# AcherStyx/SSD-Object-Detection

Measured on AMD Instinct MI355X. Metric: images/sec SSD300 train step, batch 64, higher is better.
Workload: dtype bf16; 1 GPU; BASELINE configs[2]: SSD300 full train step (anchor match+encode, image normalisation, conv fwd, loss, conv bwd, per-variable clip (64 variables) + Adam), per-GPU batch 64, 80 classes, synthetic COCO-shaped boxes; per_gpu_batch=64, global_batch=64, parallelism=single

## Files before the change

### include/ssd_hip.h

```cpp
#ifndef SSD_HIP_H
#define SSD_HIP_H

#include <stddef.h>
#include <stdint.h>

#ifdef __cplusplus
extern "C" {
#endif

typedef enum {
    SSD_OK = 0,
    SSD_ERR_ASSERT = -1,
    SSD_ERR_VALUE = -2,
    SSD_ERR_WORKSPACE = -3,
    SSD_ERR_LAUNCH = -4,
    SSD_ERR_UNSUPPORTED = -5
} ssd_status;

typedef enum { SSD_F32 = 0, SSD_BF16 = 1 } ssd_dtype;

int ssd_hip_abi_version(void);
const char* ssd_status_string(int status);

int ssd_priors_count(const int* grid_hw, int levels, const int* ratio_off);
int ssd_priors(const int* grid_hw, int levels, const double* s_ref, const int* ratios,
               const int* ratio_off, double in_size, double* out, void* stream);

#define SSD_MAX_LEVELS 8
#define SSD_GRID_VERIFIED 0x5D5D0001
typedef struct {
    int levels;
    int grid_h[SSD_MAX_LEVELS];
    int grid_w[SSD_MAX_LEVELS];
    int per_cell[SSD_MAX_LEVELS];
    int verified;
} ssd_prior_grid;

int ssd_prior_grid_verify(const double* priors, int A, ssd_prior_grid* grid, int32_t* scratch, void* stream);

int ssd_encode_zero(const double* priors, int A, float* enc_zero, void* stream);

size_t ssd_match_encode_workspace_bytes(int B, int A, int total_gt);
int ssd_match_encode(const float* gt_box, const float* gt_cls, const int32_t* gt_off, int B,
                     int total_gt, int max_nt, const double* priors, const float* enc_zero, int A,
                     const ssd_prior_grid* grid, double thresh, int32_t* out_cls, float* out_loc,
                     uint8_t* out_mask, int32_t* out_owner, void* ws, size_t ws_bytes, void* stream);

int ssd_apply_anchor_box(const float* box, const double* priors, int n, double* out, void* stream);

int ssd_iou_n(const float* b1, const double* b2, int n, double* out, void* stream);

size_t ssd_loss_workspace_bytes(int B, int A, int C);
int ssd_loss_fwd_bwd(const void* conf, const void* loc, int dtype, const int32_t* gt_cls,
                     const float* gt_loc, const uint8_t* gt_mask, int B, int A, int C, float grad_scale,
                     float* out8, void* dconf, void* dloc, void* ws, size_t ws_bytes, void* stream);

typedef struct {
    int levels;
    int hw[SSD_MAX_LEVELS];
    int per_cell[SSD_MAX_LEVELS];
    int npad[SSD_MAX_LEVELS];
    void* rows[SSD_MAX_LEVELS];
    int32_t* row_of_pixel[SSD_MAX_LEVELS];
    int32_t* pixel_of_row[SSD_MAX_LEVELS];
    int32_t* count;
} ssd_head_grads;
size_t ssd_loss_heads_workspace_bytes(int B, int A, int C);
int ssd_loss_fwd_bwd_heads(const void* conf, const void* loc, int dtype, const int32_t* gt_cls, const float* gt_loc,
                           const uint8_t* gt_mask, int B, int A, int C, float grad_scale, float* out8,
                           const ssd_head_grads* hg, void* ws, size_t ws_bytes, int ws_clean, void* stream);

int ssd_score_decode(const void* conf, const void* loc, int dtype, const double* priors, int B, int A, int C,
                     float score_thresh, double in_size, float* score, int32_t* cls, float* box,
                     uint8_t* cand, void* stream);

int ssd_nms_max_candidates(void);
int ssd_nms(const float* score, const int32_t* cls, const float* box, const uint8_t* cand, int B, int A,
            float iou_thresh, int max_cand, uint8_t* keep, int32_t* keep_count, void* stream);

int ssd_conv2d_fwd(const void* x, const void* w, const float* bias, void* y, int B, int H, int W, int Cin,
                   int Cout, int ksize, int stride, int pad_t, int pad_l, int Ho, int Wo, int relu, void* ws,
                   size_t ws_bytes, void* stream);
int ssd_conv2d_fwd_pool(const void* x, const void* w, const float* bias, void* y, void* y_pool, void* pool_code, int B, int H,
                        int W, int Cin, int Cout, int ksize, int stride, int pad_t, int pad_l, int Ho, int Wo, int relu, int Hp,
                        int Wp, void* ws, size_t ws_bytes, void* stream);
int ssd_conv2d_head_fwd(const void* x, const void* w, const float* bias, void* loc, void* conf, int B, int H, int W,
                        int Cin, int per_cell, int classes, int anchors_total, int level_off, void* ws, size_t ws_bytes,
                        void* stream);
int ssd_conv2d_bwd_data(const void* dy, const void* w_t, const void* relu_src, void* dx, int B, int H, int W, int Cin,
                        int Cout_pad, int ksize, int stride, int pad_t, int pad_l, int Ho, int Wo, int accumulate,
                        void* ws, size_t ws_bytes, void* stream);

int ssd_conv2d_fwd_relubits(const void* x, const void* w, const float* bias, void* y, void* relu_bits, int B, int H, int W, int Cin,
                            int Cout, int ksize, int stride, int pad_t, int pad_l, int Ho, int Wo, void* ws, size_t ws_bytes,
                            void* stream);
int ssd_conv2d_bwd_data_bits(const void* dy, const void* w_t, const void* relu_bits, void* dx, int B, int H, int W, int Cin,
                             int Cout_pad, int ksize, int stride, int pad_t, int pad_l, int Ho, int Wo, int accumulate, void* ws,
                             size_t ws_bytes, void* stream);
size_t ssd_conv2d_bwd_data_wgrad_first_workspace_bytes(int B, int H, int W);
int ssd_conv2d_bwd_data_wgrad_first(const void* dy, const void* w_t, const void* relu_bits, const void* image, float* dw0,
                                    float* dbias0, int B, int H, int W, void* ws, size_t ws_bytes, void* stream);
int ssd_conv2d_bwd_data_unpool(const void* dy, const void* w_t, const void* relu_src, const void* pool_code, void* dx_pooled,
                               void* dx_full, int B, int H, int W, int Cin, int Cout_pad, int Hf, int Wf, void* ws, size_t ws_bytes,
                               void* stream);
size_t ssd_conv2d_bwd_weight_unpooled_workspace_bytes(int B, int H, int W, int Cin, int Cout, int Hp, int Wp);
int ssd_conv2d_bwd_weight_unpooled(const void* x, const void* dpool, const void* pool_code, float* dw, float* dbias, int B, int H,
                                   int W, int Cin, int Cout, int Hp, int Wp, void* ws, size_t ws_bytes, void* stream);
size_t ssd_conv2d_bwd_weight_workspace_bytes(int B, int Ho, int Wo, int Cin, int Cout, int ldy, int ksize);
int ssd_conv2d_bwd_weight(const void* x, const void* dy, float* dw, float* dbias, int B, int H, int W, int Cin,
                          int Cout, int ldy, int ksize, int stride, int pad_t, int pad_l, int Ho, int Wo, void* ws,
                          size_t ws_bytes, void* stream);
typedef struct {
    const void* x;
    const void* dy;
    float* dw;
    float* dbias;
    int B, H, W, Cin, Cout, ldy, ksize, stride, pad_t, pad_l, Ho, Wo;
} ssd_wgrad_item;
size_t ssd_conv2d_bwd_weight_batched_workspace_bytes(const ssd_wgrad_item* items, int count);
int ssd_conv2d_bwd_weight_batched(const ssd_wgrad_item* items, int count, void* ws, size_t ws_bytes, void* stream);
int ssd_set_wgrad_reduce_stream(void* stream);
int ssd_weight_transpose(const void* w, void* w_t, int Cout, int ksize, int Cin, int Cout_pad, void* stream);
int ssd_weight_transpose_batched(const long long* desc, int ntensors, int max_tiles, void* stream);
int ssd_cast_bf16(const float* src, void* dst, long long n, void* stream);
int ssd_image_prep(const float* img, void* out, int B, int H, int W, int normalize, void* stream);
int ssd_image_resize_prep(const void* src, const int64_t* src_off, const int32_t* src_hw, void* out, int B, int S,
                          int normalize, void* stream);
int ssd_box_prep(const float* box_tlwh, const int32_t* gt_off, const int32_t* src_hw, float* box_out, int B, int total_gt,
                 void* stream);
int ssd_maxpool2x2_fwd(const void* x, void* y, int B, int H, int W, int C, int Ho, int Wo, void* stream);
int ssd_maxpool2x2_bwd(const void* x, const void* y, const void* dy, void* dx, int B, int H, int W, int C, int Ho,
                       int Wo, void* stream);
int ssd_maxpool2x2_fwd_argmax(const void* x, void* y, void* code, int B, int H, int W, int C, int Ho, int Wo, void* stream);
int ssd_maxpool2x2_bwd_argmax(const void* code, const void* dy, void* dx, int B, int H, int W, int C, int Ho, int Wo,
                              void* stream);
int ssd_quantize_mx_fp8(const void* x_bf16, void* q, void* scale, long long n, void* stream);
int ssd_conv3x3_fwd_mxfp8(const void* x8, const void* xscale, const void* w8, const void* wscale, const float* bias, void* y, int B,
                          int H, int W, int Cin, int Cout, int relu, void* stream);
int ssd_conv2d_fwd_mxfp8(const void* x8, const void* xscale, const void* w8, const void* wscale, const float* bias, void* y_bf16,
                         void* y8, void* yscale, int B, int H, int W, int Cin, int Cout, int k, int stride, int pad_t, int pad_l,
                         int Ho, int Wo, int relu, void* stream);
int ssd_add_relu_fwd_mxfp8(const void* a, const void* b, void* out_bf16, void* q, void* scale, long long n, void* stream);
int ssd_conv2d_fwd_pool_mxfp8(const void* x8, const void* xscale, const void* w8, const void* wscale, const float* bias,
                              void* y_pool_bf16, void* y_pool8, void* y_pool_scale, int B, int H, int W, int Cin, int Cout, int k,
                              int stride, int pad_t, int pad_l, int Ho, int Wo, int relu, int Hp, int Wp, void* stream);
int ssd_conv2d_bwd_data_mxfp8(const void* dy8, const void* dyscale, const void* wt8, const void* wtscale, const void* relu_src,
                              void* dx_bf16, void* dx8, void* dxscale, int B, int H, int W, int Cin, int Cout, int k, int pad_t,
                              int pad_l, int Ho, int Wo, int accumulate, void* stream);
#define SSD_CHAIN_MAX_LAYERS 8
#define SSD_CHAIN_PACK_MAX 16
typedef struct {
    const void* src;
    void* dst;
    int N, K;
} ssd_chain_pack;
int ssd_chain_pack_weights(const ssd_chain_pack* items, int count, void* stream);
int ssd_chain_prefetch(const ssd_chain_pack* items, int count, void* stream);
typedef struct {
    const void* w;
    const float* bias;
    void* out;
    const void* mask_bits;
    const void* mask_src;
    void* relu_bits;
    int Hi, Wi, Kc, Ho, Wo, N, ksize, mul, div, pad_t, pad_l, relu, accumulate;
} ssd_chain_layer;
int ssd_conv_chain(const void* in0, const ssd_chain_layer* layers, int nlayers, int B, void* stream);
int ssd_add_relu_fwd(const void* a, const void* b, void* out, long long n, void* stream);
int ssd_relu_mask_bwd(const void* g, const void* act, void* out, int accumulate, long long n, void* stream);
int ssd_maxpool3x3s2_fwd(const void* x, void* y, void* code, int B, int H, int W, int C, int Ho, int Wo, int pad_t, int pad_l,
                         void* stream);
int ssd_maxpool3x3s2_bwd(const void* code, const void* dy, void* dx, int B, int H, int W, int C, int Ho, int Wo, int pad_t, int pad_l,
                         void* stream);
typedef struct {
    int levels;
    int H[SSD_MAX_LEVELS], W[SSD_MAX_LEVELS], Cin[SSD_MAX_LEVELS], cout[SSD_MAX_LEVELS];
    const void* x[SSD_MAX_LEVELS];
    const void* w_tap[SSD_MAX_LEVELS];
    const void* relu_bits[SSD_MAX_LEVELS];
    const void* relu_src[SSD_MAX_LEVELS];
    void* dx[SSD_MAX_LEVELS];
    float* dw[SSD_MAX_LEVELS];
    float* dbias[SSD_MAX_LEVELS];
} ssd_head_layers;
size_t ssd_heads_bwd_data_sparse_workspace_bytes(int B, const ssd_head_layers* hl);
int ssd_heads_bwd_data_sparse(const ssd_head_grads* hg, const ssd_head_layers* hl, int B, void* ws, size_t ws_bytes,
                              void* stream);
int ssd_heads_bwd_data_sparse_levels(const ssd_head_grads* hg, const ssd_head_layers* hl, int B, unsigned level_mask, int prezeroed,
                                     void* ws, size_t ws_bytes, void* stream);
size_t ssd_heads_bwd_weight_sparse_workspace_bytes(int B, const ssd_head_grads* hg, const ssd_head_layers* hl);
int ssd_heads_bwd_weight_sparse(const ssd_head_grads* hg, const ssd_head_layers* hl, int B, void* ws, size_t ws_bytes,
                                void* stream);

int ssd_head_grad_pack(const void* dloc, const void* dconf, void* out, int B, int hw, int per_cell, int classes,
                       int npad, int anchors_total, int level_off, void* stream);

int ssd_opt_block_elems(void);
int ssd_grad_clip_scales(const float* grad, long long n, const int32_t* tensor_block_off, int ntensors, float clip,
                         double* partial, float* scale, float* norms, void* stream);
int ssd_grad_apply_scale(float* grad, long long n, const int32_t* block_tensor, const float* scale, void* stream);
int ssd_grad_accumulate(float* acc, const float* grad, long long n, const int32_t* block_tensor, const float* scale,
                        int first, void* stream);
int ssd_adam_step(float* param, const float* grad, float* m, float* v, void* param_bf16, long long n,
                  const int32_t* block_tensor, const float* scale, float grad_scale, float lr_t, float beta1,
                  float beta2, float eps, void* stream);
int ssd_sgd_step(float* param, const float* grad, void* param_bf16, long long n, const int32_t* block_tensor,
                 const float* scale, float grad_scale, float lr, void* stream);

enum ssd_conv_plan {
    SSD_PLAN_KERNEL_MASK = 0xff,
    SSD_PLAN_C64B = 1, SSD_PLAN_P32_64, SSD_PLAN_P32_128, SSD_PLAN_8PH,
    SSD_PLAN_DMA_256_256, SSD_PLAN_DMA_256_128, SSD_PLAN_DMA_256_64, SSD_PLAN_DMA_128_64, SSD_PLAN_DMA_128_128,
    SSD_PLAN_CONV0_FWD, SSD_PLAN_P512, SSD_PLAN_PW,
    SSD_PLAN_WG_FIRST = 32, SSD_PLAN_WG_PATCH_16x16, SSD_PLAN_WG_PATCH_6x40, SSD_PLAN_WG_PATCH_10x24, SSD_PLAN_WG_TILE,
    SSD_PLAN_WG_GENERIC,
    SSD_PLAN_F_FLAT = 0x100,
    SSD_PLAN_F_ROWFLAT = 0x200,
    SSD_PLAN_F_SPLITK = 0x400,
    SSD_PLAN_F_POOL_FUSED = 0x800,
    SSD_PLAN_F_S2 = 0x1000,
    SSD_PLAN_F_REDUCE_WIDE = 0x2000
};
int ssd_conv2d_fwd_plan(int B, int H, int W, int Cin, int Cout, int ksize, int stride, int pad_t, int pad_l, int Ho, int Wo,
                        int pool, size_t ws_bytes);
int ssd_conv2d_head_fwd_plan(int B, int H, int W, int Cin, int per_cell, int classes, size_t ws_bytes);
int ssd_conv2d_bwd_data_plan(int B, int H, int W, int Cin, int Cout_pad, int ksize, int stride, int pad_t, int pad_l, int Ho,
                             int Wo, int accumulate, size_t ws_bytes);
int ssd_conv2d_bwd_weight_plan(int B, int H, int W, int Cin, int Cout, int ldy, int ksize, int stride, int pad_t, int pad_l,
                               int Ho, int Wo);
const char* ssd_conv_plan_name(int plan);

int ssd_dev_knob(const char* name, int value);

int ssd_dev_mfma_calibration_workgroups(void);
double ssd_dev_mfma_calibration_flops(int iters);
int ssd_dev_mfma_calibration(int iters, void* stamps, void* sink, void* stream);

#ifdef __cplusplus
}
#endif
#endif
```

### ssd-object-detection_amd/_lib.py

```python
import ctypes
import os

HERE = os.path.dirname(os.path.abspath(__file__))
LIB_PATH = os.path.join(HERE, os.environ.get("SSD_HIP_LIB", "libssd_hip.so"))

SSD_OK, SSD_ERR_ASSERT, SSD_ERR_VALUE, SSD_ERR_WORKSPACE, SSD_ERR_LAUNCH, SSD_ERR_UNSUPPORTED = 0, -1, -2, -3, -4, -5
SSD_MAX_LEVELS = 8

_c_int_p = ctypes.POINTER(ctypes.c_int)
_c_double_p = ctypes.POINTER(ctypes.c_double)
VP = ctypes.c_void_p


class PriorGrid(ctypes.Structure):
    _fields_ = [("levels", ctypes.c_int),
                ("grid_h", ctypes.c_int * SSD_MAX_LEVELS),
                ("grid_w", ctypes.c_int * SSD_MAX_LEVELS),
                ("per_cell", ctypes.c_int * SSD_MAX_LEVELS),
                ("verified", ctypes.c_int)]


class HeadGrads(ctypes.Structure):
    _fields_ = [("levels", ctypes.c_int),
                ("hw", ctypes.c_int * SSD_MAX_LEVELS),
                ("per_cell", ctypes.c_int * SSD_MAX_LEVELS),
                ("npad", ctypes.c_int * SSD_MAX_LEVELS),
                ("rows", VP * SSD_MAX_LEVELS),
                ("row_of_pixel", VP * SSD_MAX_LEVELS),
                ("pixel_of_row", VP * SSD_MAX_LEVELS),
                ("count", VP)]


class HeadLayers(ctypes.Structure):
    _fields_ = [("levels", ctypes.c_int),
                ("H", ctypes.c_int * SSD_MAX_LEVELS),
                ("W", ctypes.c_int * SSD_MAX_LEVELS),
                ("Cin", ctypes.c_int * SSD_MAX_LEVELS),
                ("cout", ctypes.c_int * SSD_MAX_LEVELS),
                ("x", VP * SSD_MAX_LEVELS),
                ("w_tap", VP * SSD_MAX_LEVELS),
                ("relu_bits", VP * SSD_MAX_LEVELS),
                ("relu_src", VP * SSD_MAX_LEVELS),
                ("dx", VP * SSD_MAX_LEVELS),
                ("dw", VP * SSD_MAX_LEVELS),
                ("dbias", VP * SSD_MAX_LEVELS)]


class ChainLayer(ctypes.Structure):
    _fields_ = [("w", VP), ("bias", VP), ("out", VP), ("mask_bits", VP), ("mask_src", VP), ("relu_bits", VP)] + \
               [(n, ctypes.c_int) for n in ("Hi", "Wi", "Kc", "Ho", "Wo", "N", "ksize", "mul", "div", "pad_t", "pad_l", "relu",
                                            "accumulate")]


class WgradItem(ctypes.Structure):
    _fields_ = [("x", VP), ("dy", VP), ("dw", VP), ("dbias", VP)] + \
               [(n, ctypes.c_int) for n in ("B", "H", "W", "Cin", "Cout", "ldy", "ksize", "stride", "pad_t", "pad_l", "Ho", "Wo")]


class ChainPack(ctypes.Structure):
    _fields_ = [("src", VP), ("dst", VP), ("N", ctypes.c_int), ("K", ctypes.c_int)]


SSD_CHAIN_MAX_LAYERS = 8
SSD_CHAIN_PACK_MAX = 16
_HG = ctypes.POINTER(HeadGrads)
_HL = ctypes.POINTER(HeadLayers)

_SIGNATURES = {
    "ssd_hip_abi_version": (ctypes.c_int, []),
    "ssd_status_string": (ctypes.c_char_p, [ctypes.c_int]),
    "ssd_priors_count": (ctypes.c_int, [_c_int_p, ctypes.c_int, _c_int_p]),
    "ssd_priors": (ctypes.c_int, [_c_int_p, ctypes.c_int, _c_double_p, _c_int_p, _c_int_p, ctypes.c_double, VP, VP]),
    "ssd_encode_zero": (ctypes.c_int, [VP, ctypes.c_int, VP, VP]),
    "ssd_prior_grid_verify": (ctypes.c_int, [VP, ctypes.c_int, ctypes.POINTER(PriorGrid), VP, VP]),
    "ssd_match_encode_workspace_bytes": (ctypes.c_size_t, [ctypes.c_int, ctypes.c_int, ctypes.c_int]),
    "ssd_match_encode": (ctypes.c_int, [VP, VP, VP, ctypes.c_int, ctypes.c_int, ctypes.c_int, VP, VP, ctypes.c_int,
                                        ctypes.POINTER(PriorGrid), ctypes.c_double, VP, VP, VP, VP, VP, ctypes.c_size_t, VP]),
    "ssd_apply_anchor_box": (ctypes.c_int, [VP, VP, ctypes.c_int, VP, VP]),
    "ssd_iou_n": (ctypes.c_int, [VP, VP, ctypes.c_int, VP, VP]),
    "ssd_score_decode": (ctypes.c_int, [VP, VP, ctypes.c_int, VP, ctypes.c_int, ctypes.c_int, ctypes.c_int,
                                        ctypes.c_float, ctypes.c_double, VP, VP, VP, VP, VP]),
    "ssd_nms_max_candidates": (ctypes.c_int, []),
    "ssd_nms": (ctypes.c_int, [VP, VP, VP, VP, ctypes.c_int, ctypes.c_int, ctypes.c_float, ctypes.c_int, VP, VP, VP]),
    "ssd_conv2d_fwd": (ctypes.c_int, [VP, VP, VP, VP] + [ctypes.c_int] * 12 + [VP, ctypes.c_size_t, VP]),
    "ssd_conv2d_fwd_pool": (ctypes.c_int, [VP, VP, VP, VP, VP, VP] + [ctypes.c_int] * 14 + [VP, ctypes.c_size_t, VP]),
    "ssd_conv2d_head_fwd": (ctypes.c_int, [VP, VP, VP, VP, VP] + [ctypes.c_int] * 8 + [VP, ctypes.c_size_t, VP]),
    "ssd_conv2d_bwd_data": (ctypes.c_int, [VP, VP, VP, VP] + [ctypes.c_int] * 12 + [VP, ctypes.c_size_t, VP]),
    "ssd_conv2d_fwd_relubits": (ctypes.c_int, [VP] * 5 + [ctypes.c_int] * 11 + [VP, ctypes.c_size_t, VP]),
    "ssd_conv2d_bwd_data_bits": (ctypes.c_int, [VP] * 4 + [ctypes.c_int] * 12 + [VP, ctypes.c_size_t, VP]),
    "ssd_conv2d_bwd_data_unpool": (ctypes.c_int, [VP] * 6 + [ctypes.c_int] * 7 + [VP, ctypes.c_size_t, VP]),
    "ssd_quantize_mx_fp8": (ctypes.c_int, [VP, VP, VP, ctypes.c_longlong, VP]),
    "ssd_conv3x3_fwd_mxfp8": (ctypes.c_int, [VP] * 6 + [ctypes.c_int] * 6 + [VP]),
    "ssd_conv2d_fwd_mxfp8": (ctypes.c_int, [VP] * 8 + [ctypes.c_int] * 12 + [VP]),
    "ssd_add_relu_fwd_mxfp8": (ctypes.c_int, [VP] * 5 + [ctypes.c_longlong, VP]),
    "ssd_conv2d_bwd_data_mxfp8": (ctypes.c_int, [VP] * 8 + [ctypes.c_int] * 11 + [VP]),
    "ssd_conv2d_fwd_pool_mxfp8": (ctypes.c_int, [VP] * 8 + [ctypes.c_int] * 14 + [VP]),
    "ssd_chain_pack_weights": (ctypes.c_int, [ctypes.POINTER(ChainPack), ctypes.c_int, VP]),
    "ssd_chain_prefetch": (ctypes.c_int, [ctypes.POINTER(ChainPack), ctypes.c_int, VP]),
    "ssd_set_wgrad_reduce_stream": (ctypes.c_int, [VP]),
    "ssd_conv2d_bwd_weight_batched_workspace_bytes": (ctypes.c_size_t, [ctypes.POINTER(WgradItem), ctypes.c_int]),
    "ssd_conv2d_bwd_weight_batched": (ctypes.c_int, [ctypes.POINTER(WgradItem), ctypes.c_int, VP, ctypes.c_size_t, VP]),
    "ssd_conv_chain": (ctypes.c_int, [VP, ctypes.POINTER(ChainLayer), ctypes.c_int, ctypes.c_int, VP]),
    "ssd_add_relu_fwd": (ctypes.c_int, [VP, VP, VP, ctypes.c_longlong, VP]),
    "ssd_relu_mask_bwd": (ctypes.c_int, [VP, VP, VP, ctypes.c_int, ctypes.c_longlong, VP]),
    "ssd_maxpool3x3s2_fwd": (ctypes.c_int, [VP, VP, VP] + [ctypes.c_int] * 8 + [VP]),
    "ssd_maxpool3x3s2_bwd": (ctypes.c_int, [VP, VP, VP] + [ctypes.c_int] * 8 + [VP]),
    "ssd_conv2d_bwd_weight_unpooled_workspace_bytes": (ctypes.c_size_t, [ctypes.c_int] * 7),
    "ssd_conv2d_bwd_weight_unpooled": (ctypes.c_int, [VP] * 5 + [ctypes.c_int] * 7 + [VP, ctypes.c_size_t, VP]),
    "ssd_conv2d_bwd_data_wgrad_first_workspace_bytes": (ctypes.c_size_t, [ctypes.c_int] * 3),
    "ssd_conv2d_bwd_data_wgrad_first": (ctypes.c_int, [VP] * 6 + [ctypes.c_int] * 3 + [VP, ctypes.c_size_t, VP]),
    "ssd_conv2d_bwd_weight_workspace_bytes": (ctypes.c_size_t, [ctypes.c_int] * 7),
    "ssd_conv2d_bwd_weight": (ctypes.c_int, [VP, VP, VP, VP] + [ctypes.c_int] * 12 + [VP, ctypes.c_size_t, VP]),
    "ssd_weight_transpose": (ctypes.c_int, [VP, VP, ctypes.c_int, ctypes.c_int, ctypes.c_int, ctypes.c_int, VP]),
    "ssd_cast_bf16": (ctypes.c_int, [VP, VP, ctypes.c_longlong, VP]),
    "ssd_image_prep": (ctypes.c_int, [VP, VP, ctypes.c_int, ctypes.c_int, ctypes.c_int, ctypes.c_int, VP]),
    "ssd_image_resize_prep": (ctypes.c_int, [VP, VP, VP, VP, ctypes.c_int, ctypes.c_int, ctypes.c_int, VP]),
    "ssd_box_prep": (ctypes.c_int, [VP, VP, VP, VP, ctypes.c_int, ctypes.c_int, VP]),
    "ssd_maxpool2x2_fwd": (ctypes.c_int, [VP, VP] + [ctypes.c_int] * 6 + [VP]),
    "ssd_maxpool2x2_bwd": (ctypes.c_int, [VP, VP, VP, VP] + [ctypes.c_int] * 6 + [VP]),
    "ssd_weight_transpose_batched": (ctypes.c_int, [VP, ctypes.c_int, ctypes.c_int, VP]),
    "ssd_maxpool2x2_fwd_argmax": (ctypes.c_int, [VP, VP, VP] + [ctypes.c_int] * 6 + [VP]),
    "ssd_maxpool2x2_bwd_argmax": (ctypes.c_int, [VP, VP, VP] + [ctypes.c_int] * 6 + [VP]),
    "ssd_head_grad_pack": (ctypes.c_int, [VP, VP, VP] + [ctypes.c_int] * 7 + [VP]),
    "ssd_opt_block_elems": (ctypes.c_int, []),
    "ssd_grad_clip_scales": (ctypes.c_int, [VP, ctypes.c_longlong, VP, ctypes.c_int, ctypes.c_float, VP, VP, VP, VP]),
    "ssd_grad_apply_scale": (ctypes.c_int, [VP, ctypes.c_longlong, VP, VP, VP]),
    "ssd_grad_accumulate": (ctypes.c_int, [VP, VP, ctypes.c_longlong, VP, VP, ctypes.c_int, VP]),
    "ssd_adam_step": (ctypes.c_int, [VP, VP, VP, VP, VP, ctypes.c_longlong, VP, VP] + [ctypes.c_float] * 5 + [VP]),
    "ssd_sgd_step": (ctypes.c_int, [VP, VP, VP, ctypes.c_longlong, VP, VP, ctypes.c_float, ctypes.c_float, VP]),
    "ssd_dev_knob": (ctypes.c_int, [ctypes.c_char_p, ctypes.c_int]),
    "ssd_dev_mfma_calibration_workgroups": (ctypes.c_int, []),
    "ssd_dev_mfma_calibration_flops": (ctypes.c_double, [ctypes.c_int]),
    "ssd_dev_mfma_calibration": (ctypes.c_int, [ctypes.c_int, VP, VP, VP]),
    "ssd_conv2d_fwd_plan": (ctypes.c_int, [ctypes.c_int] * 12 + [ctypes.c_size_t]),
    "ssd_conv2d_head_fwd_plan": (ctypes.c_int, [ctypes.c_int] * 6 + [ctypes.c_size_t]),
    "ssd_conv2d_bwd_data_plan": (ctypes.c_int, [ctypes.c_int] * 12 + [ctypes.c_size_t]),
    "ssd_conv2d_bwd_weight_plan": (ctypes.c_int, [ctypes.c_int] * 12),
    "ssd_conv_plan_name": (ctypes.c_char_p, [ctypes.c_int]),
    "ssd_loss_workspace_bytes": (ctypes.c_size_t, [ctypes.c_int, ctypes.c_int, ctypes.c_int]),
    "ssd_loss_heads_workspace_bytes": (ctypes.c_size_t, [ctypes.c_int, ctypes.c_int, ctypes.c_int]),
    "ssd_loss_fwd_bwd_heads": (ctypes.c_int, [VP, VP, ctypes.c_int, VP, VP, VP, ctypes.c_int, ctypes.c_int, ctypes.c_int,
                                              ctypes.c_float, VP, _HG, VP, ctypes.c_size_t, ctypes.c_int, VP]),
    "ssd_heads_bwd_data_sparse_workspace_bytes": (ctypes.c_size_t, [ctypes.c_int, _HL]),
    "ssd_heads_bwd_data_sparse": (ctypes.c_int, [_HG, _HL, ctypes.c_int, VP, ctypes.c_size_t, VP]),
    "ssd_heads_bwd_data_sparse_levels": (ctypes.c_int, [_HG, _HL, ctypes.c_int, ctypes.c_uint, ctypes.c_int, VP, ctypes.c_size_t, VP]),
    "ssd_heads_bwd_weight_sparse_workspace_bytes": (ctypes.c_size_t, [ctypes.c_int, _HG, _HL]),
    "ssd_heads_bwd_weight_sparse": (ctypes.c_int, [_HG, _HL, ctypes.c_int, VP, ctypes.c_size_t, VP]),
    "ssd_loss_fwd_bwd": (ctypes.c_int, [VP, VP, ctypes.c_int, VP, VP, VP, ctypes.c_int, ctypes.c_int, ctypes.c_int,
                                        ctypes.c_float, VP, VP, VP, VP, ctypes.c_size_t, VP]),
}

_lib = None


def lib():
    global _lib
    if _lib is None:
        if not os.path.exists(LIB_PATH):
            raise RuntimeError(
                "libssd_hip.so is missing (%s): build it with `python ssd-object-detection_amd/build.py` "
                "or __graft_entry__.build(); there is no CPU fallback." % LIB_PATH)
        try:
            import torch
        except ImportError:
            pass
        L = ctypes.CDLL(LIB_PATH)
        for name, (res, args) in _SIGNATURES.items():
            fn = getattr(L, name)
            fn.restype = res
            fn.argtypes = args
        _lib = L
    return _lib


def check(status):
    if status == SSD_OK:
        return
    msg = lib().ssd_status_string(status).decode()
    if status == SSD_ERR_ASSERT:
        raise AssertionError(msg)
    if status in (SSD_ERR_VALUE, SSD_ERR_UNSUPPORTED):
        raise ValueError(msg)
    raise RuntimeError("ssd_hip: %s (status %d)" % (msg, status))
```

### ssd-object-detection_amd/csrc/conv.hip

```cpp
#include <atomic>
#include <climits>
#include <cstdint>
#include <cstring>
#include <type_traits>
#include "common.h"
#include <hip/hip_bf16.h>
#include <stdlib.h>

namespace {

}
#include "conv_common.h"
namespace {

template <int EPI>
__global__ void k_igemm_finalize(ConvGeom g, Epilogue ep) {
    const int n4 = (g.N + 3) >> 2;
    const long long idx = (long long)blockIdx.x * blockDim.x + threadIdx.x;
    if (idx >= (long long)g.M * n4) return;
    const int m = (int)(idx / n4), n = (int)(idx - (long long)m * n4) * 4;
    const bool full = n + 3 < g.N;
    float v[4] = {0.f, 0.f, 0.f, 0.f};
    if (full && !(g.N & 3)) {
        for (int z = 0; z < ep.ksplit; ++z) {
// ... 701 lines not shown
    unsigned pvo[8];
#pragma unroll
    for (int j = 0; j < 8; ++j) {
        const int q = (wave + 8 * j) * 64 + lane;
        const int pp = q / 6, sl = q - pp * 6;
        int pix;
        if constexpr (FLAT) {
            pix = pp < 512 + 2 * (Q + 1) ? flat_pixel(f0 - (Q + 1) + pp) : -1;
        } else {
            const int py = pp / PATCH_W, px = pp - py * PATCH_W;
            const int ix = x0 - 1 + px;
            const int ir = pp < P5_PIX ? image_row(py - 1) : -1;
            pix = (ir >= 0 && (unsigned)ix < (unsigned)g.W) ? ir * g.W + ix : -1;
        }
        pvo[j] = (sl < 4 && pix >= 0 && wave + 8 * j < P5_NDMA) ? ((unsigned)pix * (unsigned)g.C + (unsigned)(sl * 8)) * 2u : OOB;
    }
    unsigned wvo;
    {
        const int row = 16 * wave + (lane >> 2);
        const int piece = (lane & 3) ^ ((-(row >> 2)) & 3);
        const int n = n0 + row;
        wvo = n < g.N ? ((unsigned)n * (unsigned)g.ldw + (unsigned)(piece * 8)) * 2u : OOB;
        if (g.ablate & 16) wvo = OOB;
    }
    const int nchunk = g.C >> 5;
    const int nstep = nchunk * 9;
    auto dma_piece = [&](int chunk, int buf, int j, bool live) {
        char* dst = wave + 8 * j < P5_NDMA ? smem + buf * P5_PATCH + (wave + 8 * j) * 1024 : smem + P5_OFF_DUMMY;
        __builtin_amdgcn_raw_ptr_buffer_load_lds(xres, (lds_void*)dst, 16, live ? pvo[j] : OOB, chunk * 64, 0, 0);
    };
    auto dma_w = [&](int step) {
        const int st = step < nstep ? step : nstep - 1;
        const int ch = st / 9, tp = st - ch * 9;
        __builtin_amdgcn_raw_ptr_buffer_load_lds(wres, (lds_void*)(smem + P5_OFF_W + (step & 3) * P5_WSLOT + wave * 1024), 16, wvo,
                                                 (tp * g.C + ch * 32) * 2, 0, 0);
    };
    f32x4_t acc[CT][PT];
#pragma unroll
    for (int c = 0; c < CT; ++c)
#pragma unroll
        for (int p = 0; p < PT; ++p) acc[c][p] = f32x4_t{0.f, 0.f, 0.f, 0.f};

    const int frow = lane & 15, fk = lane >> 4;
    const int xbase = (FLAT ? 8 * wave_m * 16 + frow : 8 * wave_m * PATCH_W + frow) * P32_PITCH + fk * 16;
    constexpr int prow = (FLAT ? 16 : PATCH_W) * P32_PITCH;
    int wbase;
    {
        const int row = wave_n * 64 + frow;
        wbase = P5_OFF_W + row * 64 + ((fk ^ ((-(row >> 2)) & 3)) << 4);
    }
    auto ldf = [&](int addr) { return lds_read_b128_scoped(smem + addr, smem); };
    auto load_x = [&](bf16x8_t (&fx)[PT], int pb, int tap) {
        const int tapoff = pb + xbase + ((tap / 3) * Q + tap % 3) * P32_PITCH;
#pragma unroll
        for (int p = 0; p < PT; ++p) fx[p] = ldf(tapoff + p * prow);
    };
    auto load_w = [&](bf16x8_t (&fw)[CT], int step) {
        const int wb = (step & 3) * P5_WSLOT;
#pragma unroll
        for (int c = 0; c < CT; ++c) fw[c] = ldf(wb + wbase + c * 1024);
    };
#pragma unroll
    for (int j = 0; j < 8; ++j) dma_piece(0, 0, j, true);
    dma_w(0); dma_w(1); dma_w(2);
    bf16x8_t fxa[PT], fxb[PT], fwa[CT], fwb[CT];
    asm volatile("s_waitcnt vmcnt(2)" ::: "memory");
    __builtin_amdgcn_s_barrier();
    load_x(fxa, 0, 0);
    load_w(fwa, 0);
    auto run_chunk = [&](int chunk, auto par_tag) {
        constexpr int PAR = decltype(par_tag)::value;
        const int pb = (chunk & 1) * P5_PATCH;
        const bool next_chunk = chunk + 1 < nchunk && !(g.ablate & 32);
#pragma unroll
        for (int tap = 0; tap < 9; ++tap) {
            constexpr int NT[9] = {1, 3, 5, 5, 5, 3, 1, 1, 1};
            if (NT[tap] == 1) asm volatile("s_waitcnt vmcnt(1) lgkmcnt(0)" ::: "memory");
            else if (NT[tap] == 3) asm volatile("s_waitcnt vmcnt(3) lgkmcnt(0)" ::: "memory");
            else asm volatile("s_waitcnt vmcnt(5) lgkmcnt(0)" ::: "memory");
            __builtin_amdgcn_s_barrier();
            const int step = chunk * 9 + tap;
            dma_w(step + 3);
            if (tap < 4) {
                dma_piece(chunk + 1, (chunk + 1) & 1, 2 * tap, next_chunk);
                dma_piece(chunk + 1, (chunk + 1) & 1, 2 * tap + 1, next_chunk);
            }
            bf16x8_t (&fxc)[PT] = ((tap + PAR) & 1) ? fxb : fxa;
            bf16x8_t (&fxn)[PT] = ((tap + PAR) & 1) ? fxa : fxb;
            bf16x8_t (&fwc)[CT] = ((tap + PAR) & 1) ? fwb : fwa;
            bf16x8_t (&fwn)[CT] = ((tap + PAR) & 1) ? fwa : fwb;
            if (tap < 8) load_x(fxn, pb, tap + 1);
            else load_x(fxn, next_chunk ? (P5_PATCH - pb) : pb, next_chunk ? 0 : 8);
            load_w(fwn, step + 1 < nstep ? step + 1 : step);
#pragma unroll
            for (int c = 0; c < CT; ++c)
#pragma unroll
                for (int p = 0; p < PT; ++p)
                    acc[c][p] = __builtin_amdgcn_mfma_f32_16x16x32_bf16(fwc[c], fxc[p], acc[c][p], 0, 0, 0);
#define SSD_P5_GROUP(NM_) __builtin_amdgcn_sched_group_barrier(0x008, NM_, 0); __builtin_amdgcn_sched_group_barrier(0x100, 1, 0)
            SSD_P5_GROUP(2); SSD_P5_GROUP(2); SSD_P5_GROUP(2); SSD_P5_GROUP(2); SSD_P5_GROUP(2); SSD_P5_GROUP(2);
            SSD_P5_GROUP(2); SSD_P5_GROUP(2); SSD_P5_GROUP(2); SSD_P5_GROUP(2); SSD_P5_GROUP(2); SSD_P5_GROUP(2);
            __builtin_amdgcn_sched_group_barrier(0x008, 8, 0);
#undef SSD_P5_GROUP
            __builtin_amdgcn_sched_barrier(0);
        }
    };
    for (int chunk = 0; chunk < nchunk; chunk += 2) {
        run_chunk(chunk, std::integral_constant<int, 0>{});
        run_chunk(chunk + 1, std::integral_constant<int, 1>{});
    }
    asm volatile("s_waitcnt vmcnt(0) lgkmcnt(0)" ::: "memory");
    if (staged_ok<EPI>(g, ep)) {
        auto row_to_m = [&](int row) {
            if constexpr (FLAT) return flat_pixel(f0 + row);
            const int ir = image_row(row >> 4), xx = x0 + (row & 15);
            return (ir >= 0 && xx < g.Wo) ? ir * g.Wo + xx : -1;
        };
        auto pool_index = [&](int py, int px) -> long long {
            if (FLAT || rowflat) return -1;
            const int gy = (y0 >> 1) + py, gx = (x0 >> 1) + px;
            return (gy < ep.pool_h && gx < ep.pool_w) ? ((long long)b * ep.pool_h + gy) * ep.pool_w + gx : -1;
        };
        staged_epilogue<EPI, 512, BN, CT, PT, 512>(acc, smem, g, ep, n0, wave_m * 128, wave_n * 64, tid, row_to_m, pool_index);
        return;
    }
    int mrow[PT];
#pragma unroll
    for (int p = 0; p < PT; ++p) {
        if constexpr (FLAT) {
            mrow[p] = flat_pixel(f0 + (8 * wave_m + p) * 16 + (lane & 15));
        } else {
            const int ir = image_row(8 * wave_m + p), xx = x0 + (lane & 15);
            mrow[p] = (ir >= 0 && xx < g.Wo) ? ir * g.Wo + xx : -1;
        }
    }
    conv_epilogue_rows<EPI, CT, PT>(acc, g, ep, mrow, n0 + wave_n * 64, lane);
}

constexpr int C64_PITCH = 160;

constexpr int C64B_ROWS = 8;
constexpr int C64B_PATCH_PIX = (C64B_ROWS + 2) * PATCH_W;
constexpr int C64B_NDMA = (C64B_PATCH_PIX * 10 + 63) / 64;
constexpr int C64B_PATCH = C64B_NDMA * 1024;
constexpr int C64B_STAGE = 2 * C64B_PATCH;
constexpr int C64B_FRAG_DEPTH = 3;
constexpr int C64B_BIAS = C64B_STAGE + 128 * 128;
constexpr int C64B_LDS = C64B_BIAS + 256;

struct C64W0 {
    const bf16_raw* img;
    float* slab_w;
    float* slab_b;
};
constexpr int C64B_IMG = 6 * 256;
constexpr int C64B_W0_IMG = 2 * C64B_PATCH;
constexpr int C64B_W0_SUMS = C64B_W0_IMG + 2 * C64B_IMG;
constexpr int C64B_W0_LDS = C64B_W0_SUMS + 4 * 3 * 64 * 16;

typedef __attribute__((address_space(3))) s16x4_t lds_s16x4;
__device__ __forceinline__ s16x4_t lds_read_tr16_scoped(const char* __restrict__ p, const char* __restrict__ other) {
    (void)other;
    return __builtin_amdgcn_ds_read_tr16_b64_v4i16((lds_s16x4*)p);
}

template <int EPI, bool W0 = false>
__global__ __launch_bounds__(256) __attribute__((amdgpu_waves_per_eu(2, 2)))
void k_conv3x3_c64b(const bf16_raw* __restrict__ x, const bf16_raw* __restrict__ w, ConvGeom g, Epilogue ep, int tiles_x, int tiles_y,
                    C64W0 w0) {
    static_assert(!W0 || EPI == EPI_DGRAD, "the fused first-layer weight gradient belongs to the data gradient");
    extern __shared__ __attribute__((aligned(16))) char smem[];
    const int tid = threadIdx.x, lane = tid & 63;
    const int wave = __builtin_amdgcn_readfirstlane(tid >> 6);
    const int wave_m = wave & 1, wave_n = wave >> 1;
    const int nblocks = g.B * tiles_x * tiles_y;
    const __amdgpu_buffer_rsrc_t xres = __builtin_amdgcn_make_buffer_rsrc((void*)x, 0, (unsigned)g.B * g.H * g.W * 64u * 2u, 0x00020000);
    constexpr unsigned OOB = 0xfffffff0u;
    constexpr int NJ = (C64B_NDMA + 3) / 4;
    const __amdgpu_buffer_rsrc_t ires = __builtin_amdgcn_make_buffer_rsrc((void*)(W0 ? w0.img : x), 0, (unsigned)g.B * g.H * g.W * 16u, 0x00020000);

    int pcode[NJ];
#pragma unroll
    for (int j = 0; j < NJ; ++j) {
        const int q = (wave + 4 * j) * 64 + lane;
        const int pp = q / 10, sl = q - pp * 10;
        const int py = pp / PATCH_W, px = pp - py * PATCH_W;
        pcode[j] = (sl < 8 && pp < C64B_PATCH_PIX && wave + 4 * j < C64B_NDMA) ? ((py << 16) | (px << 8) | (sl * 16)) : -1;
    }
    auto issue_patch = [&](int t, int buf) {
        int r = t;
        const int tx = r % tiles_x; r /= tiles_x;
        const int ty = r % tiles_y;
        const int b = r / tiles_y;
#pragma unroll
        for (int j = 0; j < NJ; ++j) {
            if (wave + 4 * j < C64B_NDMA) {
                const int iy = ty * C64B_ROWS - 1 + (pcode[j] >> 16), ix = tx * 16 - 1 + ((pcode[j] >> 8) & 255);
                const bool ok = pcode[j] >= 0 && (unsigned)iy < (unsigned)g.H && (unsigned)ix < (unsigned)g.W;
                const unsigned off = (unsigned)((b * g.H + iy) * g.W + ix) * 128u + (unsigned)(pcode[j] & 255);
                __builtin_amdgcn_raw_ptr_buffer_load_lds(xres, (lds_void*)(smem + buf * C64B_PATCH + (wave + 4 * j) * 1024), 16,
                                                         ok ? off : OOB, 0, 0, 0);
            }
        }
        if constexpr (W0) {
#pragma unroll
            for (int j = 0; j < 2; ++j) {
                if (wave + 4 * j < 6) {
                    const int q = (wave + 4 * j) * 64 + lane, pp = q >> 1;
                    const int py = pp / PATCH_W, px = pp - py * PATCH_W;
                    const int iy = ty * C64B_ROWS - 1 + py, ix = tx * 16 - 1 + px;
                    const bool ok = pp < C64B_PATCH_PIX && (unsigned)iy < (unsigned)g.H && (unsigned)ix < (unsigned)g.W;
                    const unsigned off = (unsigned)((b * g.H + iy) * g.W + ix) * 16u + (unsigned)(q & 1) * 4u;
                    __builtin_amdgcn_raw_ptr_buffer_load_lds(ires, (lds_void*)(smem + C64B_W0_IMG + buf * C64B_IMG + (wave + 4 * j) * 256), 4,
                                                             ok ? off : OOB, 0, 0, 0);
                }
            }
        }
    };
    const bool xcd_order = (gridDim.x & 7) == 0 && !(g.ablate & 64);
    const int per_xcd = (nblocks + 7) >> 3, slots = gridDim.x >> 3;
    auto block_of = [&](int i) {
        if (!xcd_order) { const int t = blockIdx.x + i * gridDim.x; return t < nblocks ? t : -1; }
        const int lin = i * slots + ((int)blockIdx.x >> 3);
        const int t = ((int)blockIdx.x & 7) * per_xcd + lin;
        return (lin < per_xcd && t < nblocks) ? t : -1;
    };
    if (block_of(0) >= 0) issue_patch(block_of(0), 0);

    const int frow = lane & 15, fk = lane >> 4;
    bf16x8_t fw[2][9][2];
#pragma unroll
    for (int c = 0; c < 2; ++c) {
        const int n = wave_n * 32 + c * 16 + frow;
#pragma unroll
        for (int tap = 0; tap < 9; ++tap)
#pragma unroll
            for (int ks = 0; ks < 2; ++ks) {
                uint4 v = make_uint4(0, 0, 0, 0);
                if (n < g.N) v = *reinterpret_cast<const uint4*>(w + (unsigned)n * 576u + (unsigned)(tap * 64 + ks * 32 + fk * 8));
                fw[c][tap][ks] = *reinterpret_cast<const bf16x8_t*>(&v);
            }
    }
    const int xbase = (4 * wave_m * PATCH_W + frow) * C64_PITCH + fk * 16;
    if constexpr (EPI == EPI_FWD) {
        if (tid < 64) reinterpret_cast<float*>(smem + C64B_BIAS)[tid] = (ep.bias && tid < g.N) ? ep.bias[tid] : 0.f;
    }
    if constexpr (W0) {
        f32x4_t* sums = reinterpret_cast<f32x4_t*>(smem + C64B_W0_SUMS) + wave * 3 * 64 + lane;
#pragma unroll
        for (int nt = 0; nt < 3; ++nt) sums[nt * 64] = f32x4_t{0.f, 0.f, 0.f, 0.f};
    }

    unsigned mkn[4] = {0u, 0u, 0u, 0u};
    auto load_masks = [&](int t) {
        int r = t;
        const int tx = r % tiles_x; r /= tiles_x;
        const int ty = r % tiles_y;
        const int b = r / tiles_y;
#pragma unroll
        for (int p = 0; p < 4; ++p) {
            const int y = ty * C64B_ROWS + 4 * wave_m + p, xx = tx * 16 + (lane & 15);
            mkn[p] = 0u;
            if (y < g.Ho && xx < g.Wo)
                mkn[p] = *reinterpret_cast<const unsigned*>(ep.mask_bits + (long long)((b * g.Ho + y) * g.Wo + xx) * 8 + wave_n * 4);
        }
    };
    if constexpr (W0) { if (block_of(0) >= 0) load_masks(block_of(0)); }

    int it = 0, prev_st = 0;
    for (int t = block_of(0); t >= 0; t = block_of(++it)) {
        const int cur = it & 1;
        if (g.ablate & 2) {}
        else if (prev_st >= 6) asm volatile("s_waitcnt vmcnt(6) lgkmcnt(0)" ::: "memory");
        else if (prev_st == 5) asm volatile("s_waitcnt vmcnt(5) lgkmcnt(0)" ::: "memory");
        else if (prev_st == 4) asm volatile("s_waitcnt vmcnt(4) lgkmcnt(0)" ::: "memory");
        else if (prev_st == 3) asm volatile("s_waitcnt vmcnt(3) lgkmcnt(0)" ::: "memory");
        else if (prev_st == 2) asm volatile("s_waitcnt vmcnt(2) lgkmcnt(0)" ::: "memory");
        else if (prev_st == 1) asm volatile("s_waitcnt vmcnt(1) lgkmcnt(0)" ::: "memory");
        else asm volatile("s_waitcnt vmcnt(0) lgkmcnt(0)" ::: "memory");
        __syncthreads();
        __builtin_amdgcn_s_setprio(0);
        int r = t;
        const int tx = r % tiles_x; r /= tiles_x;
        const int ty = r % tiles_y;
        const int b = r / tiles_y;
        const int y0 = ty * C64B_ROWS, x0 = tx * 16;
        unsigned mk[4];
        auto chunk_pixel = [&](int t, int i) {
            const int y = y0 + 2 * i + (t >> 7), xx = x0 + ((t >> 3) & 15);
            return (y < g.Ho && xx < g.Wo) ? (b * g.Ho + y) * g.Wo + xx : -1;
        };
        const bool premask = EPI == EPI_DGRAD && ep.mask_bits != nullptr && !(g.ablate & 128);
        if constexpr (W0) {
#pragma unroll
            for (int p = 0; p < 4; ++p) mk[p] = mkn[p];
        } else if constexpr (EPI == EPI_DGRAD) {
#pragma unroll
            for (int i = 0; i < 4; ++i) {
                const int m = chunk_pixel(tid, i);
                mk[i] = 0u;
                if (premask && m >= 0) mk[i] = ep.mask_bits[(long long)m * 8 + (tid & 7)];
            }
        }
        const int tnext = block_of(it + 1);
        if (tnext >= 0 && !(g.ablate & 1)) issue_patch(tnext, cur ^ 1);
        if constexpr (W0) { if (tnext >= 0) load_masks(tnext); }
        const int pb = cur * C64B_PATCH + xbase;
        f32x4_t acc[2][4];
#pragma unroll
        for (int c = 0; c < 2; ++c) {
            f32x4_t a0 = f32x4_t{0.f, 0.f, 0.f, 0.f};
            if constexpr (EPI == EPI_FWD)
                a0 = *reinterpret_cast<const f32x4_t*>(smem + C64B_BIAS + (wave_n * 32 + c * 16 + (lane >> 4) * 4) * 4);
#pragma unroll
            for (int p = 0; p < 4; ++p) acc[c][p] = a0;
        }
        auto frag = [&](int s2) {
            return *reinterpret_cast<const bf16x8_t*>(smem + pb + ((s2 / 6) * PATCH_W + (s2 / 2) % 3) * C64_PITCH + (s2 & 1) * 64);
        };
        constexpr int FD = C64B_FRAG_DEPTH;
        bf16x8_t fr[FD];
#pragma unroll
        for (int i = 0; i < FD - 1; ++i) fr[i] = frag(i);
#pragma unroll
        for (int s2 = 0; s2 < 36; ++s2) {
            if (s2 + FD - 1 < 36) fr[(s2 + FD - 1) % FD] = frag(s2 + FD - 1);
            const int rr = s2 / 6, dx = (s2 / 2) % 3, ks = s2 & 1;
#pragma unroll
            for (int dy = 0; dy < 3; ++dy) {
                const int p = rr - dy;
                if (p >= 0 && p < 4) {
#pragma unroll
                    for (int c = 0; c < 2; ++c)
                        acc[c][p] = __builtin_amdgcn_mfma_f32_16x16x32_bf16(fw[c][dy * 3 + dx][ks], fr[s2 % FD], acc[c][p], 0, 0, 0);
                }
            }
            __builtin_amdgcn_sched_barrier(0);
        }
        __builtin_amdgcn_s_setprio(3);
        if (g.ablate & 8) {
#pragma unroll
            for (int c = 0; c < 2; ++c)
#pragma unroll
                for (int p = 0; p < 4; ++p) asm volatile("" :: "v"(acc[c][p]));
            prev_st = 0;
            continue;
        }
        auto row_to_m = [&](int row) {
            const int y = y0 + (row >> 4), xx = x0 + (row & 15);
            return (y < g.Ho && xx < g.Wo) ? (b * g.Ho + y) * g.Wo + xx : -1;
        };
        auto pool_index = [&](int py, int px) -> long long {
            const int gy = (y0 >> 1) + py, gx = (x0 >> 1) + px;
            return (gy < ep.pool_h && gx < ep.pool_w) ? ((long long)b * ep.pool_h + gy) * ep.pool_w + gx : -1;
        };
        if constexpr (W0) {
            char* st = smem + cur * C64B_PATCH;
            asm volatile("s_waitcnt lgkmcnt(0)" ::: "memory");
            __builtin_amdgcn_s_barrier();
            int t2 = tid;
            asm volatile("" : "+v"(t2));
            {
                const int l3 = t2 & 63;
#pragma unroll
                for (int c = 0; c < 2; ++c) {
                    const int col = wave_n * 32 + c * 16 + (l3 >> 4) * 4;
                    const int sh = 8 * (2 * c + (l3 >> 5)) + 4 * ((l3 >> 4) & 1);
#pragma unroll
                    for (int p = 0; p < 4; ++p) {
                        const int row = wave_m * 64 + p * 16 + (l3 & 15);
                        const unsigned bits = mk[p] >> sh;
                        const unsigned k0 = keep_mask2(bits, 0), k1 = keep_mask2(bits, 2);
                        lds_st8_scoped(st + row * 128 + ((((col >> 3) ^ row) & 7) << 4) + (col & 4) * 2, smem,
                            make_uint2((pack_bf16x2(acc[c][p][0], acc[c][p][1])) & k0,
                                       (pack_bf16x2(acc[c][p][2], acc[c][p][3])) & k1));
                    }
                }
            }
            asm volatile("s_waitcnt lgkmcnt(0)" ::: "memory");
            __builtin_amdgcn_s_barrier();
            int l2 = t2 & 63;
            const int gq = l2 >> 4, q = (l2 >> 2) & 3, p4 = l2 & 3;
            int db[2], ib[3];
#pragma unroll
            for (int h = 0; h < 2; ++h) {
                const int r = 8 * gq + q + 4 * h;
                db[h] = r * 128 + ((((2 * wave + (p4 >> 1)) ^ r) & 7) << 4) + (p4 & 1) * 8;
            }
#pragma unroll
            for (int nt = 0; nt < 3; ++nt) {
                int tap = 4 * nt + p4;
                if (tap > 8) tap = 8;
                ib[nt] = (((gq >> 1) + tap / 3) * PATCH_W + 8 * (gq & 1) + q + tap % 3) * 8;
            }
            const char* im = smem + C64B_W0_IMG + cur * C64B_IMG;
            f32x4_t* sums = reinterpret_cast<f32x4_t*>(smem + C64B_W0_SUMS) + wave * 3 * 64 + l2;
            f32x4_t aw[3];
#pragma unroll
            for (int nt = 0; nt < 3; ++nt) {
                const uint4 u = lds_ld16_scoped(reinterpret_cast<const char*>(sums + nt * 64), smem);
                aw[nt] = f32x4_t{__uint_as_float(u.x), __uint_as_float(u.y), __uint_as_float(u.z), __uint_as_float(u.w)};
            }
            bf16x8_t ones;
#pragma unroll
            for (int e = 0; e < 8; ++e) ones[e] = (__bf16)1.0f;
#pragma unroll
            for (int s = 0; s < 4; ++s) {
                bf16x8_t fd;
                reinterpret_cast<s16x4_t*>(&fd)[0] = lds_read_tr16_scoped(st + db[0] + s * 4096, smem);
                reinterpret_cast<s16x4_t*>(&fd)[1] = lds_read_tr16_scoped(st + db[1] + s * 4096, smem);
#pragma unroll
                for (int nt = 0; nt < 3; ++nt) {
                    bf16x8_t fp;
                    reinterpret_cast<s16x4_t*>(&fp)[0] = lds_read_tr16_scoped(im + ib[nt] + s * (2 * PATCH_W * 8), smem);
                    reinterpret_cast<s16x4_t*>(&fp)[1] = lds_read_tr16_scoped(im + ib[nt] + s * (2 * PATCH_W * 8) + 32, smem);
                    if (nt == 1) fp = (l2 & 15) == 3 ? ones : fp;
                    aw[nt] = __builtin_amdgcn_mfma_f32_16x16x32_bf16(fd, fp, aw[nt], 0, 0, 0);
                }
            }
#pragma unroll
            for (int nt = 0; nt < 3; ++nt)
                lds_st16_scoped(reinterpret_cast<char*>(sums + nt * 64), smem,
                                make_uint4(__float_as_uint(aw[nt][0]), __float_as_uint(aw[nt][1]), __float_as_uint(aw[nt][2]), __float_as_uint(aw[nt][3])));
            prev_st = 0;
            continue;
        }
        if constexpr (EPI == EPI_FWD) {
            char* st = smem + C64B_STAGE;
#pragma unroll
            for (int c = 0; c < 2; ++c) {
                const int col = wave_n * 32 + c * 16 + (lane >> 4) * 4;
#pragma unroll
                for (int p = 0; p < 4; ++p) {
                    const int row = wave_m * 64 + p * 16 + (lane & 15);
                    float v[4] = {acc[c][p][0], acc[c][p][1], acc[c][p][2], acc[c][p][3]};
                    if (ep.relu) {
#pragma unroll
                        for (int j = 0; j < 4; ++j) v[j] = fmaxf(v[j], 0.f);
                    }
                    lds_st8_scoped(st + row * 128 + ((((col >> 3) ^ row) & 7) << 4) + (col & 4) * 2, smem,
                        make_uint2(pack_bf16x2(v[0], v[1]), pack_bf16x2(v[2], v[3])));
                }
            }
            asm volatile("s_waitcnt lgkmcnt(0)" ::: "memory");
            __builtin_amdgcn_s_barrier();
            int t2 = tid;
            asm volatile("" : "+v"(t2));
            staged_store<EPI_FWD, 128, 64, 256, decltype(row_to_m), decltype(pool_index)>(st, g, ep, 0, t2, row_to_m, pool_index);
        } else if (premask) {
            if constexpr (EPI == EPI_DGRAD) {
                char* st = smem + C64B_STAGE;
#pragma unroll
                for (int c = 0; c < 2; ++c) {
                    const int col = wave_n * 32 + c * 16 + (lane >> 4) * 4;
#pragma unroll
                    for (int p = 0; p < 4; ++p) {
                        const int row = wave_m * 64 + p * 16 + (lane & 15);
                        lds_st8_scoped(st + row * 128 + ((((col >> 3) ^ row) & 7) << 4) + (col & 4) * 2, smem,
                            make_uint2(pack_bf16x2(acc[c][p][0], acc[c][p][1]),
// ... 444 lines not shown
                ok = ok && (unsigned)iy < (unsigned)g.H && (unsigned)ix < (unsigned)g.W;
                pix = (unsigned)((b * g.H + iy) * g.W + ix);
            }
            const unsigned ox_ = pix * (unsigned)g.C * 2u + xcol[j];
            __builtin_amdgcn_raw_ptr_buffer_load_lds(xres, (lds_void*)(base + XOFF + (wave + 8 * j) * 1024), 16,
                                                     ok ? ox_ : OOB, 0, 0, 0);
        }
    };

    f32x4_t acc[8][4];
    f32x4_t accb[8];
#pragma unroll
    for (int a = 0; a < 8; ++a) {
        accb[a] = f32x4_t{0.f, 0.f, 0.f, 0.f};
#pragma unroll
        for (int c = 0; c < 4; ++c) acc[a][c] = f32x4_t{0.f, 0.f, 0.f, 0.f};
    }
    const bool do_bias = slab_b != nullptr && bx == 0 && wave_n == 0;
    bf16x8_t ones;
#pragma unroll
    for (int i = 0; i < 8; ++i) ones[i] = (__bf16)1.0f;

    const int gq = lane >> 4, li = lane & 15;
    const int kk0 = (gq >> 1) * 16 + (gq & 1) * 4 + (li >> 2);
    const int key = kk0 & 7;
    int abase[8], bbase[4];
#pragma unroll
    for (int a = 0; a < 8; ++a) abase[a] = kk0 * 512 + ((wave_m * 8 + (a ^ key)) << 5) + (li & 3) * 8;
#pragma unroll
    for (int c = 0; c < 4; ++c) {
        const int gl = wave_n * 4 + c;
        bbase[c] = XOFF + kk0 * 512 + (((gl & 8) | ((gl & 7) ^ key)) << 5) + (li & 3) * 8;
    }
    auto rd = [&](int addr) { return lds_read_tr16_scoped(smem + addr, smem); };

    const int nsteps = STAGES == 4 ? (m_end - m_begin + 31) / 32 : (m_end - m_begin + 63) / 64;
    if constexpr (STAGES == 4) {
#pragma unroll
        for (int p = 0; p < 3; ++p)
            if (p < nsteps) issue_dma(m_begin + p * 32, p);
    } else {
        if (nsteps > 0) issue_dma(m_begin, 0);
    }
    auto run = [&](auto bias_tag) {
        constexpr bool BIAS = decltype(bias_tag)::value;
        for (int st = 0; st < nsteps; ++st) {
            if constexpr (STAGES == 4) {
                const int younger = min(2, nsteps - 1 - st);
                if (younger == 2) asm volatile("s_waitcnt vmcnt(8)" ::: "memory");
                else if (younger == 1) asm volatile("s_waitcnt vmcnt(4)" ::: "memory");
                else asm volatile("s_waitcnt vmcnt(0)" ::: "memory");
                __builtin_amdgcn_s_barrier();
                asm volatile("" ::: "memory");
                if (st + 3 < nsteps) issue_dma(m_begin + (st + 3) * 32, (st + 3) & 3);
                const int boff = (st & 3) * (2 * XOFF);
                bf16x8_t fb[4], fa[8];
#pragma unroll
                for (int c = 0; c < 4; ++c)
#pragma unroll
                    for (int half = 0; half < 2; ++half)
                        reinterpret_cast<s16x4_t*>(&fb[c])[half] = rd(bbase[c] + boff + half * 4096);
#pragma unroll
                for (int a = 0; a < 8; ++a)
#pragma unroll
                    for (int half = 0; half < 2; ++half)
                        reinterpret_cast<s16x4_t*>(&fa[a])[half] = rd(abase[a] + boff + half * 4096);
#pragma unroll
                for (int a = 0; a < 8; ++a) {
#pragma unroll
                    for (int c = 0; c < 4; ++c)
                        acc[a][c] = __builtin_amdgcn_mfma_f32_16x16x32_bf16(fa[a], fb[c], acc[a][c], 0, 0, 0);
                    if constexpr (BIAS) accb[a] = __builtin_amdgcn_mfma_f32_16x16x32_bf16(fa[a], ones, accb[a], 0, 0, 0);
                }
                continue;
            }
            const int cur = st & 1;
            asm volatile("s_waitcnt vmcnt(0)" ::: "memory");
            __syncthreads();
            if (st + 1 < nsteps) issue_dma(m_begin + (st + 1) * 64, cur ^ 1);
            const int boff = cur * (2 * WT_TILE);
            int ab[8], bb[4];
#pragma unroll
            for (int a = 0; a < 8; ++a) ab[a] = abase[a] + boff;
#pragma unroll
            for (int c = 0; c < 4; ++c) bb[c] = bbase[c] + boff;
#pragma unroll
            for (int ksub = 0; ksub < 2; ++ksub) {
                bf16x8_t fb[4], fa[8];
#pragma unroll
                for (int c = 0; c < 4; ++c)
#pragma unroll
                    for (int half = 0; half < 2; ++half)
                        reinterpret_cast<s16x4_t*>(&fb[c])[half] = rd(bb[c] + ksub * 16384 + half * 4096);
#pragma unroll
                for (int a = 0; a < 8; ++a)
#pragma unroll
                    for (int half = 0; half < 2; ++half)
                        reinterpret_cast<s16x4_t*>(&fa[a])[half] = rd(ab[a] + ksub * 16384 + half * 4096);
#pragma unroll
                for (int a = 0; a < 8; ++a) {
#pragma unroll
                    for (int c = 0; c < 4; ++c)
                        acc[a][c] = __builtin_amdgcn_mfma_f32_16x16x32_bf16(fa[a], fb[c], acc[a][c], 0, 0, 0);
                    if constexpr (BIAS) accb[a] = __builtin_amdgcn_mfma_f32_16x16x32_bf16(fa[a], ones, accb[a], 0, 0, 0);
                }
            }
        }
    };
    if (do_bias) run(std::true_type{}); else run(std::false_type{});

    float* out = slab_w + (long long)split * g.N * ktot;
#pragma unroll
    for (int a = 0; a < 8; ++a)
#pragma unroll
        for (int c = 0; c < 4; ++c) {
            const int col = col0 + wave_n * 64 + c * 16 + (lane & 15);
            if (col >= ktot) continue;
#pragma unroll
            for (int j = 0; j < 4; ++j) {
                const int co = co0 + wave_m * 128 + a * 16 + (lane >> 4) * 4 + j;
                if (co < g.N) out[(long long)co * ktot + col] = acc[a][c][j];
            }
        }
    if (do_bias && (lane & 15) == 0) {
        float* ob = slab_b + (long long)split * g.N;
#pragma unroll
        for (int a = 0; a < 8; ++a)
#pragma unroll
            for (int j = 0; j < 4; ++j) {
                const int co = co0 + wave_m * 128 + a * 16 + (lane >> 4) * 4 + j;
                if (co < g.N) ob[co] = accb[a][j];
            }
    }
}

template <int BH, int BW8>
struct WpGeom {
    static constexpr int BW = BW8 * 8;
    static constexpr int PW = BW + 2, PH = BH + 2;
    static constexpr int PPIX = PW * PH;
    static constexpr int P_INSTR = (PPIX * 8 + 63) / 64;
    static constexpr int P_BYTES = P_INSTR * 1024;
    static constexpr int NPG = (BH / 2) * BW8;
    static constexpr int KS = (NPG + 1) / 2;
    static constexpr int DY_PIX = KS * 32;
    static constexpr int DY_BYTES = DY_PIX * 128;
    static constexpr int DY_INSTR = DY_PIX / 8;
    static constexpr int BUF = DY_BYTES + P_BYTES;
    static_assert(BH % 2 == 0 && DY_INSTR % 8 == 0, "block shape");
};

__device__ __forceinline__ int wp_key(int px) { return (px >> 1) & 3; }

template <int BH, int BW8>
__global__ __launch_bounds__(512) void k_conv3x3_wgrad_patch(const bf16_raw* __restrict__ x, const bf16_raw* __restrict__ dy,
                                                             float* __restrict__ slab_w, float* __restrict__ slab_b,
                                                             ConvGeom g, int tiles_x, int tiles_y, int tiles_per_split,
                                                             int nsplit, int cout, int single_buf, int xg) {
    using G = WpGeom<BH, BW8>;
    extern __shared__ __attribute__((aligned(16))) char smem[];

    const int tid = threadIdx.x, lane = tid & 63;
    const int wave = __builtin_amdgcn_readfirstlane(tid >> 6);
    const int ct = wave & 3, role = wave >> 2;
    const int nchunk = g.C >> 6, cotiles = (cout + 63) >> 6;
    const int nunits = nchunk * cotiles * nsplit;
    const int j = blockIdx.x >> 3;
    int id = ((j / xg) * 8 + (blockIdx.x & 7)) * xg + j % xg;
    if (id >= nunits) return;
    const int chunk = id % nchunk; id /= nchunk;
    const int cot = id % cotiles;
    const int split = id / cotiles;
    const int co0 = cot * 64, ci0 = chunk * 64;
    const int ntiles = g.B * tiles_x * tiles_y;
    const int t_begin = split * tiles_per_split, t_end = min(ntiles, t_begin + tiles_per_split);

    const __amdgpu_buffer_rsrc_t xres = __builtin_amdgcn_make_buffer_rsrc((void*)x, 0, (unsigned)g.B * g.H * g.W * g.C * 2u, 0x00020000);
    const __amdgpu_buffer_rsrc_t dyres = __builtin_amdgcn_make_buffer_rsrc((void*)dy, 0, (unsigned)g.B * g.Ho * g.Wo * g.N * 2u, 0x00020000);
    constexpr unsigned WP_OOB = 0xfffffff0u;
    auto issue_dma = [&](int t, int buf) {
        int r = t;
        const int tx = r % tiles_x; r /= tiles_x;
        const int ty = r % tiles_y;
        const int b = r / tiles_y;
        const int y0 = ty * BH, x0 = tx * G::BW;
        char* base = smem + buf * G::BUF;
#pragma unroll
        for (int j = 0; j < G::DY_INSTR / 4; ++j) {
            const int i = ct + 4 * j;
            const int kk = 8 * i + (lane >> 3), sl = lane & 7;
            const int c16 = (((sl >> 1) ^ wp_key(kk)) << 1) | (sl & 1);
            const int pg = kk >> 4;
            const int rp = pg / BW8, xg = pg - rp * BW8;
            const int y = y0 + 2 * rp + ((kk >> 3) & 1), xx = x0 + xg * 8 + (kk & 7);
            const int co = co0 + c16 * 8;
            const bool ok = pg < G::NPG && y < g.Ho && xx < g.Wo && co < g.N;
            const unsigned off = ((unsigned)((b * g.Ho + y) * g.Wo + xx) * (unsigned)g.N + (unsigned)co) * 2u;
            __builtin_amdgcn_raw_ptr_buffer_load_lds(dyres, (lds_void*)(base + i * 1024), 16, ok ? off : WP_OOB, 0, 0, 0);
        }
#pragma unroll
        for (int j = 0; j < (G::P_INSTR + 3) / 4; ++j) {
            const int i = ct + 4 * j;
            if (i < G::P_INSTR) {
                const int pp = 8 * i + (lane >> 3), sl = lane & 7;
                const int c16 = (((sl >> 1) ^ wp_key(pp)) << 1) | (sl & 1);
                const int py = pp / G::PW, px = pp - py * G::PW;
                const int iy = y0 - 1 + py, ix = x0 - 1 + px;
                const bool ok = pp < G::PPIX && (unsigned)iy < (unsigned)g.H && (unsigned)ix < (unsigned)g.W;
                const unsigned off = ((unsigned)((b * g.H + iy) * g.W + ix) * (unsigned)g.C + (unsigned)(ci0 + c16 * 8)) * 2u;
                __builtin_amdgcn_raw_ptr_buffer_load_lds(xres, (lds_void*)(base + G::DY_BYTES + i * 1024), 16, ok ? off : WP_OOB, 0, 0, 0);
            }
        }
    };

    constexpr int LTAPS = 4;
    f32x4_t acc[4][9 - LTAPS];
    f32x4_t accb[4];
#pragma unroll
    for (int a = 0; a < 4; ++a) {
        accb[a] = f32x4_t{0.f, 0.f, 0.f, 0.f};
#pragma unroll
        for (int t5 = 0; t5 < 9 - LTAPS; ++t5) acc[a][t5] = f32x4_t{0.f, 0.f, 0.f, 0.f};
    }
    const bool do_bias = slab_b != nullptr && chunk == 0 && ct == 0 && role == 1;
    bf16x8_t ones;
#pragma unroll
    for (int i = 0; i < 8; ++i) ones[i] = (__bf16)1.0f;

    if (t_begin < t_end && role == 0) issue_dma(t_begin, 0);
    const int gq = lane >> 4, li = lane & 15;
    int abase[4];
    {
        const int kk0 = (gq >> 1) * 8 + (gq & 1) * 4 + (li >> 2);
#pragma unroll
        for (int a = 0; a < 4; ++a) abase[a] = kk0 * 128 + ((a ^ wp_key(kk0)) << 5) + (li & 3) * 8;
    }
    int gbase[8];
    {
        const int p0 = (gq >> 1) * G::PW + (gq & 1) * 4 + (li >> 2);
#pragma unroll
        for (int r = 0; r < 8; ++r) gbase[r] = G::DY_BYTES + (p0 + r) * 128 + ((ct ^ wp_key(p0 + r)) << 5) + (li & 3) * 8;
    }
    typedef __attribute__((address_space(3))) s16x4_t lds_s16x4;
    struct Frag { bf16x8_t fa[4]; bf16x8_t fb[9 - LTAPS]; };
    auto run = [&](auto role_tag, auto bias_tag) {
        constexpr int ROLE = decltype(role_tag)::value;
        constexpr bool BIAS = decltype(bias_tag)::value;
        constexpr int TAP0 = ROLE == 0 ? 0 : LTAPS, NTAP = ROLE == 0 ? LTAPS : 9 - LTAPS;
        auto load_frag = [&](Frag& f, const int (&ab)[4], const int (&gb)[8], auto ks_tag) {
            constexpr int ks = decltype(ks_tag)::value;
#pragma unroll
            for (int half = 0; half < 2; ++half)
#pragma unroll
                for (int a = 0; a < 4; ++a)
                    reinterpret_cast<s16x4_t*>(&f.fa[a])[half] =
                        lds_read_tr16_scoped(smem + ab[a] + (ks * 2 + half) * 2048, smem);
#pragma unroll
            for (int t5 = 0; t5 < NTAP; ++t5)
#pragma unroll
                for (int half = 0; half < 2; ++half) {
                    const int tap = TAP0 + t5;
                    const int pg = (ks * 2 + half) < G::NPG ? (ks * 2 + half) : 0;
                    const int rp = pg / BW8, xg = pg - rp * BW8;
                    const int ctap = (2 * rp + tap / 3) * G::PW + xg * 8 + (tap % 3);
                    reinterpret_cast<s16x4_t*>(&f.fb[t5])[half] =
                        lds_read_tr16_scoped(smem + gb[ctap & 7] + (ctap >> 3) * 1024, smem);
                }
        };
        for (int t = t_begin; t < t_end; ++t) {
            const int cur = (t - t_begin) & 1;
            asm volatile("s_waitcnt vmcnt(0)" ::: "memory");
            __syncthreads();
            if constexpr (ROLE == 0) { if (t + 1 < t_end) issue_dma(t + 1, cur ^ 1); }
            const int boff = cur * G::BUF;
            int ab[4], gb[8];
#pragma unroll
            for (int a = 0; a < 4; ++a) ab[a] = abase[a] + boff;
#pragma unroll
            for (int r = 0; r < 8; ++r) gb[r] = gbase[r] + boff;
            Frag f0, f1;
            auto mma = [&](const Frag& f) {
#pragma unroll
                for (int t5 = 0; t5 < NTAP; ++t5)
#pragma unroll
                    for (int a = 0; a < 4; ++a)
                        acc[a][t5] = __builtin_amdgcn_mfma_f32_16x16x32_bf16(f.fa[a], f.fb[t5], acc[a][t5], 0, 0, 0);
                if constexpr (BIAS) {
#pragma unroll
                    for (int a = 0; a < 4; ++a) accb[a] = __builtin_amdgcn_mfma_f32_16x16x32_bf16(f.fa[a], ones, accb[a], 0, 0, 0);
                }
            };
            auto weave = [&]() {
                constexpr int NR = 8 + 2 * NTAP, NM = 4 * NTAP;
                constexpr int PAIRS = NR < NM ? NR : NM;
                if constexpr (NR > PAIRS) {
                    __builtin_amdgcn_sched_group_barrier(0x100, NR - PAIRS, 0);
                }
#pragma unroll
                for (int i = 0; i < PAIRS; ++i) {
                    __builtin_amdgcn_sched_group_barrier(0x008, 1, 0);
                    __builtin_amdgcn_sched_group_barrier(0x100, 1, 0);
                }
                constexpr int REST = NM - PAIRS + (BIAS ? 4 : 0);
                if constexpr (REST > 0) __builtin_amdgcn_sched_group_barrier(0x008, REST, 0);
            };
            static_assert(G::KS == 8, "the hand-unrolled pipeline below assumes eight k-steps per block");
            load_frag(f0, ab, gb, std::integral_constant<int, 0>{});
            __builtin_amdgcn_s_setprio(0);
            load_frag(f1, ab, gb, std::integral_constant<int, 1>{}); mma(f0); weave();
            load_frag(f0, ab, gb, std::integral_constant<int, 2>{}); mma(f1); weave();
            load_frag(f1, ab, gb, std::integral_constant<int, 3>{}); mma(f0); weave();
            load_frag(f0, ab, gb, std::integral_constant<int, 4>{}); mma(f1); weave();
            load_frag(f1, ab, gb, std::integral_constant<int, 5>{}); mma(f0); weave();
            load_frag(f0, ab, gb, std::integral_constant<int, 6>{}); mma(f1); weave();
            load_frag(f1, ab, gb, std::integral_constant<int, 7>{}); mma(f0); weave();
            mma(f1);
            __builtin_amdgcn_s_setprio(3);
        }
    };
    if (role == 0) run(std::integral_constant<int, 0>{}, std::false_type{});
    else if (do_bias) run(std::integral_constant<int, 1>{}, std::true_type{});
    else run(std::integral_constant<int, 1>{}, std::false_type{});
    const int ktot = g.ldw;
    float* out = slab_w + (long long)split * g.N * ktot;
    const int tap0 = role == 0 ? 0 : LTAPS, ntap = role == 0 ? LTAPS : 9 - LTAPS;
#pragma unroll
    for (int a = 0; a < 4; ++a)
#pragma unroll
        for (int t5 = 0; t5 < 9 - LTAPS; ++t5) {
            if (t5 >= ntap) continue;
            const int col = (tap0 + t5) * g.C + ci0 + ct * 16 + (lane & 15);
#pragma unroll
            for (int j = 0; j < 4; ++j) {
                const int co = co0 + a * 16 + (lane >> 4) * 4 + j;
                if (co < g.N) out[(long long)co * ktot + col] = acc[a][t5][j];
            }
        }
    if (do_bias && (lane & 15) == 0) {
        float* ob = slab_b + (long long)split * g.N;
#pragma unroll
        for (int a = 0; a < 4; ++a)
#pragma unroll
            for (int j = 0; j < 4; ++j) {
                const int co = co0 + a * 16 + (lane >> 4) * 4 + j;
                if (co < g.N) ob[co] = accb[a][j];
            }
    }
}

constexpr int W0_DY = 256 * 128;
constexpr int W0_PATCH = 6 * 1024;
constexpr int W0_BUF = W0_DY + W0_PATCH;

__global__ __launch_bounds__(512) void k_conv0_wgrad(const bf16_raw* __restrict__ x, const bf16_raw* __restrict__ dy,
                                                     float* __restrict__ slab_w, float* __restrict__ slab_b, ConvGeom g,
                                                     int tiles_x, int tiles_y, int tiles_per_split, int cout) {
    extern __shared__ __attribute__((aligned(16))) char smem[];
    const int tid = threadIdx.x, lane = tid & 63;
    const int wave = __builtin_amdgcn_readfirstlane(tid >> 6);
    const int split = blockIdx.x;
    const int ntiles = g.B * tiles_x * tiles_y;
    const int t_begin = split * tiles_per_split, t_end = min(ntiles, t_begin + tiles_per_split);

    auto issue_dma = [&](int t, int buf) {
        int r = t;
        const int tx = r % tiles_x; r /= tiles_x;
        const int ty = r % tiles_y;
        const int b = r / tiles_y;
        const int y0 = ty * 16, x0 = tx * 16;
        char* base = smem + buf * W0_BUF;
#pragma unroll
        for (int j = 0; j < 4; ++j) {
            const int i = wave + 8 * j;
            const int kk = 8 * i + (lane >> 3), sl = lane & 7;
            const int c16 = (((sl >> 1) ^ wp_key(kk)) << 1) | (sl & 1);
            const int pg = kk >> 4;
            const int y = y0 + 2 * (pg >> 1) + ((kk >> 3) & 1), xx = x0 + (pg & 1) * 8 + (kk & 7);
            const int co = c16 * 8;
            const bool ok = y < g.Ho && xx < g.Wo && co < g.N;
            const bf16_raw* src = ok ? dy + ((unsigned)((b * g.Ho + y) * g.Wo + xx) * (unsigned)g.N + (unsigned)co)
                                     : reinterpret_cast<const bf16_raw*>(g_zero16);
            __builtin_amdgcn_global_load_lds((gbl_void*)src, (lds_void*)(base + i * 1024), 16, 0, 0);
        }
        if (wave < 6) {
            const int pp = wave * 64 + lane;
            const int py = pp / PATCH_W, px = pp - py * PATCH_W;
            const int iy = y0 - 1 + py, ix = x0 - 1 + px;
            const bool ok = pp < PATCH_PIX && (unsigned)iy < (unsigned)g.H && (unsigned)ix < (unsigned)g.W;
            const bf16_raw* src = ok ? x + (unsigned)((b * g.H + iy) * g.W + ix) * 8u : reinterpret_cast<const bf16_raw*>(g_zero16);
            __builtin_amdgcn_global_load_lds((gbl_void*)src, (lds_void*)(base + W0_DY + wave * 1024), 16, 0, 0);
        }
    };

    f32x4_t acc[4][5];
    f32x4_t accb[4];
#pragma unroll
    for (int a = 0; a < 4; ++a) {
        accb[a] = f32x4_t{0.f, 0.f, 0.f, 0.f};
#pragma unroll
        for (int c = 0; c < 5; ++c) acc[a][c] = f32x4_t{0.f, 0.f, 0.f, 0.f};
    }
    bf16x8_t ones;
#pragma unroll
    for (int i = 0; i < 8; ++i) ones[i] = (__bf16)1.0f;

    const int gq = lane >> 4, li = lane & 15;
    const int kk0 = (gq >> 1) * 8 + (gq & 1) * 4 + (li >> 2);
    int abase[4];
#pragma unroll
    for (int a = 0; a < 4; ++a) abase[a] = wave * 4096 + kk0 * 128 + ((a ^ wp_key(kk0)) << 5) + (li & 3) * 8;
    const int p0 = (2 * wave + (gq >> 1)) * PATCH_W + (gq & 1) * 4 + (li >> 2);
    int bbase[5];
#pragma unroll
    for (int t = 0; t < 5; ++t) {
        int tap = 2 * t + ((li >> 1) & 1);
        if (tap > 8) tap = 8;
        bbase[t] = W0_DY + (p0 + (tap / 3) * PATCH_W + tap % 3) * 16 + (li & 1) * 8;
    }
    typedef __attribute__((address_space(3))) s16x4_t lds_s16x4;
    auto rd = [&](int addr) { return lds_read_tr16_scoped(smem + addr, smem); };

    if (t_begin < t_end) issue_dma(t_begin, 0);
    for (int t = t_begin; t < t_end; ++t) {
        const int cur = (t - t_begin) & 1;
        asm volatile("s_waitcnt vmcnt(0)" ::: "memory");
        __syncthreads();
        if (t + 1 < t_end) issue_dma(t + 1, cur ^ 1);
        const int boff = cur * W0_BUF;
        bf16x8_t fa[4], fb[5];
#pragma unroll
        for (int half = 0; half < 2; ++half) {
#pragma unroll
            for (int a = 0; a < 4; ++a) reinterpret_cast<s16x4_t*>(&fa[a])[half] = rd(boff + abase[a] + half * 2048);
#pragma unroll
            for (int c = 0; c < 5; ++c) reinterpret_cast<s16x4_t*>(&fb[c])[half] = rd(boff + bbase[c] + half * 8 * 16);
        }
#pragma unroll
        for (int a = 0; a < 4; ++a) {
#pragma unroll
            for (int c = 0; c < 5; ++c) acc[a][c] = __builtin_amdgcn_mfma_f32_16x16x32_bf16(fa[a], fb[c], acc[a][c], 0, 0, 0);
            accb[a] = __builtin_amdgcn_mfma_f32_16x16x32_bf16(fa[a], ones, accb[a], 0, 0, 0);
        }
    }
    __syncthreads();
    float* red = reinterpret_cast<float*>(smem);
    for (int w = 0; w < 8; ++w) {
        if (wave == w) {
#pragma unroll
            for (int a = 0; a < 4; ++a) {
#pragma unroll
                for (int c = 0; c < 6; ++c) {
                    f32x4_t v;
                    if (c < 5) v = acc[a][c < 5 ? c : 0]; else v = accb[a];
                    f32x4_t* slot = reinterpret_cast<f32x4_t*>(red + ((a * 6 + c) * 64 + lane) * 4);
                    if (w > 0) { const f32x4_t o = *slot; v[0] += o[0]; v[1] += o[1]; v[2] += o[2]; v[3] += o[3]; }
                    *slot = v;
                }
            }
        }
        __syncthreads();
    }
    const int ktot = g.ldw;
    for (int idx = tid; idx < 24 * 64; idx += 512) {
        const int tile = idx >> 6, l = idx & 63;
        const int a = tile / 6, c = tile - a * 6;
        const f32x4_t v = *reinterpret_cast<const f32x4_t*>(red + idx * 4);
#pragma unroll
        for (int j = 0; j < 4; ++j) {
            const int co = a * 16 + (l >> 4) * 4 + j;
            if (co >= g.N) continue;
// ... 544 lines not shown
}

extern "C" {

int ssd_set_wgrad_reduce_stream(void* stream) {
    t_reduce_stream = (hipStream_t)stream;
    return SSD_OK;
}

int ssd_dev_knob(const char* name, int value) {
    if (!name) return SSD_ERR_VALUE;
    Knob* k = find_knob(name);
    if (!k) return SSD_ERR_VALUE;
    k->value.store(value, std::memory_order_relaxed);
    return SSD_OK;
}

static int conv2d_fwd_impl(const void* x, const void* w, const float* bias, void* y, int B, int H, int W, int Cin, int Cout,
                           int ksize, int stride, int pad_t, int pad_l, int Ho, int Wo, int relu, void* ws, size_t ws_bytes,
                           void* stream, int* plan, void* relu_bits = nullptr) {
    if (!x || !w || !y || !geom_ok(B, H, W, Cin, Ho, Wo, Cout, ksize) || stride <= 0) return SSD_ERR_VALUE;
    const ConvGeom g = make_geom(B, H, W, Cin, Ho, Wo, Cout, ksize, ksize, stride, 1, pad_t, pad_l);
    if (knob("SSD_CONV_FIRST", 1) && Cin == 8 && Cout == 64 && ksize == 3 && stride == 1 && pad_t == 1 && pad_l == 1 && H == Ho &&
        W == Wo && H >= 16 && W >= 16) {
        SSD_PLAN(SSD_PLAN_CONV0_FWD);
        const int tx = (Wo + 15) / 16, ty = (Ho + 15) / 16;
        hipLaunchKernelGGL(k_conv0_fwd, dim3((unsigned)(B * tx * ty < 768 ? B * tx * ty : 768)), dim3(512), 0, (hipStream_t)stream,
                           static_cast<const bf16_raw*>(x), static_cast<const bf16_raw*>(w), bias, static_cast<bf16_raw*>(y), g, relu,
                           tx, ty, static_cast<unsigned char*>(relu_bits));
        return ssd_launch_status();
    }
    Epilogue ep = {};
    ep.bias = bias; ep.relu = relu; ep.out = static_cast<bf16_raw*>(y); ep.ldo = Cout;
    ep.relu_bits = static_cast<unsigned char*>(relu_bits);
    return launch_igemm<EPI_FWD>(x, w, g, ep, (hipStream_t)stream, ws, ws_bytes, nullptr, plan);
}

int ssd_conv2d_fwd(const void* x, const void* w, const float* bias, void* y, int B, int H, int W, int Cin, int Cout,
                   int ksize, int stride, int pad_t, int pad_l, int Ho, int Wo, int relu, void* ws, size_t ws_bytes,
                   void* stream) {
    return conv2d_fwd_impl(x, w, bias, y, B, H, W, Cin, Cout, ksize, stride, pad_t, pad_l, Ho, Wo, relu, ws, ws_bytes, stream,
                           nullptr);
}

static int conv2d_fwd_pool_impl(const void* x, const void* w, const float* bias, void* y, void* y_pool, void* pool_code, int B,
                                int H, int W, int Cin, int Cout, int ksize, int stride, int pad_t, int pad_l, int Ho, int Wo,
                                int relu, int Hp, int Wp, void* ws, size_t ws_bytes, void* stream, int* plan) {
    if (!x || !w || !y_pool || !pool_code || !geom_ok(B, H, W, Cin, Ho, Wo, Cout, ksize) || stride <= 0 || Cout % 8)
        return SSD_ERR_VALUE;
    if ((Hp != Ho / 2 && Hp != (Ho + 1) / 2) || (Wp != Wo / 2 && Wp != (Wo + 1) / 2) || Hp <= 0 || Wp <= 0) return SSD_ERR_VALUE;
    const ConvGeom g = make_geom(B, H, W, Cin, Ho, Wo, Cout, ksize, ksize, stride, 1, pad_t, pad_l);
    Epilogue ep = {};
    ep.bias = bias; ep.relu = relu; ep.out = static_cast<bf16_raw*>(y); ep.ldo = Cout;
    if (!y && !knob("SSD_CONV_POOL_FUSE", 1)) return SSD_ERR_VALUE;
    if (knob("SSD_CONV_POOL_FUSE", 1)) {
        ep.pool_out = static_cast<bf16_raw*>(y_pool); ep.pool_code = static_cast<unsigned*>(pool_code); ep.pool_h = Hp; ep.pool_w = Wp;
    }
    bool pooled = false;
    const int rc = launch_igemm<EPI_FWD>(x, w, g, ep, (hipStream_t)stream, ws, ws_bytes, &pooled, plan);
    if (rc != SSD_OK || pooled || plan) return rc;
    return ssd_maxpool2x2_fwd_argmax(y, y_pool, pool_code, B, Ho, Wo, Cout, Hp, Wp, stream);
}

int ssd_conv2d_fwd_pool(const void* x, const void* w, const float* bias, void* y, void* y_pool, void* pool_code, int B, int H,
                        int W, int Cin, int Cout, int ksize, int stride, int pad_t, int pad_l, int Ho, int Wo, int relu, int Hp,
                        int Wp, void* ws, size_t ws_bytes, void* stream) {
    return conv2d_fwd_pool_impl(x, w, bias, y, y_pool, pool_code, B, H, W, Cin, Cout, ksize, stride, pad_t, pad_l, Ho, Wo, relu,
                                Hp, Wp, ws, ws_bytes, stream, nullptr);
}

static int conv2d_head_fwd_impl(const void* x, const void* w, const float* bias, void* loc, void* conf, int B, int H, int W,
                                int Cin, int per_cell, int classes, int anchors_total, int level_off, void* ws, size_t ws_bytes,
                                void* stream, int* plan) {
    const int N = per_cell * (4 + classes);
    if (!x || !w || !loc || !conf || !geom_ok(B, H, W, Cin, H, W, N, 3) || per_cell <= 0 || classes <= 0) return SSD_ERR_VALUE;
    const ConvGeom g = make_geom(B, H, W, Cin, H, W, N, 3, 3, 1, 1, 1, 1);
    Epilogue ep = {};
    ep.bias = bias; ep.loc = static_cast<bf16_raw*>(loc); ep.conf = static_cast<bf16_raw*>(conf);
    ep.n_loc = per_cell * 4; ep.n_conf = per_cell * classes; ep.anchors_total = anchors_total;
    ep.level_off = level_off; ep.per_cell = per_cell; ep.classes = classes;
    return launch_igemm<EPI_HEAD>(x, w, g, ep, (hipStream_t)stream, ws, ws_bytes, nullptr, plan);
}

int ssd_conv2d_head_fwd(const void* x, const void* w, const float* bias, void* loc, void* conf, int B, int H, int W,
                        int Cin, int per_cell, int classes, int anchors_total, int level_off, void* ws, size_t ws_bytes,
                        void* stream) {
    return conv2d_head_fwd_impl(x, w, bias, loc, conf, B, H, W, Cin, per_cell, classes, anchors_total, level_off, ws, ws_bytes,
                                stream, nullptr);
}

static int conv2d_bwd_data_impl(const void* dy, const void* w_t, const void* relu_src, void* dx, int B, int H, int W, int Cin,
                                int Cout_pad, int ksize, int stride, int pad_t, int pad_l, int Ho, int Wo, int accumulate,
                                void* ws, size_t ws_bytes, void* stream, int* plan, const void* up_code = nullptr,
                                void* up_dx = nullptr, int up_h = 0, int up_w = 0, const void* mask_bits = nullptr) {
    if (!dy || !w_t || (!dx && !up_dx) || !geom_ok(B, Ho, Wo, Cout_pad, H, W, Cin, ksize) || stride <= 0) return SSD_ERR_VALUE;
    const ConvGeom g = make_geom(B, Ho, Wo, Cout_pad, H, W, Cin, ksize, ksize, 1, stride, ksize - 1 - pad_t,
                                 ksize - 1 - pad_l);
    Epilogue ep = {};
    ep.out = static_cast<bf16_raw*>(dx); ep.ldo = Cin; ep.mask_src = static_cast<const bf16_raw*>(relu_src);
    ep.accumulate = accumulate;
    ep.up_code = static_cast<const unsigned*>(up_code); ep.up_out = static_cast<bf16_raw*>(up_dx); ep.up_h = up_h; ep.up_w = up_w;
    ep.mask_bits = static_cast<const unsigned char*>(mask_bits);
    return launch_igemm<EPI_DGRAD>(dy, w_t, g, ep, (hipStream_t)stream, ws, ws_bytes, nullptr, plan);
}

int ssd_conv2d_fwd_relubits(const void* x, const void* w, const float* bias, void* y, void* relu_bits, int B, int H, int W, int Cin,
                            int Cout, int ksize, int stride, int pad_t, int pad_l, int Ho, int Wo, void* ws, size_t ws_bytes,
                            void* stream) {
    if (!relu_bits || Cout % 8) return SSD_ERR_VALUE;
    return conv2d_fwd_impl(x, w, bias, y, B, H, W, Cin, Cout, ksize, stride, pad_t, pad_l, Ho, Wo, 1, ws, ws_bytes, stream, nullptr,
                           relu_bits);
}

int ssd_conv2d_bwd_data_bits(const void* dy, const void* w_t, const void* relu_bits, void* dx, int B, int H, int W, int Cin,
                             int Cout_pad, int ksize, int stride, int pad_t, int pad_l, int Ho, int Wo, int accumulate, void* ws,
                             size_t ws_bytes, void* stream) {
    if (!relu_bits || Cin % 8) return SSD_ERR_VALUE;
    return conv2d_bwd_data_impl(dy, w_t, nullptr, dx, B, H, W, Cin, Cout_pad, ksize, stride, pad_t, pad_l, Ho, Wo, accumulate, ws,
                                ws_bytes, stream, nullptr, nullptr, nullptr, 0, 0, relu_bits);
}

int ssd_conv2d_bwd_data_unpool(const void* dy, const void* w_t, const void* relu_src, const void* pool_code, void* dx_pooled,
                               void* dx_full, int B, int H, int W, int Cin, int Cout_pad, int Hf, int Wf, void* ws, size_t ws_bytes,
                               void* stream) {
    if (!pool_code || !dx_full || Cin % 8 || Hf <= 0 || Wf <= 0) return SSD_ERR_VALUE;
    if ((H != Hf / 2 && H != (Hf + 1) / 2) || (W != Wf / 2 && W != (Wf + 1) / 2)) return SSD_ERR_VALUE;
    if (2 * H < Hf || 2 * W < Wf) return SSD_ERR_UNSUPPORTED;
    if ((long long)B * Hf * Wf * Cin >= (1ll << 32)) return SSD_ERR_VALUE;
    return conv2d_bwd_data_impl(dy, w_t, relu_src, dx_pooled, B, H, W, Cin, Cout_pad, 3, 1, 1, 1, H, W, 0, ws, ws_bytes, stream, nullptr,
                                pool_code, dx_full, Hf, Wf);
}

int ssd_conv2d_bwd_data(const void* dy, const void* w_t, const void* relu_src, void* dx, int B, int H, int W, int Cin,
                        int Cout_pad, int ksize, int stride, int pad_t, int pad_l, int Ho, int Wo, int accumulate,
                        void* ws, size_t ws_bytes, void* stream) {
    return conv2d_bwd_data_impl(dy, w_t, relu_src, dx, B, H, W, Cin, Cout_pad, ksize, stride, pad_t, pad_l, Ho, Wo, accumulate,
                                ws, ws_bytes, stream, nullptr);
}

static int wgrad_patch_min_hw() {
    return knob("SSD_WGRAD_PATCH", 16);
}

static void launch_wgrad_reduce(hipStream_t s, const float* slab_w, long long sw, long long nw, float* dw, const float* slab_b,
                                long long sb, int nb, float* db, int ns) {
    ssd_launch_wgrad_reduce(s, slab_w, sw, nw, dw, slab_b, sb, nb, db, ns);
}

size_t ssd_conv2d_bwd_data_wgrad_first_workspace_bytes(int B, int H, int W) {
    if (B <= 0 || H <= 0 || W <= 0) return 0;
    return (size_t)512 * (64 * 72 + 64) * sizeof(float);
}

int ssd_conv2d_bwd_data_wgrad_first(const void* dy, const void* w_t, const void* relu_bits, const void* image, float* dw0,
                                    float* dbias0, int B, int H, int W, void* ws, size_t ws_bytes, void* stream) {
    if (!dy || !w_t || !relu_bits || !image || !dw0 || B <= 0 || H <= 0 || W <= 0) return SSD_ERR_VALUE;
    if (H < 16 || W < 16 || (long long)B * H * W * 64 >= (1ll << 31) - 16) return SSD_ERR_UNSUPPORTED;
    if (!ws || ws_bytes < ssd_conv2d_bwd_data_wgrad_first_workspace_bytes(B, H, W)) return SSD_ERR_WORKSPACE;
    const ConvGeom g = make_geom(B, H, W, 64, H, W, 64, 3, 3, 1, 1, 1, 1);
    Epilogue ep = {};
    ep.ldo = 64;
    ep.mask_bits = static_cast<const unsigned char*>(relu_bits);
    const int tiles_x = (W + 15) / 16, tiles_y = (H + C64B_ROWS - 1) / C64B_ROWS;
    const int nblocks = B * tiles_x * tiles_y;
    const unsigned grid = (unsigned)(nblocks < 512 ? nblocks : 512);
    float* slab_w = static_cast<float*>(ws);
    float* slab_b = slab_w + (size_t)512 * 64 * 72;
    hipStream_t s = (hipStream_t)stream;
    auto kern = k_conv3x3_c64b<EPI_DGRAD, true>;
    static OnceLds set; if (ensure_lds(set, reinterpret_cast<const void*>(kern), (int)(C64B_W0_LDS)) != 0) return SSD_ERR_LAUNCH;
    hipLaunchKernelGGL(kern, dim3(grid), dim3(256), C64B_W0_LDS, s, static_cast<const bf16_raw*>(dy), static_cast<const bf16_raw*>(w_t),
                       g, ep, tiles_x, tiles_y, C64W0{static_cast<const bf16_raw*>(image), slab_w, dbias0 ? slab_b : nullptr});
    if (hipGetLastError() != hipSuccess) return SSD_ERR_LAUNCH;
    launch_wgrad_reduce(s, slab_w, 64ll * 72, 64ll * 72, dw0, slab_b, 64ll, 64, dbias0, (int)grid);
    return ssd_launch_status();
}

static bool wgrad_first_layer(int H, int W, int Ho, int Wo, int Cin, int Cout, int ldy, int ksize, int stride, int pad_t, int pad_l) {
    return knob("SSD_WGRAD_FIRST", 1) && Cin == 8 && Cout <= 64 && ldy <= 64 && ksize == 3 && stride == 1 && pad_t == 1 && pad_l == 1 &&
           H == Ho && W == Wo && H >= 16 && W >= 16;
}

static bool wgrad_use_patch(int H, int W, int Ho, int Wo, int Cin, int ksize, int stride, int pad_t, int pad_l) {
    const int mn = wgrad_patch_min_hw();
    return mn > 0 && ksize == 3 && stride == 1 && pad_t == 1 && pad_l == 1 && H == Ho && W == Wo && Cin % 64 == 0 &&
           H >= mn && W >= mn;
}

static int wgrad_patch_shape(int Ho, int Wo, int* bh, int* bw) {
    static const int shapes[3][3] = {{16, 16, 16}, {6, 40, 15}, {10, 24, 15}};
    int best = 0;
    double best_cost = 0;
    for (int i = 0; i < 3; ++i) {
        const double cost = (double)((Ho + shapes[i][0] - 1) / shapes[i][0]) * ((Wo + shapes[i][1] - 1) / shapes[i][1]);
        if (i == 0 || cost < best_cost) { best = i; best_cost = cost; }
    }
    const int forced = knob("SSD_WGRAD_PATCH_SHAPE", -1);
    if (forced >= 0 && forced < 3) best = forced;
    *bh = shapes[best][0]; *bw = shapes[best][1];
    return best;
}

static void wgrad_patch_plan(int B, int Ho, int Wo, int Cin, int Cout, int* tiles_x, int* tiles_y, int* tps, int* ns) {
    int bh, bw;
    wgrad_patch_shape(Ho, Wo, &bh, &bw);
    *tiles_x = (Wo + bw - 1) / bw; *tiles_y = (Ho + bh - 1) / bh;
    const int ntiles = B * *tiles_x * *tiles_y;
    const int groups = (Cin / 64) * ((Cout + 63) / 64);
    const int wp_mult = knob("SSD_WGRAD_PATCH_SINGLE", 0) ? 2 : 1;
    int want = knob("SSD_WGRAD_PATCH_WGS", 256) * wp_mult / groups;
    if (want < 1) want = 1;
    if (want > ntiles) want = ntiles;
    *tps = (ntiles + want - 1) / want;
    *ns = (ntiles + *tps - 1) / *tps;
}

static void wgrad_tiles(int Cout, long long ktot, int* bmo, int* bnc) {
    (void)Cout; (void)ktot;
    *bmo = 128; *bnc = 128;
}

static int wgrad_splits(long long M, int tiles) {
    long long want = 768 / tiles;
    long long maxs = (M + 511) / 512;
    if (want > maxs) want = maxs;
    if (want < 1) want = 1;
    if (want > 512) want = 512;
    return (int)want;
}

static bool wgrad_use_tile(long long M, int Cout, int ldy, long long ktot, long long x_elems) {
    const long long tiles = ((ktot + 255) / 256) * ((Cout + 255) / 256);
    return knob("SSD_WGRAD_TILE", 1) && Cout > 128 && ktot >= 256 && M >= 2048 && M * ldy < (1ll << 31) - 16 &&
           x_elems < (1ll << 31) - 16 && tiles >= knob("SSD_WGTILE_MIN_TILES", 0);
}

static int wgrad_tile_splits(long long M, int tiles, long long slab_elems) {
    int best = 1;
    double best_cost = 0;
    const long long maxs = M / 256 > 0 ? M / 256 : 1;
    for (int ns = 1; ns <= 64 && ns <= maxs; ++ns) {
        const long long rounds = ((long long)tiles * ns + 255) / 256;
        const long long steps = ((M + ns - 1) / ns + 63) / 64;
        const double cost = (double)rounds * steps * 2.2 + (double)ns * slab_elems * 8.0 / 4.0e6 * (knob("SSD_WGTILE_SLAB_X", 10) / 10.0);
        if (ns == 1 || cost < best_cost) { best = ns; best_cost = cost; }
    }
    return best;
}

size_t ssd_conv2d_bwd_weight_workspace_bytes(int B, int Ho, int Wo, int Cin, int Cout, int ldy, int ksize) {
    if (B <= 0 || Ho <= 0 || Wo <= 0 || Cin <= 0 || Cout <= 0 || ldy < Cout || ksize <= 0) return 0;
    const long long ktot = (long long)ksize * ksize * Cin;
    size_t patch_bytes = 0;
    if (wgrad_use_patch(Ho, Wo, Ho, Wo, Cin, ksize, 1, 1, 1)) {
        int tx, ty, tps, ns;
        wgrad_patch_plan(B, Ho, Wo, Cin, Cout, &tx, &ty, &tps, &ns);
        patch_bytes = (size_t)ns * ((size_t)ldy * ktot + ldy) * sizeof(float);
    }
    int bmo, bnc;
    wgrad_tiles(Cout, ktot, &bmo, &bnc);
    const int tiles = (int)(((ktot + bnc - 1) / bnc) * ((Cout + bmo - 1) / bmo));
    const int ns = wgrad_splits((long long)B * Ho * Wo, tiles);
    size_t gen = (size_t)ns * ((size_t)ldy * ktot + ldy) * sizeof(float);
    if (Cin == 8 && Cout <= 64 && ldy <= 64 && ksize == 3) {
        const size_t first = (size_t)512 * ((size_t)ldy * ktot + ldy) * sizeof(float);
        if (first > gen) gen = first;
    }
    if (Cout > 128 && ktot >= 256) {
        const int t2 = (int)(((ktot + 255) / 256) * ((Cout + 255) / 256));
        const int ns2 = wgrad_tile_splits((long long)B * Ho * Wo, t2, (long long)ldy * ktot);
        const size_t gen2 = (size_t)ns2 * ((size_t)ldy * ktot + ldy) * sizeof(float);
        if (gen2 > gen) gen = gen2;
    }
    return gen > patch_bytes ? gen : patch_bytes;
}

static int conv2d_bwd_weight_impl(const void* x, const void* dy, float* dw, float* dbias, int B, int H, int W, int Cin, int Cout,
                                  int ldy, int ksize, int stride, int pad_t, int pad_l, int Ho, int Wo, void* ws, size_t ws_bytes,
                                  void* stream, int* plan) {
    if (!x || !dy || !dw || !geom_ok(B, H, W, Cin, Ho, Wo, Cout, ksize) || stride <= 0 || ldy < Cout || ldy % 8) return SSD_ERR_VALUE;
    if (!ws || ws_bytes < ssd_conv2d_bwd_weight_workspace_bytes(B, Ho, Wo, Cin, Cout, ldy, ksize)) return SSD_ERR_WORKSPACE;
    ConvGeom g = make_geom(B, H, W, Cin, Ho, Wo, ldy, ksize, ksize, stride, 1, pad_t, pad_l);
    const long long ktot = g.ldw;
    if (wgrad_first_layer(H, W, Ho, Wo, Cin, Cout, ldy, ksize, stride, pad_t, pad_l)) {
        const int tx = (Wo + 15) / 16, ty = (Ho + 15) / 16, ntiles = B * tx * ty;
        const int ns = ntiles < 512 ? ntiles : 512;
        const int tps = (ntiles + ns - 1) / ns;
        SSD_PLAN(SSD_PLAN_WG_FIRST | ((ntiles + tps - 1) / tps >= 32 ? SSD_PLAN_F_REDUCE_WIDE : 0));
        float* slab_w = static_cast<float*>(ws);
        float* slab_b = slab_w + (size_t)ns * ldy * ktot;
        hipStream_t s = (hipStream_t)stream;
        static OnceLds set; if (ensure_lds(set, reinterpret_cast<const void*>(k_conv0_wgrad), (int)(2 * W0_BUF)) != 0) return SSD_ERR_LAUNCH;
        hipLaunchKernelGGL(k_conv0_wgrad, dim3((unsigned)((ntiles + tps - 1) / tps)), dim3(512), 2 * W0_BUF, s,
                           static_cast<const bf16_raw*>(x), static_cast<const bf16_raw*>(dy), slab_w, dbias ? slab_b : nullptr, g,
                           tx, ty, tps, Cout);
        if (hipGetLastError() != hipSuccess) return SSD_ERR_LAUNCH;
        const int nsr = (ntiles + tps - 1) / tps;
        launch_wgrad_reduce(s, slab_w, (long long)ldy * ktot, (long long)Cout * ktot, dw, slab_b, (long long)ldy, Cout, dbias, nsr);
        return ssd_launch_status();
    }
    if (wgrad_use_patch(H, W, Ho, Wo, Cin, ksize, stride, pad_t, pad_l) &&
        (long long)B * H * W * Cin * 2 < (1ll << 32) - 16 && (long long)B * Ho * Wo * ldy * 2 < (1ll << 32) - 16) {
        int tx, ty, tps, ns;
        wgrad_patch_plan(B, Ho, Wo, Cin, Cout, &tx, &ty, &tps, &ns);
        float* slab_w = static_cast<float*>(ws);
        float* slab_b = slab_w + (size_t)ns * ldy * ktot;
        hipStream_t s = (hipStream_t)stream;
        const int single = 0;
        const int groups = (Cin / 64) * ((Cout + 63) / 64), nunits = groups * ns;
        int xg = 1;
        for (int d = groups; d >= 1; --d) {
            if (groups % d) continue;
            const int ngr = (nunits + d - 1) / d;
            const int load = ((ngr + 7) / 8) * d, fair = (nunits + 7) / 8;
            if (load * 100 <= fair * 107) { xg = d; break; }
        }
        if (!knob("SSD_WGRAD_PATCH_XCD", 1)) xg = 1;
        const unsigned grid = (unsigned)(8 * xg * ((nunits + 8 * xg - 1) / (8 * xg)));
        int bh, bw;
        const int shape = wgrad_patch_shape(Ho, Wo, &bh, &bw);
        SSD_PLAN((shape == 1 ? SSD_PLAN_WG_PATCH_6x40 : (shape == 2 ? SSD_PLAN_WG_PATCH_10x24 : SSD_PLAN_WG_PATCH_16x16)) |
                 (ns >= 32 ? SSD_PLAN_F_REDUCE_WIDE : 0));
#define SSD_LAUNCH_WP(BH_, BW8_)                                                                                    \
        do {                                                                                                        \
            using G_ = WpGeom<BH_, BW8_>;                                                                           \
            auto kern_ = k_conv3x3_wgrad_patch<BH_, BW8_>;                                                          \
            static OnceLds set_; if (ensure_lds(set_, reinterpret_cast<const void*>(kern_), (int)(2 * G_::BUF)) != 0) return SSD_ERR_LAUNCH; \
            hipLaunchKernelGGL(kern_, dim3(grid), dim3(512), (size_t)(single ? 1 : 2) * G_::BUF, s,                  \
                               static_cast<const bf16_raw*>(x), static_cast<const bf16_raw*>(dy), slab_w,          \
                               dbias ? slab_b : nullptr, g, tx, ty, tps, ns, Cout, single, xg);                     \
        } while (0)
        if (shape == 1) SSD_LAUNCH_WP(6, 5);
        else if (shape == 2) SSD_LAUNCH_WP(10, 3);
        else SSD_LAUNCH_WP(16, 2);
#undef SSD_LAUNCH_WP
        if (hipGetLastError() != hipSuccess) return SSD_ERR_LAUNCH;
        launch_wgrad_reduce(s, slab_w, (long long)ldy * ktot, (long long)Cout * ktot, dw, slab_b, (long long)ldy, Cout, dbias, ns);
        return ssd_launch_status();
    }
    if (wgrad_use_tile(g.M, Cout, ldy, ktot, (long long)B * H * W * Cin)) {
        const int ctiles = (int)((ktot + 255) / 256), mtiles = (Cout + 255) / 256;
        const int ns = wgrad_tile_splits(g.M, ctiles * mtiles, (long long)ldy * ktot);
        int mps = (int)(((long long)g.M + ns - 1) / ns);
        mps = (mps + 63) / 64 * 64;
        SSD_PLAN(SSD_PLAN_WG_TILE | (ns >= 32 ? SSD_PLAN_F_REDUCE_WIDE : 0));
        float* slab_w = static_cast<float*>(ws);
        float* slab_b = slab_w + (size_t)ns * ldy * ktot;
        hipStream_t s = (hipStream_t)stream;
if (knob("SSD_WGTILE_STAGES", 4) == 4) {
            static OnceLds set; if (ensure_lds(set, reinterpret_cast<const void*>(k_conv_wgrad_tile<4>), (int)(4 * WT_TILE)) != 0) return SSD_ERR_LAUNCH;
            hipLaunchKernelGGL(k_conv_wgrad_tile<4>, dim3(ctiles * mtiles * ns), dim3(512), 4 * WT_TILE, s,
                           static_cast<const bf16_raw*>(x), static_cast<const bf16_raw*>(dy), slab_w, dbias ? slab_b : nullptr, g,
                           mps, ns, Cout);
        } else {
            static OnceLds set; if (ensure_lds(set, reinterpret_cast<const void*>(k_conv_wgrad_tile<2>), (int)(4 * WT_TILE)) != 0) return SSD_ERR_LAUNCH;
            hipLaunchKernelGGL(k_conv_wgrad_tile<2>, dim3(ctiles * mtiles * ns), dim3(512), 4 * WT_TILE, s,
                           static_cast<const bf16_raw*>(x), static_cast<const bf16_raw*>(dy), slab_w, dbias ? slab_b : nullptr, g,
                           mps, ns, Cout);
        }
        if (hipGetLastError() != hipSuccess) return SSD_ERR_LAUNCH;
        launch_wgrad_reduce(s, slab_w, (long long)ldy * ktot, (long long)Cout * ktot, dw, slab_b, (long long)ldy, Cout, dbias, ns);
        return ssd_launch_status();
    }
    int bmo, bnc;
    wgrad_tiles(Cout, ktot, &bmo, &bnc);
    const int ctiles = (int)((ktot + bnc - 1) / bnc), mtiles = (Cout + bmo - 1) / bmo;
    const int ns = wgrad_splits(g.M, ctiles * mtiles);
    int mps = (int)(((long long)g.M + ns - 1) / ns);
    mps = (mps + 63) / 64 * 64;
    SSD_PLAN(SSD_PLAN_WG_GENERIC | (ns >= 32 ? SSD_PLAN_F_REDUCE_WIDE : 0));
    float* slab_w = static_cast<float*>(ws);
    float* slab_b = slab_w + (size_t)ns * ldy * ktot;
    hipStream_t s = (hipStream_t)stream;
    const bf16_raw* xp = static_cast<const bf16_raw*>(x);
    const bf16_raw* dyp = static_cast<const bf16_raw*>(dy);
    float* sb = dbias ? slab_b : nullptr;
    {
        const size_t lds = 4 * 64 * WG_LD;
        static OnceLds attr_set; if (ensure_lds(attr_set, reinterpret_cast<const void*>(k_conv_wgrad), (int)((int)lds)) != 0) return SSD_ERR_LAUNCH;
        hipLaunchKernelGGL(k_conv_wgrad, dim3(ctiles, mtiles, ns), dim3(WG), lds, s, xp, dyp, slab_w, sb, g, mps);
    }
    if (hipGetLastError() != hipSuccess) return SSD_ERR_LAUNCH;
    launch_wgrad_reduce(s, slab_w, (long long)ldy * ktot, (long long)Cout * ktot, dw, slab_b, (long long)ldy, Cout, dbias, ns);
    return ssd_launch_status();
}

size_t ssd_conv2d_bwd_weight_batched_workspace_bytes(const ssd_wgrad_item* items, int count) {
    if (!items || count <= 0) return 0;
    size_t tot = 0;
    for (int i = 0; i < count; ++i)
        tot += ssd_align_up(ssd_conv2d_bwd_weight_workspace_bytes(items[i].B, items[i].Ho, items[i].Wo, items[i].Cin, items[i].Cout,
                                                                   items[i].ldy, items[i].ksize), 256);
    return tot;
}

int ssd_conv2d_bwd_weight_batched(const ssd_wgrad_item* items, int count, void* ws, size_t ws_bytes, void* stream) {
    if (!items || count <= 0) return SSD_ERR_VALUE;
    if (count > WGB_MAX) return SSD_ERR_UNSUPPORTED;
    if (!ws || ws_bytes < ssd_conv2d_bwd_weight_batched_workspace_bytes(items, count)) return SSD_ERR_WORKSPACE;
    WgradBatchArgs wa;
    ReduceBatchArgs ra;
    wa.count = ra.count = count;
    char* p = static_cast<char*>(ws);
    int blk = 0, rblk = 0;
    for (int i = 0; i < count; ++i) {
        const ssd_wgrad_item& it = items[i];
        if (!it.x || !it.dy || !it.dw || !geom_ok(it.B, it.H, it.W, it.Cin, it.Ho, it.Wo, it.Cout, it.ksize) || it.stride <= 0 ||
            it.ldy < it.Cout || it.ldy % 8)
            return SSD_ERR_VALUE;
        const ConvGeom g = make_geom(it.B, it.H, it.W, it.Cin, it.Ho, it.Wo, it.ldy, it.ksize, it.ksize, it.stride, 1, it.pad_t, it.pad_l);
        const long long ktot = g.ldw;
        if (wgrad_first_layer(it.H, it.W, it.Ho, it.Wo, it.Cin, it.Cout, it.ldy, it.ksize, it.stride, it.pad_t, it.pad_l) ||
            wgrad_use_patch(it.H, it.W, it.Ho, it.Wo, it.Cin, it.ksize, it.stride, it.pad_t, it.pad_l) ||
            wgrad_use_tile(g.M, it.Cout, it.ldy, ktot, (long long)it.B * it.H * it.W * it.Cin))
            return SSD_ERR_UNSUPPORTED;
        int bmo, bnc;
        wgrad_tiles(it.Cout, ktot, &bmo, &bnc);
        const int ctiles = (int)((ktot + bnc - 1) / bnc), mtiles = (it.Cout + bmo - 1) / bmo;
        const int ns = wgrad_splits(g.M, ctiles * mtiles);
        if (ns >= 32) return SSD_ERR_UNSUPPORTED;
        int mps = (int)(((long long)g.M + ns - 1) / ns);
        mps = (mps + 63) / 64 * 64;
        float* slab_w = reinterpret_cast<float*>(p);
        float* slab_b = slab_w + (size_t)ns * it.ldy * ktot;
        p += ssd_align_up(ssd_conv2d_bwd_weight_workspace_bytes(it.B, it.Ho, it.Wo, it.Cin, it.Cout, it.ldy, it.ksize), 256);
        wa.it[i] = WgradBatchItem{static_cast<const bf16_raw*>(it.x), static_cast<const bf16_raw*>(it.dy), slab_w,
                                  it.dbias ? slab_b : nullptr, g, mps, ctiles, mtiles, blk};
        blk += ctiles * mtiles * ns;
        const long long nw = (long long)it.Cout * ktot;
        const unsigned nbw = (unsigned)((nw / 4 + 255) / 256), nbb = it.dbias ? (unsigned)((it.Cout + 255) / 256) : 0u;
        ra.it[i] = ReduceBatchItem{slab_w, slab_b, it.dw, it.dbias, (long long)it.ldy * ktot, nw, (long long)it.ldy, it.Cout, ns, rblk, nbw};
        rblk += (int)(nbw + nbb);
    }
    for (int i = count; i < WGB_MAX; ++i) { wa.it[i] = wa.it[0]; wa.it[i].blk0 = blk; ra.it[i] = ra.it[0]; ra.it[i].blk0 = rblk; }
    hipStream_t s = (hipStream_t)stream;
    const size_t lds = 4 * 64 * WG_LD;
    static OnceLds attr_set; if (ensure_lds(attr_set, reinterpret_cast<const void*>(k_conv_wgrad_batched), (int)lds) != 0) return SSD_ERR_LAUNCH;
    hipLaunchKernelGGL(k_conv_wgrad_batched, dim3(blk), dim3(WG), lds, s, wa);
    if (hipGetLastError() != hipSuccess) return SSD_ERR_LAUNCH;
    hipLaunchKernelGGL(k_wgrad_reduce2_batched, dim3(rblk), dim3(256), 0, s, ra);
    return ssd_launch_status();
}

int ssd_conv2d_bwd_weight(const void* x, const void* dy, float* dw, float* dbias, int B, int H, int W, int Cin, int Cout,
                          int ldy, int ksize, int stride, int pad_t, int pad_l, int Ho, int Wo, void* ws, size_t ws_bytes,
                          void* stream) {
    return conv2d_bwd_weight_impl(x, dy, dw, dbias, B, H, W, Cin, Cout, ldy, ksize, stride, pad_t, pad_l, Ho, Wo, ws, ws_bytes,
                                  stream, nullptr);
}

static void* const PLAN_PTR = reinterpret_cast<void*>(static_cast<uintptr_t>(64));

int ssd_conv2d_fwd_plan(int B, int H, int W, int Cin, int Cout, int ksize, int stride, int pad_t, int pad_l, int Ho, int Wo,
                        int pool, size_t ws_bytes) {
    int plan = 0, rc;
    void* ws = ws_bytes ? PLAN_PTR : nullptr;
    if (pool) {
        const int Hp = (Ho + 1) / 2, Wp = (Wo + 1) / 2;
        rc = conv2d_fwd_pool_impl(PLAN_PTR, PLAN_PTR, nullptr, pool == 2 ? nullptr : PLAN_PTR, PLAN_PTR, PLAN_PTR, B, H, W, Cin, Cout,
                                  ksize, stride, pad_t, pad_l, Ho, Wo, 1, Hp, Wp, ws, ws_bytes, nullptr, &plan);
    } else {
        rc = conv2d_fwd_impl(PLAN_PTR, PLAN_PTR, nullptr, PLAN_PTR, B, H, W, Cin, Cout, ksize, stride, pad_t, pad_l, Ho, Wo, 1, ws,
                             ws_bytes, nullptr, &plan);
    }
    return rc != SSD_OK ? rc : plan;
}

int ssd_conv2d_head_fwd_plan(int B, int H, int W, int Cin, int per_cell, int classes, size_t ws_bytes) {
    int plan = 0;
    const int rc = conv2d_head_fwd_impl(PLAN_PTR, PLAN_PTR, nullptr, PLAN_PTR, PLAN_PTR, B, H, W, Cin, per_cell, classes,
                                        H * W * per_cell, 0, ws_bytes ? PLAN_PTR : nullptr, ws_bytes, nullptr, &plan);
    return rc != SSD_OK ? rc : plan;
}

int ssd_conv2d_bwd_data_plan(int B, int H, int W, int Cin, int Cout_pad, int ksize, int stride, int pad_t, int pad_l, int Ho,
                             int Wo, int accumulate, size_t ws_bytes) {
    int plan = 0;
    const int rc = conv2d_bwd_data_impl(PLAN_PTR, PLAN_PTR, nullptr, PLAN_PTR, B, H, W, Cin, Cout_pad, ksize, stride, pad_t, pad_l,
                                        Ho, Wo, accumulate, ws_bytes ? PLAN_PTR : nullptr, ws_bytes, nullptr, &plan);
    return rc != SSD_OK ? rc : plan;
}

int ssd_conv2d_bwd_weight_plan(int B, int H, int W, int Cin, int Cout, int ldy, int ksize, int stride, int pad_t, int pad_l,
                               int Ho, int Wo) {
    int plan = 0;
    const size_t need = ssd_conv2d_bwd_weight_workspace_bytes(B, Ho, Wo, Cin, Cout, ldy, ksize);
    const int rc = conv2d_bwd_weight_impl(PLAN_PTR, PLAN_PTR, reinterpret_cast<float*>(PLAN_PTR), reinterpret_cast<float*>(PLAN_PTR),
                                          B, H, W, Cin, Cout, ldy, ksize, stride, pad_t, pad_l, Ho, Wo, PLAN_PTR, need, nullptr,
                                          &plan);
    return rc != SSD_OK ? rc : plan;
}

const char* ssd_conv_plan_name(int plan) {
    switch (plan & SSD_PLAN_KERNEL_MASK) {
        case SSD_PLAN_C64B: return "k_conv3x3_c64b";
        case SSD_PLAN_P32_64: return "k_conv3x3_patch32<64>";
        case SSD_PLAN_P32_128: return "k_conv3x3_patch32<128>";
        case SSD_PLAN_P512: return "k_conv3x3_p512";
        case SSD_PLAN_8PH: return "k_conv_igemm_8ph";
        case SSD_PLAN_PW: return "k_pw_gemm";
        case SSD_PLAN_DMA_256_256: return "k_conv_igemm_dma<256,256>";
        case SSD_PLAN_DMA_256_128: return "k_conv_igemm_dma<256,128>";
        case SSD_PLAN_DMA_256_64: return "k_conv_igemm_dma<256,64>";
        case SSD_PLAN_DMA_128_64: return "k_conv_igemm_dma<128,64>";
        case SSD_PLAN_DMA_128_128: return "k_conv_igemm_dma<128,128>";
        case SSD_PLAN_CONV0_FWD: return "k_conv0_fwd";
        case SSD_PLAN_WG_FIRST: return "k_conv0_wgrad";
        case SSD_PLAN_WG_PATCH_16x16: return "k_conv3x3_wgrad_patch<16,2>";
        case SSD_PLAN_WG_PATCH_6x40: return "k_conv3x3_wgrad_patch<6,5>";
        case SSD_PLAN_WG_PATCH_10x24: return "k_conv3x3_wgrad_patch<10,3>";
        case SSD_PLAN_WG_TILE: return "k_conv_wgrad_tile";
        case SSD_PLAN_WG_GENERIC: return "k_conv_wgrad";
        default: return "?";
    }
}

int ssd_weight_transpose(const void* w, void* w_t, int Cout, int ksize, int Cin, int Cout_pad, void* stream) {
    if (!w || !w_t || Cout <= 0 || ksize <= 0 || Cin <= 0 || Cout_pad < Cout || Cout_pad % 8) return SSD_ERR_VALUE;
    const long long total = (long long)Cin * ksize * ksize * Cout_pad;
    hipLaunchKernelGGL(k_weight_transpose, dim3((unsigned)((total + 255) / 256)), dim3(256), 0, (hipStream_t)stream,
                       static_cast<const bf16_raw*>(w), static_cast<bf16_raw*>(w_t), Cout, ksize, ksize, Cin, Cout_pad);
    return ssd_launch_status();
}

int ssd_weight_transpose_batched(const long long* desc, int ntensors, int max_tiles, void* stream) {
    if (!desc || ntensors <= 0 || max_tiles <= 0) return SSD_ERR_VALUE;
    hipLaunchKernelGGL(k_weight_transpose_batched, dim3((unsigned)max_tiles, (unsigned)ntensors), dim3(256), 0, (hipStream_t)stream, desc);
    return ssd_launch_status();
}

int ssd_cast_bf16(const float* src, void* dst, long long n, void* stream) {
    if (n < 0 || (n > 0 && (!src || !dst))) return SSD_ERR_VALUE;
    if (n == 0) return SSD_OK;
    hipLaunchKernelGGL(k_cast_bf16, dim3((unsigned)((n + 255) / 256)), dim3(256), 0, (hipStream_t)stream, src,
                       static_cast<bf16_raw*>(dst), n);
    return ssd_launch_status();
}

int ssd_image_prep(const float* img, void* out, int B, int H, int W, int normalize, void* stream) {
    if (!img || !out || B <= 0 || H <= 0 || W <= 0) return SSD_ERR_VALUE;
    const long long npix = (long long)B * H * W;
    hipLaunchKernelGGL(k_image_prep, dim3((unsigned)((npix + 255) / 256)), dim3(256), 0, (hipStream_t)stream, img,
                       static_cast<bf16_raw*>(out), npix, normalize);
    return ssd_launch_status();
}

int ssd_maxpool2x2_fwd(const void* x, void* y, int B, int H, int W, int C, int Ho, int Wo, void* stream) {
    if (!x || !y || B <= 0 || C <= 0 || C % 8) return SSD_ERR_VALUE;
    if ((Ho != H / 2 && Ho != (H + 1) / 2) || (Wo != W / 2 && Wo != (W + 1) / 2) || Ho <= 0 || Wo <= 0) return SSD_ERR_VALUE;
    const long long total = (long long)B * Ho * Wo * (C / 8);
    hipLaunchKernelGGL(k_maxpool_fwd, dim3((unsigned)((total + 255) / 256)), dim3(256), 0, (hipStream_t)stream,
                       static_cast<const bf16_raw*>(x), static_cast<bf16_raw*>(y), B, H, W, C, Ho, Wo);
    return ssd_launch_status();
}

int ssd_maxpool2x2_fwd_argmax(const void* x, void* y, void* code, int B, int H, int W, int C, int Ho, int Wo, void* stream) {
    if (!x || !y || !code || B <= 0 || C <= 0 || C % 8) return SSD_ERR_VALUE;
    if ((Ho != H / 2 && Ho != (H + 1) / 2) || (Wo != W / 2 && Wo != (W + 1) / 2) || Ho <= 0 || Wo <= 0) return SSD_ERR_VALUE;
    const long long total = (long long)B * Ho * Wo * (C / 8);
    hipLaunchKernelGGL(k_maxpool_fwd_argmax, dim3((unsigned)((total + 255) / 256)), dim3(256), 0, (hipStream_t)stream,
                       static_cast<const bf16_raw*>(x), static_cast<bf16_raw*>(y), static_cast<unsigned*>(code), B, H, W, C, Ho, Wo);
    return ssd_launch_status();
}

int ssd_maxpool2x2_bwd_argmax(const void* code, const void* dy, void* dx, int B, int H, int W, int C, int Ho, int Wo,
                              void* stream) {
    if (!code || !dy || !dx || B <= 0 || C <= 0 || C % 8 || Ho <= 0 || Wo <= 0) return SSD_ERR_VALUE;
    if (2 * Ho < H || 2 * Wo < W) {
        if (hipMemsetAsync(dx, 0, (size_t)B * H * W * C * 2, (hipStream_t)stream) != hipSuccess) return SSD_ERR_LAUNCH;
    }
    const long long total = (long long)B * Ho * Wo * (C / 8);
    hipLaunchKernelGGL(k_maxpool_bwd_argmax, dim3((unsigned)((total + 255) / 256)), dim3(256), 0, (hipStream_t)stream,
                       static_cast<const unsigned*>(code), static_cast<const bf16_raw*>(dy), static_cast<bf16_raw*>(dx), B, H, W, C,
                       Ho, Wo);
    return ssd_launch_status();
}

int ssd_maxpool2x2_bwd(const void* x, const void* y, const void* dy, void* dx, int B, int H, int W, int C, int Ho, int Wo,
                       void* stream) {
    if (!x || !y || !dy || !dx || B <= 0 || C % 8) return SSD_ERR_VALUE;
    if (2 * Ho < H || 2 * Wo < W) {
        if (hipMemsetAsync(dx, 0, (size_t)B * H * W * C * 2, (hipStream_t)stream) != hipSuccess) return SSD_ERR_LAUNCH;
    }
    const long long total = (long long)B * Ho * Wo * (C / 8);
    hipLaunchKernelGGL(k_maxpool_bwd, dim3((unsigned)((total + 255) / 256)), dim3(256), 0, (hipStream_t)stream,
                       static_cast<const bf16_raw*>(x), static_cast<const bf16_raw*>(y), static_cast<const bf16_raw*>(dy),
                       static_cast<bf16_raw*>(dx), B, H, W, C, Ho, Wo);
    return ssd_launch_status();
}

int ssd_head_grad_pack(const void* dloc, const void* dconf, void* out, int B, int hw, int per_cell, int classes, int npad,
                       int anchors_total, int level_off, void* stream) {
    if (!dloc || !dconf || !out || B <= 0 || hw <= 0 || npad < per_cell * (4 + classes) || npad % 8) return SSD_ERR_VALUE;
    const long long total = (long long)B * hw * (npad / 8);
    hipLaunchKernelGGL(k_head_grad_pack, dim3((unsigned)((total + 255) / 256)), dim3(256), 0, (hipStream_t)stream,
                       static_cast<const bf16_raw*>(dloc), static_cast<const bf16_raw*>(dconf), static_cast<bf16_raw*>(out),
                       B, hw, per_cell, classes, npad, anchors_total, level_off);
    return ssd_launch_status();
}

}
```

### ssd-object-detection_amd/engine.py

```python
import ctypes
import math
import os

import numpy as np
import torch

from . import _lib, ops

SSD300_TRUNK = [
    ("conv", 8, 64, 3, 1, "same", False),
    ("conv", 64, 64, 3, 1, "same", False),
    ("pool", 64, 64, 2, 2, "valid", False),
    ("conv", 64, 128, 3, 1, "same", False),
    ("conv", 128, 128, 3, 1, "same", False),
    ("pool", 128, 128, 2, 2, "valid", False),
    ("conv", 128, 256, 3, 1, "same", False),
    ("conv", 256, 256, 3, 1, "same", False),
    ("conv", 256, 256, 3, 1, "same", False),
    ("pool", 256, 256, 2, 2, "same", False),
    ("conv", 256, 512, 3, 1, "same", False),
    ("conv", 512, 512, 3, 1, "same", False),
    ("conv", 512, 512, 1, 1, "same", True),
    ("conv", 512, 1024, 3, 2, "same", False),
    ("conv", 1024, 1024, 1, 1, "same", True),
    ("conv", 1024, 256, 1, 1, "same", False),
    ("conv", 256, 512, 3, 2, "same", True),
    ("conv", 512, 128, 1, 1, "same", False),
    ("conv", 128, 256, 3, 2, "same", True),
    ("conv", 256, 128, 1, 1, "same", False),
    ("conv", 128, 256, 3, 1, "valid", True),
    ("conv", 256, 128, 1, 1, "same", False),
    ("conv", 128, 256, 3, 1, "valid", True),
]
SSD300_NUM_PRIORS = (4, 6, 6, 6, 4, 4)
IMAGE_CHANNELS = 3

SSD512_TRUNK = SSD300_TRUNK[:13] + [
    ("conv", 512, 1024, 3, 2, "same", False),
    ("conv", 1024, 1024, 1, 1, "same", True),
    ("conv", 1024, 256, 1, 1, "same", False),
    ("conv", 256, 512, 3, 2, "same", True),
    ("conv", 512, 128, 1, 1, "same", False),
    ("conv", 128, 256, 3, 2, "same", True),
    ("conv", 256, 128, 1, 1, "same", False),
    ("conv", 128, 256, 3, 2, "same", True),
    ("conv", 256, 128, 1, 1, "same", False),
    ("conv", 128, 256, 3, 2, "same", True),
    ("conv", 256, 128, 1, 1, "same", False),
    ("conv", 128, 256, 3, 2, "same", True),
]
SSD512_NUM_PRIORS = (4, 6, 6, 6, 6, 4, 4)


def _mx_conv(nd):
    return (nd["kind"] == "conv" and nd["cin"] % 128 == 0 and nd["cout"] % 32 == 0 and nd["k"] in (1, 3)
            and nd["stride"] in (1, 2))


def mxfp8_vgg_plan(nodes, chain_start):
    n = len(nodes)
    end = n if chain_start is None else chain_start

    def pools_itself(i):
        return (_mx_conv(nodes[i]) and nodes[i]["k"] == 3 and nodes[i]["stride"] == 1 and i + 1 < end
                and nodes[i + 1]["kind"] == "pool")

    s = end
    while s > 1 and (_mx_conv(nodes[s - 1]) or (nodes[s - 1]["kind"] == "pool" and pools_itself(s - 2))):
        s -= 1
    size = [nd["hout"] ** 2 * nd["cout"] for nd in nodes]
    start = None
    for i in range(s, end):
        out = size[i + 1] if pools_itself(i) else size[i]
        if nodes[i]["kind"] == "conv" and size[i - 1] < out:
            start = i
            break
    assert start is not None, "no layer of this trunk can run in fp8 behind a quantise cheaper than its own store"
    fp8 = {i for i in range(start, end) if nodes[i]["kind"] == "conv"}
    pooled = {i + 1 for i in fp8 if pools_itself(i)}
    quant = {start - 1}
    writes = {i: set() for i in range(n)}
    for i, nd in enumerate(nodes):
        if nd["feature"]:
            writes[i].add("bf16")
        if i > 0 and i not in pooled:
            writes[i - 1].add("fp8" if i in fp8 else "bf16")
    writes[start - 1].add("bf16")
    for i, w in writes.items():
        assert w or (i in fp8 and i + 1 in pooled), "node %d has no consumer" % i
        if "fp8" in w:
            assert i in fp8 or i in pooled or i in quant, "node %d would need a standalone activation quantise" % i
    assert all(i - 1 in fp8 for i in pooled)
    return fp8, pooled, quant, {i: frozenset(w) for i, w in writes.items()}


class ParamTensor:

    def __init__(self, name, shape, offset, index, block0, nblocks):
        self.name, self.shape, self.offset, self.index = name, tuple(shape), offset, index
        self.numel = int(np.prod(shape))
        self.block0, self.nblocks = block0, nblocks


class FusedView:

    def __init__(self, name, shape, parts):
        self.name, self.shape, self.parts = name, tuple(shape), tuple(parts)
        self.offset, self.index = parts[0].offset, parts[0].index
        self.numel = int(np.prod(shape))
        assert parts[1].offset == parts[0].offset + parts[0].numel and self.numel == parts[0].numel + parts[1].numel
        self.indices = [p.index for p in parts]


class SSDEngine:
    def __init__(self, classes=81, in_size=300, trunk=SSD300_TRUNK, num_priors=SSD300_NUM_PRIORS, device="cuda",
                 seed=0, sparse_heads=None):
        self.L = _lib.lib()
        self.classes, self.in_size, self.device = classes, in_size, torch.device(device)
        self.trunk, self.num_priors = list(trunk), tuple(num_priors)
        self.block = self.L.ssd_opt_block_elems()
        self.sparse_heads = (os.environ.get("SSD_SPARSE_HEADS", "1") == "1") if sparse_heads is None else bool(sparse_heads)
        self.chain = {"1": {"fwd", "bwd"}, "fwd": {"fwd"}, "bwd": {"bwd"}}.get(os.environ.get("SSD_CHAIN", "1"), set())
        self._plan_shapes()
        self._plan_params()
        self._alloc_params()
        self.init_params(seed)
        self._act_cache = {}
        self._ws = ops.MatchWorkspace()
        self._ws_hz = ops.MatchWorkspace()
        self._ws_hw = ops.MatchWorkspace()
        self._side = None
        self.overlap_heads = os.environ.get("SSD_OVERLAP_HEADS", "1") != "0" and self.device.type == "cuda"
        self.step_count = 0
        self.skip_fullres = os.environ.get("SSD_SKIP_FULLRES", "1") == "1"
        self.tail_stream = os.environ.get("SSD_TAIL_STREAM", "1") == "1"
        self.big_heads_side = os.environ.get("SSD_BIG_HEADS_SIDE", "1") == "1"
        self.pack_side = os.environ.get("SSD_PACK_SIDE", "1") == "1"
        self.side_streams = int(os.environ.get("SSD_SIDE_STREAMS", "1"))
        self.reduce_stream = os.environ.get("SSD_REDUCE_STREAM", "0") == "1"
        self.batch_chain_wgrads = os.environ.get("SSD_BATCH_CHAIN_WGRADS", "1") == "1"
        self.batch_chain_front = os.environ.get("SSD_BATCH_CHAIN_FRONT", "0") == "1"
        self.wgrad_group = int(os.environ.get("SSD_WGRAD_GROUP", "3"))
        self.wgrad_on_main = set(int(v) for v in os.environ.get("SSD_WGRAD_ON_MAIN", "").split(",") if v.strip())
        self.split_heads_dgrad = int(os.environ.get("SSD_SPLIT_HEADS_DGRAD", "2"))
        self.chain_heads_split = os.environ.get("SSD_CHAIN_HEADS_SPLIT", "1") == "1"
        self.chain_prefetch = os.environ.get("SSD_CHAIN_PREFETCH", "1") == "1"
        self.prezero_maps = os.environ.get("SSD_PREZERO_MAPS", "0") == "1"
        self._prezeroed = set()
        self.opt_defer = int(os.environ.get("SSD_OPT_DEFER", "4"))
        self.opt_defer_heads = int(os.environ.get("SSD_OPT_DEFER_HEADS", "0"))
        self.pool_only = {}
        self.fuse_unpool = {} if os.environ.get("SSD_FUSE_UNPOOL", "1") == "1" else None
        self.relu_bits = {} if os.environ.get("SSD_RELU_BITS", "1") == "1" else None
        self.bits_valid = set()
        self.fuse_first = os.environ.get("SSD_FUSE_FIRST", "1") == "1"
        self.wgrad_probe = None
        self._vgg_mx, self._vgg_mx_range, self._vgg_mx_w = None, None, None
        self._vgg_fp8_fwd = False

    def _plan_shapes(self):
        s = self.in_size
        self.nodes = []
        self.fm = []
        for kind, cin, cout, k, stride, mode, feat in self.trunk:
            if mode == "same":
                ho, pt = ops.same_pad(s, k, stride)
            else:
                ho, pt = ops.valid_out(s, k, stride), 0
            self.nodes.append(dict(kind=kind, cin=cin, cout=cout, k=k, stride=stride, pt=pt, pl=pt, hin=s, hout=ho,
                                   feature=feat, same=(mode == "same")))
            s = ho
            if feat:
                self.fm.append((len(self.nodes) - 1, ho, cout))
        assert len(self.fm) == len(self.num_priors)
        j = len(self.nodes)
        while (j > 1 and len(self.nodes) - j < _lib.SSD_CHAIN_MAX_LAYERS and self.nodes[j - 1]["kind"] == "conv"
               and self.nodes[j - 2]["kind"] == "conv" and self.nodes[j - 1]["hin"] ** 2 <= 112 and self.nodes[j - 1]["hout"] ** 2 <= 112
               and self.nodes[j - 1]["cin"] % 128 == 0 and self.nodes[j - 1]["cout"] % 128 == 0):
            j -= 1
        self.chain_start = j if len(self.nodes) - j >= 2 else None
        if any(c % 128 for _, _, c in self.fm) or len(self.fm) > _lib.SSD_MAX_LEVELS:
            self.sparse_heads = False
        self.level_off = [0]
        for (_, h, _), n in zip(self.fm, self.num_priors):
            self.level_off.append(self.level_off[-1] + h * h * n)
        self.A = self.level_off[-1]
        self.grids = tuple((h, h) for _, h, _ in self.fm)

    def _plan_params(self):
        self.tensors = []
        off = 0

        def add(name, shape, end_aligned=False):
            nonlocal off
            numel = int(np.prod(shape))
            nb = (numel + self.block - 1) // self.block
            start = off + (nb * self.block - numel if end_aligned else 0)
            if start % 8:
                raise ValueError("%s: %d elements do not end-align on a 16-byte boundary (per-cell anchor counts must make "
                                 "n*4 a multiple of 8, i.e. even: the reference's are 4 and 6)" % (name, numel))
            t = ParamTensor(name, shape, start, len(self.tensors), off // self.block, nb)
            self.tensors.append(t)
            off += nb * self.block
            return t

        self.conv_params = {}
        for i, nd in enumerate(self.nodes):
            if nd["kind"] != "conv":
                continue
            self.conv_params[i] = (add("conv%d/kernel" % i, (nd["cout"], nd["k"], nd["k"], nd["cin"])),
                                   add("conv%d/bias" % i, (nd["cout"],)))
        self.head_params = []
        for lvl, ((_, h, c), n) in enumerate(zip(self.fm, self.num_priors)):
            nl, nc = n * 4, n * self.classes
            lk, ck = add("head%d/loc_kernel" % lvl, (nl, 3, 3, c), True), add("head%d/conf_kernel" % lvl, (nc, 3, 3, c))
            lb, cb = add("head%d/loc_bias" % lvl, (nl,), True), add("head%d/conf_bias" % lvl, (nc,))
            self.head_params.append((FusedView("head%d/kernel" % lvl, (nl + nc, 3, 3, c), (lk, ck)),
                                     FusedView("head%d/bias" % lvl, (nl + nc,), (lb, cb))))
        self.n_flat = off
        self.n_params = sum(t.numel for t in self.tensors)

    def _alloc_params(self):
        dev, n = self.device, self.n_flat
        self.param = torch.zeros(n, dtype=torch.float32, device=dev)
        self.grad = torch.zeros(n, dtype=torch.float32, device=dev)
        self.grad_acc = None
        self.adam_m = torch.zeros(n, dtype=torch.float32, device=dev)
        self.adam_v = torch.zeros(n, dtype=torch.float32, device=dev)
        self.param_bf16 = torch.zeros(n, dtype=torch.bfloat16, device=dev)
        nb = n // self.block
        tbo = np.zeros(len(self.tensors) + 1, np.int32)
        bt = np.zeros(nb, np.int32)
        for i, t in enumerate(self.tensors):
            b0, b1 = t.block0, t.block0 + t.nblocks
            tbo[i], tbo[i + 1] = b0, b1
            bt[b0:b1] = i
        self.tensor_block_off = torch.from_numpy(tbo).to(dev)
        self.block_tensor = torch.from_numpy(bt).to(dev)
        self.sq_partial = torch.empty(nb, dtype=torch.float64, device=dev)
        self.clip_scale = torch.empty(len(self.tensors), dtype=torch.float32, device=dev)
        self.grad_norms = torch.empty(len(self.tensors), dtype=torch.float32, device=dev)
        self.w_t = {}
        for i, nd in enumerate(self.nodes):
            if nd["kind"] == "conv" and i > 0:
                self.w_t[i] = torch.empty((nd["cin"], nd["k"], nd["k"], nd["cout"]), dtype=torch.bfloat16, device=dev)
        self.chain_pk_fwd, self.chain_pk_bwd = {}, {}
        if getattr(self, "chain_start", None) is not None and self.chain:
            for i in range(self.chain_start, len(self.nodes)):
                nd = self.nodes[i]
                self.chain_pk_fwd[i] = torch.empty((nd["cout"], nd["k"], nd["k"], nd["cin"]), dtype=torch.bfloat16, device=dev)
                self.chain_pk_bwd[i] = torch.empty_like(self.w_t[i])
        self.head_npad = [(n * (4 + self.classes) + 7) // 8 * 8 for n in self.num_priors]
        self.head_w_t = [torch.empty((3, 3, c, npad) if self.sparse_heads else (c, 3, 3, npad), dtype=torch.bfloat16, device=dev)
                         for (_, _, c), npad in zip(self.fm, self.head_npad)]

    def view(self, t, buf):
        return buf[t.offset:t.offset + t.numel].view(t.shape)

    def init_params(self, seed=0):
        rng = np.random.default_rng(seed)
        host = np.zeros(self.n_flat, np.float32)
        for t in self.tensors:
            if not t.name.endswith("kernel"):
                continue
            cout, k, _, cin = t.shape
            if t.name.startswith("head"):
                lim = math.sqrt(6.0 / (k * k * cin + k * k * cout))
                w = rng.uniform(-lim, lim, (cout, k, k, cin))
            else:
                real_cin = IMAGE_CHANNELS if t.name == "conv0/kernel" else cin
                lim = math.sqrt(6.0 / (k * k * real_cin + k * k * cout))
                w = rng.uniform(-lim, lim, (cout, k, k, cin))
                if real_cin != cin:
                    w[..., real_cin:] = 0.0
            host[t.offset:t.offset + t.numel] = w.astype(np.float32).reshape(-1)
        self.param.copy_(torch.from_numpy(host))
        self.adam_m.zero_()
        self.adam_v.zero_()
        self.step_count = 0
        self.refresh_weights(cast=True)

    def refresh_weights(self, cast=False, tensors=None):
        if cast:
            ops.cast_bf16(self.param, self.param_bf16)
        if getattr(self, "_tr_desc", None) is None:
            rows, tiles = [], 0
            pairs = [(self.conv_params[i][0], wt) for i, wt in self.w_t.items()]
            n_trunk = len(pairs)
            pairs += [(self.head_params[lvl][0], wt) for lvl, wt in enumerate(self.head_w_t)]
            for r, (pt, wt) in enumerate(pairs):
                cout, k, _, cin = pt.shape
                cpad = wt.shape[-1]
                kfield = k | (0x100 if (self.sparse_heads and r >= n_trunk) else 0)
                rows.append([self.view(pt, self.param_bf16).data_ptr(), wt.data_ptr(), cout, kfield, cin, cpad])
                tiles = max(tiles, ((cpad + 31) // 32) * ((cin + 31) // 32) * k * k)
            self._tr_desc = torch.tensor(rows, dtype=torch.int64, device=self.device)
            self._tr_tiles = tiles
            self._tr_tensor = [pt.index for pt, _ in pairs]
        r0, r1 = 0, self._tr_desc.shape[0]
        if tensors is not None:
            inside = [r for r, t in enumerate(self._tr_tensor) if tensors[0] <= t < tensors[1]]
            if not inside:
                return
            r0, r1 = inside[0], inside[-1] + 1
            assert inside == list(range(r0, r1))
        _lib.check(self.L.ssd_weight_transpose_batched(ops._ptr(self._tr_desc[r0:]), r1 - r0, self._tr_tiles,
                                                       ops._stream()))
        if self.chain_pk_fwd:
# ... 422 lines not shown

        if side is not None and self.chain_start is not None and "bwd" in self.chain and self.chain_prefetch:
            if getattr(self, "_tail", None) is None:
                self._tail = torch.cuda.Stream(device=self.device)
                self._ws_tail = ops.MatchWorkspace()
            ev = torch.cuda.Event()
            ev.record(main)
            with torch.cuda.stream(self._tail):
                self._tail.wait_event(ev)
                ops.chain_prefetch([self.chain_pk_bwd[j] for j in range(self.chain_start, len(self.nodes))])
            prefetch_done = torch.cuda.Event()
            prefetch_done.record(self._tail)
        else:
            prefetch_done = None
        sparse_head_done = {}
        if heads is not None:
            hl, keep = self._head_layers(c)
            on_side(lambda ws: ops.heads_bwd_weight_sparse(heads, hl, ws=self._ws_hw),
                    [i for wt, bt in self.head_params for t in (wt, bt) for i in t.indices], now=True)
            big_lv = [lvl for lvl, (ni, h, ch) in enumerate(self.fm) if B * h * h >= 16384]
            small_lv = [lvl for lvl in range(len(self.fm)) if lvl not in big_lv]
            if side is not None and self.split_heads_dgrad and big_lv and small_lv:
                ops.heads_bwd_data_sparse(heads, hl, ws=self._ws_hz, levels=small_lv)
                if getattr(self, "_tail", None) is None:
                    self._tail = torch.cuda.Stream(device=self.device)
                    self._ws_tail = ops.MatchWorkspace()
                ev = torch.cuda.Event()
                ev.record(main)
                with torch.cuda.stream(self._tail):
                    self._tail.wait_event(ev)
                    pz = all(self.fm[lvl][0] + 1 in self._prezeroed for lvl in big_lv)
                    self._prezeroed = set()
                    if self.split_heads_dgrad == 2:
                        for lvl in reversed(big_lv):
                            ops.heads_bwd_data_sparse(heads, hl, ws=self._ws_hz, levels=[lvl], prezeroed=pz)
                            done = torch.cuda.Event()
                            done.record(self._tail)
                            sparse_head_done[self.fm[lvl][0] + 1] = done
                    else:
                        ops.heads_bwd_data_sparse(heads, hl, ws=self._ws_hz, levels=big_lv, prezeroed=pz)
                        done = torch.cuda.Event()
                        done.record(self._tail)
                        for lvl in big_lv:
                            sparse_head_done[self.fm[lvl][0] + 1] = done
            else:
                ops.heads_bwd_data_sparse(heads, hl, ws=self._ws_hz)
            for ni, _, _ in self.fm:
                written[ni + 1] = True
            del keep
        big = [lvl for lvl, (ni, h, ch) in enumerate(self.fm) if heads is None and side is not None and B * h * h >= 16384
               and self.big_heads_side]
        head_done = {}
        packed = [None] * len(self.fm)

        def pack(lvl):
            h = self.fm[lvl][1]
            packed[lvl] = ops.head_grad_pack(dloc, dconf, h * h, self.num_priors[lvl], self.classes, self.head_npad[lvl],
                                             self.level_off[lvl], out=c["packed"][lvl]).view(B, h, h, self.head_npad[lvl])

        pack_side = self.pack_side
        for lvl in range(len(self.fm) if heads is None else 0):
            if lvl not in big or not pack_side:
                pack(lvl)

        def masked_dgrad(key, dy, w_t, a, stride, pt, pl, accumulate, ws):
            if self.relu_bits is not None and a in self.bits_valid and self.relu_bits.get(key, True):
                try:
                    ops.conv2d_bwd_data_bits(dy, w_t, c["rbits"][a], acts[a].shape, stride, pt, pl, accumulate=accumulate,
                                             out=gacts[a], ws=ws)
                    self.relu_bits[key] = True
                    return
                except NotImplementedError:
                    self.relu_bits[key] = False
            ops.conv2d_bwd_data(dy, w_t, acts[a], acts[a].shape, stride, pt, pl, accumulate=accumulate, out=gacts[a], ws=ws)

        def head_dgrad(lvl, ws):
            ni = self.fm[lvl][0]
            masked_dgrad("head%d" % lvl, packed[lvl], self.head_w_t[lvl], ni + 1, 1, 1, 1, False, ws)
            written[ni + 1] = True

        def head_wgrad(lvl, ws):
            ni = self.fm[lvl][0]
            wt, bt = self.head_params[lvl]
            ops.conv2d_bwd_weight(acts[ni + 1], packed[lvl], wt.shape[0], 3, 1, 1, 1, dw=self.view(wt, self.grad),
                                  dbias=self.view(bt, self.grad), ws=ws)

        if big:
            ev = torch.cuda.Event()
            ev.record(main)
            with torch.cuda.stream(side):
                side.wait_event(ev)
                for lvl in reversed(big):
                    if pack_side:
                        pack(lvl)
                    head_dgrad(lvl, self._ws_side)
                    done = torch.cuda.Event()
                    done.record(side)
                    head_done[self.fm[lvl][0] + 1] = done
                for lvl in reversed(big):
                    head_wgrad(lvl, self._ws_side)
                    if on_ready:
                        on_ready([i for t in self.head_params[lvl] for i in t.indices])
        for lvl in range(len(self.fm) if heads is None else 0):
            if lvl in big:
                continue
            on_side(lambda ws, lvl=lvl: head_wgrad(lvl, ws), [i for t in self.head_params[lvl] for i in t.indices], now=True)
            head_dgrad(lvl, self._ws)
        opt_bucket(None)
        unpooled = set()
        first_fused = False
        chained = set()
        if self.chain_start is not None and "bwd" in self.chain:
            last = len(self.nodes) - 1
            assert written[last + 1]
            layers = []
            for j in range(last, self.chain_start - 1, -1):
                ndj = self.nodes[j]
                use_bits = self.relu_bits is not None and j in self.bits_valid
                layers.append(ops.chain_layer_dgrad(self.w_t[j], self.chain_pk_bwd[j], gacts[j], ndj["stride"], ndj["pt"], ndj["pl"], accumulate=written[j],
                                                    mask_bits=c["rbits"][j] if use_bits else None,
                                                    mask_src=None if use_bits else acts[j]))
            try:
                for j in range(last, self.chain_start - 1, -1):
                    for done in (head_done, sparse_head_done):
                        if j in done:
                            main.wait_event(done.pop(j))
                ops.conv_chain(gacts[last + 1], layers)
                chained = set(range(self.chain_start, last + 1))
                for j in chained:
                    written[j] = True
            except NotImplementedError:
                self.chain = self.chain - {"bwd"}
        batched_w = set()
        if chained and side is not None and self.batch_chain_wgrads and side2 is None and red is None and self.wgrad_probe is None:
            extra = [self.chain_start - 1] if (self.batch_chain_front and self.nodes[self.chain_start - 1]["kind"] == "conv") else []
            for front in (extra, []):
                order = sorted(chained, reverse=True) + front
                layers, tens = [], []
                for j in order:
                    ndj = self.nodes[j]
                    wt, bt = self.conv_params[j]
                    layers.append((acts[j], gacts[j + 1], ndj["cout"], ndj["k"], ndj["stride"], ndj["pt"], ndj["pl"],
                                   self.view(wt, self.grad), self.view(bt, self.grad)))
                    tens += [wt.index, bt.index]
                try:
                    on_side(lambda ws: ops.conv2d_bwd_weight_batched(layers, ws=ws), tens, now=True)
                    batched_w = set(order)
                    break
                except NotImplementedError:
                    if front:
                        self.batch_chain_front = False
                    else:
                        self.batch_chain_wgrads = False
        for i in range(len(self.nodes) - 1, -1, -1):
            nd = self.nodes[i]
            g_out = gacts[i + 1]
            assert written[i + 1]
            if nd["kind"] == "pool":
                assert not written[i], "a pooled activation cannot also feed a head (the pool gradient overwrites)"
                if i not in unpooled:
                    ops.maxpool2x2_bwd_argmax(c["pool_code"][i], g_out, acts[i].shape, out=gacts[i])
                written[i] = True
                continue
            wt, bt = self.conv_params[i]
            if i == 0 and first_fused:
                on_side(lambda ws: None, [wt.index, bt.index])
                opt_bucket(i)
                continue
            def wgrad(ws, i=i, a=acts[i], go=g_out, nd=nd, wt=wt, bt=bt):
                probe = self.wgrad_probe
                timed = probe is not None and i in probe["nodes"]
                if timed:
                    e0, e1 = torch.cuda.Event(enable_timing=True), torch.cuda.Event(enable_timing=True)
                    e0.record()
                ops.conv2d_bwd_weight(a, go, nd["cout"], nd["k"], nd["stride"], nd["pt"], nd["pl"], dw=self.view(wt, self.grad),
                                      dbias=self.view(bt, self.grad), ws=ws)
                if timed:
                    e1.record()
                    probe["events"].append((i, e0, e1))
            if i in batched_w:
                pass
            elif side is not None and i in self.wgrad_on_main:
                wgrad(self._ws)
                if on_ready:
                    on_ready([wt.index, bt.index])
            else:
                on_side(wgrad, [wt.index, bt.index])
            if i == 0 or i in chained:
                opt_bucket(i)
                continue
            if (i == 1 and self.fuse_first and not written[1] and self.nodes[0]["kind"] == "conv" and self.nodes[0]["cin"] == 8
                    and self.nodes[0]["cout"] == 64 and nd["cin"] == 64 and nd["cout"] == 64 and nd["k"] == 3 and nd["stride"] == 1
                    and nd["pt"] == 1 and nd["pl"] == 1 and self.nodes[0]["k"] == 3 and self.nodes[0]["stride"] == 1
                    and self.relu_bits is not None and 1 in self.bits_valid):
                wt0, bt0 = self.conv_params[0]
                try:
                    ops.conv2d_bwd_data_wgrad_first(g_out, self.w_t[1], c["rbits"][1], acts[0], dw=self.view(wt0, self.grad),
                                                    dbias=self.view(bt0, self.grad), ws=self._ws)
                    first_fused = True
                    written[1] = True
                    opt_bucket(i)
                    continue
                except NotImplementedError:
                    self.fuse_first = False
            prev_is_relu_conv = self.nodes[i - 1]["kind"] == "conv"
            if i in head_done:
                main.wait_event(head_done.pop(i))
            if i in sparse_head_done:
                main.wait_event(sparse_head_done.pop(i))
            fused = False
            if (self.fuse_unpool is not None and self.fuse_unpool.get(i, True) and self.nodes[i - 1]["kind"] == "pool" and not written[i] and not written[i - 1]
                    and nd["k"] == 3 and nd["stride"] == 1 and nd["pt"] == 1 and nd["pl"] == 1):
                try:
                    ops.conv2d_bwd_data_unpool(g_out, self.w_t[i], None, c["pool_code"][i - 1], tuple(gacts[i - 1].shape),
                                               out=gacts[i - 1], ws=self._ws)
                    fused = True
                    unpooled.add(i - 1)
                except NotImplementedError:
                    pass
                self.fuse_unpool[i] = fused
            if not fused and prev_is_relu_conv:
                masked_dgrad("conv%d" % i, g_out, self.w_t[i], i, nd["stride"], nd["pt"], nd["pl"], written[i], self._ws)
            elif not fused:
                ops.conv2d_bwd_data(g_out, self.w_t[i], None, acts[i].shape, nd["stride"], nd["pt"], nd["pl"],
                                    accumulate=written[i], out=gacts[i], ws=self._ws)
            written[i] = True
            opt_bucket(i)
        assert not opt_at
        flush_side()
        if prefetch_done is not None:
            main.wait_event(prefetch_done)
        for ev in sparse_head_done.values():
            main.wait_event(ev)
        for t0, t1, ev, ev2 in deferred:
            main.wait_event(ev)
            if ev2 is not None:
                main.wait_event(ev2)
            self.adam_range(t0, t1, lr_t, hp["beta1"], hp["beta2"], hp["eps"], hp["clip"])
        if side is not None:
            main.wait_stream(side)
            if side2 is not None:
                main.wait_stream(side2)
            if red is not None:
                main.wait_stream(red)
                _lib.check(self.L.ssd_set_wgrad_reduce_stream(None))
                self._red_active = None

    def clip_scales(self, clip=0.01):
        _lib.check(self.L.ssd_grad_clip_scales(ops._ptr(self.grad), self.n_flat, ops._ptr(self.tensor_block_off),
                                               len(self.tensors), float(clip), ops._ptr(self.sq_partial),
                                               ops._ptr(self.clip_scale), ops._ptr(self.grad_norms), ops._stream()))

    def apply_clip_in_place(self):
        _lib.check(self.L.ssd_grad_apply_scale(ops._ptr(self.grad), self.n_flat, ops._ptr(self.block_tensor),
                                               ops._ptr(self.clip_scale), ops._stream()))

    def _range_table(self, t0, t1):
        key = (t0, t1)
        if not hasattr(self, "_range_tables"):
            self._range_tables = {}
        tab = self._range_tables.get(key)
        if tab is None:
            b0 = self.tensors[t0].block0
            tbo = (self.tensor_block_off[t0:t1 + 1] - b0).contiguous()
            bt = (self.block_tensor[b0:int(self.tensor_block_off[t1].item())] - t0).contiguous()
            tab = (b0, tbo, bt)
            self._range_tables[key] = tab
        return tab

    def opt_buckets(self, min_elems=2_000_000):
        if getattr(self, "_opt_buckets", None) is None:
            first_head = self.head_params[0][0].index
            out = [(first_head, len(self.tensors), None)]
            hi, acc = first_head, 0
            conv_nodes = sorted(self.conv_params)
            for i in reversed(conv_nodes):
                wt, bt = self.conv_params[i]
                acc += wt.numel + bt.numel
                if acc >= min_elems or i == conv_nodes[0]:
                    out.append((wt.index, hi, i))
                    hi, acc = wt.index, 0
            self._opt_buckets = out
        return self._opt_buckets

    def adam_range(self, t0, t1, lr_t, beta1, beta2, eps, clip, grad_scale=1.0):
        b0, tbo, bt = self._range_table(t0, t1)
        start, n = b0 * self.block, bt.numel() * self.block
        sl = slice(start, start + n)
        if clip is not None:
            _lib.check(self.L.ssd_grad_clip_scales(ops._ptr(self.grad[sl]), n, ops._ptr(tbo), t1 - t0, float(clip),
                                                   ops._ptr(self.sq_partial[b0:]), ops._ptr(self.clip_scale[t0:]),
                                                   ops._ptr(self.grad_norms[t0:]), ops._stream()))
        _lib.check(self.L.ssd_adam_step(ops._ptr(self.param[sl]), ops._ptr(self.grad[sl]), ops._ptr(self.adam_m[sl]),
                                        ops._ptr(self.adam_v[sl]), ops._ptr(self.param_bf16[sl]), n, ops._ptr(bt),
                                        ops._ptr(self.clip_scale[t0:]) if clip is not None else None, float(grad_scale),
                                        float(lr_t), float(beta1), float(beta2), float(eps), ops._stream()))
        self.refresh_weights(tensors=(t0, t1))

    def clip_range_in_place(self, t0, t1, clip=0.01):
        b0, tbo, bt = self._range_table(t0, t1)
        start = b0 * self.block
        n = bt.numel() * self.block
        g = self.grad[start:start + n]
        _lib.check(self.L.ssd_grad_clip_scales(ops._ptr(g), n, ops._ptr(tbo), t1 - t0, float(clip),
                                               ops._ptr(self.sq_partial[b0:]), ops._ptr(self.clip_scale[t0:]),
                                               ops._ptr(self.grad_norms[t0:]), ops._stream()))
        _lib.check(self.L.ssd_grad_apply_scale(ops._ptr(g), n, ops._ptr(bt), ops._ptr(self.clip_scale[t0:]), ops._stream()))

    def accumulate_clipped(self, first):
        if self.grad_acc is None:
            self.grad_acc = torch.empty_like(self.grad)
        _lib.check(self.L.ssd_grad_accumulate(ops._ptr(self.grad_acc), ops._ptr(self.grad), self.n_flat,
                                              ops._ptr(self.block_tensor), ops._ptr(self.clip_scale), 1 if first else 0,
                                              ops._stream()))

    def adam(self, lr, grad, grad_scale=1.0, use_clip_scale=False, beta1=0.9, beta2=0.999, eps=1e-7):
        self.step_count += 1
        t = self.step_count
        lr_t = lr * math.sqrt(1.0 - beta2 ** t) / (1.0 - beta1 ** t)
        _lib.check(self.L.ssd_adam_step(ops._ptr(self.param), ops._ptr(grad), ops._ptr(self.adam_m), ops._ptr(self.adam_v),
                                        ops._ptr(self.param_bf16), self.n_flat, ops._ptr(self.block_tensor),
                                        ops._ptr(self.clip_scale) if use_clip_scale else None, float(grad_scale),
                                        float(lr_t), float(beta1), float(beta2), float(eps), ops._stream()))
        self.refresh_weights()

    def sgd(self, lr, grad, grad_scale=1.0, use_clip_scale=False):
        self.step_count += 1
        _lib.check(self.L.ssd_sgd_step(ops._ptr(self.param), ops._ptr(grad), ops._ptr(self.param_bf16), self.n_flat,
                                       ops._ptr(self.block_tensor), ops._ptr(self.clip_scale) if use_clip_scale else None,
                                       float(grad_scale), float(lr), ops._stream()))
        self.refresh_weights()

    LAYOUT_VERSION = 2

    def state_dict(self):
        return dict(param=self.param.cpu(), adam_m=self.adam_m.cpu(), adam_v=self.adam_v.cpu(), step=self.step_count,
                    names=[t.name for t in self.tensors], shapes=[t.shape for t in self.tensors],
                    offsets=[t.offset for t in self.tensors], layout_version=self.LAYOUT_VERSION)

    def load_state_dict(self, sd):
        mine = ([t.name for t in self.tensors], [tuple(t.shape) for t in self.tensors], [t.offset for t in self.tensors])
        theirs = (list(sd.get("names", [])), [tuple(x) for x in sd.get("shapes", [])], list(sd.get("offsets", [])))
        if sd.get("layout_version", 1) != self.LAYOUT_VERSION or mine != theirs or sd["param"].numel() != self.n_flat:
            bad = [n for n in mine[0] if n not in theirs[0]][:3] + [n for n in theirs[0] if n not in mine[0]][:3]
            raise ValueError("checkpoint parameter layout (version %s, %d variables, %d elements) does not match this engine's "
                             "(version %d, %d variables, %d elements)%s" % (
                                 sd.get("layout_version", 1), len(theirs[0]), sd["param"].numel(), self.LAYOUT_VERSION,
                                 len(mine[0]), self.n_flat, "; e.g. " + ", ".join(bad) if bad else ""))
        self.param.copy_(sd["param"])
        self.adam_m.copy_(sd["adam_m"])
        self.adam_v.copy_(sd["adam_v"])
        self.step_count = int(sd["step"])
        self.refresh_weights(cast=True)
```

### ssd-object-detection_amd/ops.py

```python
import ctypes

import numpy as np
import torch

from . import _lib

SSD300_GRIDS = ((38, 38), (19, 19), (10, 10), (5, 5), (3, 3), (1, 1))
SSD300_S_REF = (21, 45, 99, 153, 207, 261, 315)
SSD300_RATIOS = ((2,), (2, 3), (2, 3), (2, 3), (2,), (2,))


def _ptr(t):
    return ctypes.c_void_p(t.data_ptr()) if t is not None else ctypes.c_void_p(0)


def _stream():
    return ctypes.c_void_p(torch.cuda.current_stream().cuda_stream)


def _dev(t, dtype):
    assert t.is_cuda and t.dtype == dtype and t.is_contiguous(), (t.device, t.dtype, t.is_contiguous())
    return t


# ... 359 lines not shown
def conv2d_head_fwd(x, w, bias, loc, conf, per_cell, classes, level_off, ws=None):
    L = _lib.lib()
    _bf(x); _bf(w); _bf(loc); _bf(conf)
    B, H, W, Cin = x.shape
    A = loc.shape[1]
    assert w.shape == (per_cell * (4 + classes), 3, 3, Cin)
    wbuf = _splitk_ws(ws)
    _lib.check(L.ssd_conv2d_head_fwd(_ptr(x), _ptr(w), _ptr(bias), _ptr(loc), _ptr(conf), B, H, W, Cin, per_cell,
                                     classes, A, level_off, _ptr(wbuf), wbuf.numel(), _stream()))


def weight_transpose(w, cout_pad=None, out=None):
    L = _lib.lib()
    _bf(w)
    Cout, k, _, Cin = w.shape
    cout_pad = cout_pad or (Cout + 7) // 8 * 8
    if out is None:
        out = torch.empty((Cin, k, k, cout_pad), dtype=torch.bfloat16, device=w.device)
    _lib.check(L.ssd_weight_transpose(_ptr(w), _ptr(out), Cout, k, Cin, cout_pad, _stream()))
    return out


def conv2d_bwd_data(dy, w_t, relu_src, x_shape, stride, pad_t, pad_l, accumulate=False, out=None, ws=None):
    L = _lib.lib()
    _bf(dy); _bf(w_t)
    B, H, W, Cin = x_shape
    _, Ho, Wo, cpad = dy.shape
    k = w_t.shape[1]
    assert w_t.shape == (Cin, k, k, cpad)
    if out is None:
        assert not accumulate
        out = torch.empty(x_shape, dtype=torch.bfloat16, device=dy.device)
    wbuf = _splitk_ws(ws)
    _lib.check(L.ssd_conv2d_bwd_data(_ptr(dy), _ptr(w_t), _ptr(relu_src), _ptr(out), B, H, W, Cin, cpad, k, stride,
                                     pad_t, pad_l, Ho, Wo, 1 if accumulate else 0, _ptr(wbuf), wbuf.numel(), _stream()))
    return out


def chain_pack_weights(pairs):
    L = _lib.lib()
    out = []
    for i0 in range(0, len(pairs), _lib.SSD_CHAIN_PACK_MAX):
        chunk = pairs[i0:i0 + _lib.SSD_CHAIN_PACK_MAX]
        arr = (_lib.ChainPack * len(chunk))()
        for d, (w, packed) in zip(arr, chunk):
            _bf(w)
            if packed is None:
                packed = torch.empty_like(w)
            _bf(packed)
            assert packed.numel() == w.numel()
            d.src, d.dst, d.N, d.K = _ptr(w), _ptr(packed), w.shape[0], w.numel() // w.shape[0]
            out.append(packed)
        _lib.check(L.ssd_chain_pack_weights(arr, len(chunk), _stream()))
    return out


def chain_prefetch(packed_list):
    L = _lib.lib()
    arr = (_lib.ChainPack * len(packed_list))()
    for d, t in zip(arr, packed_list):
        _bf(t)
        d.src, d.dst, d.N, d.K = None, _ptr(t), t.shape[0], t.numel() // t.shape[0]
    _lib.check(L.ssd_chain_prefetch(arr, len(packed_list), _stream()))


def chain_layer_fwd(w, packed, bias, out, stride, pad_t, pad_l, relu=True, relu_bits=None):
    return dict(w=packed, bias=bias, out=out, ksize=w.shape[1], mul=stride, div=1, pad_t=pad_t, pad_l=pad_l, relu=relu,
                relu_bits=relu_bits, Kc=w.shape[3], N=w.shape[0])


def chain_layer_dgrad(w_t, packed, out, stride, pad_t, pad_l, accumulate=False, mask_bits=None, mask_src=None):
    k = w_t.shape[1]
    return dict(w=packed, bias=None, out=out, ksize=k, mul=1, div=stride, pad_t=k - 1 - pad_t, pad_l=k - 1 - pad_l, relu=False,
                accumulate=accumulate, mask_bits=mask_bits, mask_src=mask_src, Kc=w_t.shape[3], N=w_t.shape[0])


def conv_chain(in0, layers):
    L = _lib.lib()
    _bf(in0)
    B, Hi, Wi, Kc = in0.shape
    arr = (_lib.ChainLayer * len(layers))()
    for d, s in zip(arr, layers):
        out = s["out"]
        _bf(s["w"]); _bf(out)
        assert out.shape[0] == B and out.shape[3] == s["N"] and s["Kc"] == Kc, (tuple(out.shape), s["N"], s["Kc"], Kc)
        d.w, d.bias, d.out = _ptr(s["w"]), _ptr(s.get("bias")), _ptr(out)
        d.mask_bits, d.mask_src, d.relu_bits = _ptr(s.get("mask_bits")), _ptr(s.get("mask_src")), _ptr(s.get("relu_bits"))
        d.Hi, d.Wi, d.Kc, d.Ho, d.Wo, d.N = Hi, Wi, Kc, out.shape[1], out.shape[2], s["N"]
        d.ksize, d.mul, d.div, d.pad_t, d.pad_l = s["ksize"], s["mul"], s["div"], s["pad_t"], s["pad_l"]
        d.relu, d.accumulate = int(bool(s.get("relu"))), int(bool(s.get("accumulate")))
        Hi, Wi, Kc = out.shape[1], out.shape[2], s["N"]
    rc = L.ssd_conv_chain(_ptr(in0), arr, len(layers), B, _stream())
    if rc == _lib.SSD_ERR_UNSUPPORTED:
        raise NotImplementedError("ssd_conv_chain does not serve these layers")
    _lib.check(rc)


def conv2d_fwd_relubits(x, w, bias, stride, pad_t, pad_l, Ho, Wo, bits, out=None, ws=None):
    L = _lib.lib()
    _bf(x); _bf(w)
    B, H, W, Cin = x.shape
    Cout, k = w.shape[0], w.shape[1]
    assert bits.dtype == torch.uint8 and bits.shape == (B, Ho, Wo, Cout // 8) and bits.is_contiguous()
    if out is None:
        out = torch.empty((B, Ho, Wo, Cout), dtype=torch.bfloat16, device=x.device)
    wbuf = _splitk_ws(ws)
    rc = L.ssd_conv2d_fwd_relubits(_ptr(x), _ptr(w), _ptr(bias), _ptr(out), _ptr(bits), B, H, W, Cin, Cout, k, stride, pad_t, pad_l,
                                   Ho, Wo, _ptr(wbuf), wbuf.numel(), _stream())
    if rc == _lib.SSD_ERR_UNSUPPORTED:
        raise NotImplementedError("this layer's kernel does not write sign bits")
    _lib.check(rc)
    return out


def conv2d_bwd_data_bits(dy, w_t, bits, x_shape, stride, pad_t, pad_l, accumulate=False, out=None, ws=None):
    L = _lib.lib()
    _bf(dy); _bf(w_t)
    B, H, W, Cin = x_shape
    _, Ho, Wo, cpad = dy.shape
    k = w_t.shape[1]
    assert w_t.shape == (Cin, k, k, cpad) and bits.dtype == torch.uint8 and bits.shape == (B, H, W, Cin // 8)
    if out is None:
        assert not accumulate
        out = torch.empty(x_shape, dtype=torch.bfloat16, device=dy.device)
    wbuf = _splitk_ws(ws)
    rc = L.ssd_conv2d_bwd_data_bits(_ptr(dy), _ptr(w_t), _ptr(bits), _ptr(out), B, H, W, Cin, cpad, k, stride, pad_t, pad_l, Ho, Wo,
                                    1 if accumulate else 0, _ptr(wbuf), wbuf.numel(), _stream())
    if rc == _lib.SSD_ERR_UNSUPPORTED:
        raise NotImplementedError("this layer's kernel does not read sign bits")
    _lib.check(rc)
    return out


def conv2d_bwd_data_wgrad_first(dy, w_t, bits, image, dw=None, dbias=None, ws=None):
    L = _lib.lib()
    _bf(dy); _bf(w_t); _bf(image)
    B, H, W, c = dy.shape
    assert c == 64 and w_t.shape == (64, 3, 3, 64) and image.shape == (B, H, W, 8)
    assert bits.dtype == torch.uint8 and bits.shape == (B, H, W, 8)
    if dw is None:
        dw = torch.empty((64, 3, 3, 8), dtype=torch.float32, device=dy.device)
    if dbias is None:
        dbias = torch.empty((64,), dtype=torch.float32, device=dy.device)
    assert dw.dtype == torch.float32 and dw.numel() == 64 * 72 and dw.is_contiguous() and dbias.dtype == torch.float32
    wbuf = (ws or _conv_ws).get(L.ssd_conv2d_bwd_data_wgrad_first_workspace_bytes(B, H, W), dy.device)
    rc = L.ssd_conv2d_bwd_data_wgrad_first(_ptr(dy), _ptr(w_t), _ptr(bits), _ptr(image), _ptr(dw), _ptr(dbias), B, H, W, _ptr(wbuf),
                                           wbuf.numel(), _stream())
    if rc == _lib.SSD_ERR_UNSUPPORTED:
        raise NotImplementedError("maps smaller than 16x16 take the two separate calls")
    _lib.check(rc)
    return dw, dbias


def conv2d_bwd_data_unpool(dy, w_t, relu_src, pool_code, full_shape, out=None, ws=None, pooled_out=None):
    L = _lib.lib()
    _bf(dy); _bf(w_t)
    B, Hf, Wf, Cin = full_shape
    _, H, W, cpad = dy.shape
    assert w_t.shape == (Cin, 3, 3, cpad) and pool_code.shape == (B, H, W, Cin // 8) and pool_code.dtype == torch.int32
    if out is None:
        out = torch.empty(full_shape, dtype=torch.bfloat16, device=dy.device)
    wbuf = _splitk_ws(ws)
    if pooled_out is not None:
        _bf(pooled_out)
        assert pooled_out.shape == (B, H, W, Cin)
    rc = L.ssd_conv2d_bwd_data_unpool(_ptr(dy), _ptr(w_t), _ptr(relu_src), _ptr(pool_code), _ptr(pooled_out), _ptr(out), B, H, W, Cin,
                                      cpad, Hf, Wf, _ptr(wbuf), wbuf.numel(), _stream())
    if rc == _lib.SSD_ERR_UNSUPPORTED:
        raise NotImplementedError("no LDS-patch kernel for this layer")
    _lib.check(rc)
    return out


def conv2d_bwd_weight(x, dy, Cout, k, stride, pad_t, pad_l, dw=None, dbias=None, want_bias=True, ws=None):
    L = _lib.lib()
    _bf(x); _bf(dy)
    B, H, W, Cin = x.shape
    _, Ho, Wo, ldy = dy.shape
    if dw is None:
        dw = torch.empty((Cout, k, k, Cin), dtype=torch.float32, device=x.device)
    if dbias is None and want_bias:
        dbias = torch.empty((Cout,), dtype=torch.float32, device=x.device)
    nbytes = L.ssd_conv2d_bwd_weight_workspace_bytes(B, Ho, Wo, Cin, Cout, ldy, k)
    wbuf = (ws or _conv_ws).get(nbytes, x.device)
    _lib.check(L.ssd_conv2d_bwd_weight(_ptr(x), _ptr(dy), _ptr(dw), _ptr(dbias), B, H, W, Cin, Cout, ldy, k, stride,
                                       pad_t, pad_l, Ho, Wo, _ptr(wbuf), wbuf.numel(), _stream()))
    return dw, dbias


def conv2d_bwd_weight_batched(layers, ws=None):
    L = _lib.lib()
    arr = (_lib.WgradItem * len(layers))()
    for d, (x, dy, Cout, k, stride, pad_t, pad_l, dw, dbias) in zip(arr, layers):
        _bf(x); _bf(dy)
        B, H, W, Cin = x.shape
        _, Ho, Wo, ldy = dy.shape
        assert dw.dtype == torch.float32 and dw.shape == (Cout, k, k, Cin) and dw.is_contiguous()
        d.x, d.dy, d.dw, d.dbias = _ptr(x), _ptr(dy), _ptr(dw), _ptr(dbias)
        d.B, d.H, d.W, d.Cin, d.Cout, d.ldy, d.ksize, d.stride, d.pad_t, d.pad_l, d.Ho, d.Wo = B, H, W, Cin, Cout, ldy, k, stride, pad_t, pad_l, Ho, Wo
    nbytes = L.ssd_conv2d_bwd_weight_batched_workspace_bytes(arr, len(layers))
    wbuf = (ws or _conv_ws).get(nbytes, layers[0][0].device)
    rc = L.ssd_conv2d_bwd_weight_batched(arr, len(layers), _ptr(wbuf), wbuf.numel(), _stream())
    if rc == _lib.SSD_ERR_UNSUPPORTED:
        raise NotImplementedError("ssd_conv2d_bwd_weight_batched does not serve these layers")
    _lib.check(rc)


def conv2d_bwd_weight_unpooled(x, dpool, pool_code, dw=None, dbias=None, want_bias=True, ws=None):
    L = _lib.lib()
    _bf(x); _bf(dpool)
    B, H, W, Cin = x.shape
    _, Hp, Wp, Cout = dpool.shape
    assert pool_code.shape == (B, Hp, Wp, Cout // 8) and pool_code.dtype == torch.int32
    if dw is None:
        dw = torch.empty((Cout, 3, 3, Cin), dtype=torch.float32, device=x.device)
    if dbias is None and want_bias:
        dbias = torch.empty((Cout,), dtype=torch.float32, device=x.device)
    nbytes = L.ssd_conv2d_bwd_weight_unpooled_workspace_bytes(B, H, W, Cin, Cout, Hp, Wp)
    if nbytes == 0:
        raise NotImplementedError("no structured-sparse weight-gradient kernel for this layer")
    wbuf = (ws or _conv_ws).get(nbytes, x.device)
    rc = L.ssd_conv2d_bwd_weight_unpooled(_ptr(x), _ptr(dpool), _ptr(pool_code), _ptr(dw), _ptr(dbias), B, H, W, Cin, Cout, Hp, Wp,
                                          _ptr(wbuf), wbuf.numel(), _stream())
    if rc == _lib.SSD_ERR_UNSUPPORTED:
        raise NotImplementedError("no structured-sparse weight-gradient kernel for this layer")
    _lib.check(rc)
    return dw, dbias


def image_resize_prep(src, src_off, src_hw, S=300, normalize=True, out=None):
    L = _lib.lib()
    _dev(src, torch.uint8); _dev(src_off, torch.int64); _dev(src_hw, torch.int32)
    B = src_hw.shape[0]
    if out is None:
        out = torch.empty((B, S, S, 8), dtype=torch.bfloat16, device=src.device)
    _lib.check(L.ssd_image_resize_prep(_ptr(src), _ptr(src_off), _ptr(src_hw), _ptr(out), B, S, 1 if normalize else 0, _stream()))
    return out


def box_prep(box_tlwh, gt_off, src_hw):
    L = _lib.lib()
    _dev(box_tlwh, torch.float32); _dev(gt_off, torch.int32); _dev(src_hw, torch.int32)
    total = box_tlwh.shape[0]
    out = torch.empty_like(box_tlwh)
    _lib.check(L.ssd_box_prep(_ptr(box_tlwh), _ptr(gt_off), _ptr(src_hw), _ptr(out), src_hw.shape[0], total, _stream()))
    return out


def maxpool2x2_fwd(x, same=False):
    L = _lib.lib()
    _bf(x)
    B, H, W, C = x.shape
    Ho, Wo = ((H + 1) // 2, (W + 1) // 2) if same else (H // 2, W // 2)
    y = torch.empty((B, Ho, Wo, C), dtype=torch.bfloat16, device=x.device)
    _lib.check(L.ssd_maxpool2x2_fwd(_ptr(x), _ptr(y), B, H, W, C, Ho, Wo, _stream()))
    return y


def maxpool2x2_fwd_argmax(x, same=False, out=None, code=None):
    L = _lib.lib()
    _bf(x)
    B, H, W, C = x.shape
    Ho, Wo = ((H + 1) // 2, (W + 1) // 2) if same else (H // 2, W // 2)
    if out is None:
        out = torch.empty((B, Ho, Wo, C), dtype=torch.bfloat16, device=x.device)
    if code is None:
        code = torch.empty((B, Ho, Wo, C // 8), dtype=torch.int32, device=x.device)
    _lib.check(L.ssd_maxpool2x2_fwd_argmax(_ptr(x), _ptr(out), _ptr(code), B, H, W, C, Ho, Wo, _stream()))
    return out, code


def maxpool2x2_bwd_argmax(code, dy, x_shape, out=None):
    L = _lib.lib()
    _bf(dy)
    B, H, W, C = x_shape
    _, Ho, Wo, _ = dy.shape
    if out is None:
        out = torch.empty(tuple(x_shape), dtype=torch.bfloat16, device=dy.device)
    _lib.check(L.ssd_maxpool2x2_bwd_argmax(_ptr(code), _ptr(dy), _ptr(out), B, H, W, C, Ho, Wo, _stream()))
    return out


def maxpool2x2_bwd(x, y, dy, out=None):
    L = _lib.lib()
    _bf(x); _bf(y); _bf(dy)
    B, H, W, C = x.shape
    _, Ho, Wo, _ = y.shape
    if out is None:
        out = torch.empty_like(x)
    _lib.check(L.ssd_maxpool2x2_bwd(_ptr(x), _ptr(y), _ptr(dy), _ptr(out), B, H, W, C, Ho, Wo, _stream()))
    return out


def quantize_mx_fp8(x, q=None, scale=None):
    L = _lib.lib()
    _bf(x)
    assert x.shape[-1] % 32 == 0
    if q is None:
        q = torch.empty(x.shape, dtype=torch.uint8, device=x.device)
    if scale is None:
        scale = torch.empty(x.shape[:-1] + (x.shape[-1] // 32,), dtype=torch.uint8, device=x.device)
    assert q.numel() == x.numel() and scale.numel() == x.numel() // 32
    _lib.check(L.ssd_quantize_mx_fp8(_ptr(x), _ptr(q), _ptr(scale), x.numel(), _stream()))
    return q, scale


def dequantize_mx_fp8(q, scale):
    v = q.view(torch.float8_e4m3fn).float()
    s = torch.exp2(scale.float() - 127.0)
    return (v.view(*scale.shape, 32) * s.unsqueeze(-1)).view(q.shape)


def conv3x3_fwd_mxfp8(xq, xs, wq, ws, bias, relu=True, out=None):
    L = _lib.lib()
    B, H, W, Cin = xq.shape
    Cout = wq.shape[0]
    assert wq.shape == (Cout, 3, 3, Cin) and xs.shape == (B, H, W, Cin // 32) and ws.shape == (Cout, 3, 3, Cin // 32)
    for t in (xq, xs, wq, ws):
        _dev(t, torch.uint8)
    if out is None:
        out = torch.empty((B, H, W, Cout), dtype=torch.bfloat16, device=xq.device)
    rc = L.ssd_conv3x3_fwd_mxfp8(_ptr(xq), _ptr(xs), _ptr(wq), _ptr(ws), _ptr(bias), _ptr(out), B, H, W, Cin, Cout, 1 if relu else 0,
                                 _stream())
    if rc == _lib.SSD_ERR_UNSUPPORTED:
        raise NotImplementedError("block-scaled fp8 forward needs Cin % 128 == 0")
    _lib.check(rc)
    return out


def conv2d_fwd_mxfp8(xq, xs, wq, ws, bias, stride, pad_t, pad_l, Ho, Wo, relu, want_bf16=True, want_fp8=False, out=None,
                     out_q=None, out_scale=None):
    L = _lib.lib()
    B, H, W, Cin = xq.shape
    Cout, k = wq.shape[0], wq.shape[1]
    assert want_bf16 or want_fp8
    assert wq.shape == (Cout, k, k, Cin) and xs.shape == (B, H, W, Cin // 32) and ws.shape == (Cout, k, k, Cin // 32)
    for t in (xq, xs, wq, ws):
        _dev(t, torch.uint8)
    if want_bf16 and out is None:
# ... 166 lines not shown
```

Before: 7024 images/sec.

## Consume pooled gradient directly in first-layer dgrad and wgrad kernels

Adds pooled-dY variants of the fused first-layer dgrad+wgrad kernel and of the 16x16 wgrad patch kernel. Each reads the 2x2-pooled gradient plus argmax codes and scatters them into the full-resolution LDS tile, instead of first materialising the unpooled layer-1 gradient. The model's backward pass now routes conv3 dgrad output and the pool codes straight to both layer-1 consumers, with fallback to explicit maxpool backward when unsupported. This removes a full-resolution gradient write and two reads in exchange for extra LDS scatter work and barriers inside the kernels.

Result: no change. 7050 images/sec, median of 6 (+0.4%).

```diff
diff --git a/include/ssd_hip.h b/include/ssd_hip.h
--- a/include/ssd_hip.h
+++ b/include/ssd_hip.h
@@ -100,12 +100,18 @@
 size_t ssd_conv2d_bwd_data_wgrad_first_workspace_bytes(int B, int H, int W);
 int ssd_conv2d_bwd_data_wgrad_first(const void* dy, const void* w_t, const void* relu_bits, const void* image, float* dw0,
                                     float* dbias0, int B, int H, int W, void* ws, size_t ws_bytes, void* stream);
+int ssd_conv2d_bwd_data_wgrad_first_pooled(const void* dy_pooled, const void* pool_code, const void* w_t, const void* relu_bits,
+                                           const void* image, float* dw0, float* dbias0, int B, int H, int W, int Hp, int Wp, void* ws,
+                                           size_t ws_bytes, void* stream);
 int ssd_conv2d_bwd_data_unpool(const void* dy, const void* w_t, const void* relu_src, const void* pool_code, void* dx_pooled,
                                void* dx_full, int B, int H, int W, int Cin, int Cout_pad, int Hf, int Wf, void* ws, size_t ws_bytes,
                                void* stream);
 size_t ssd_conv2d_bwd_weight_unpooled_workspace_bytes(int B, int H, int W, int Cin, int Cout, int Hp, int Wp);
 int ssd_conv2d_bwd_weight_unpooled(const void* x, const void* dpool, const void* pool_code, float* dw, float* dbias, int B, int H,
                                    int W, int Cin, int Cout, int Hp, int Wp, void* ws, size_t ws_bytes, void* stream);
+size_t ssd_conv2d_bwd_weight_pooled_dy_workspace_bytes(int B, int H, int W, int Cin, int Cout);
+int ssd_conv2d_bwd_weight_pooled_dy(const void* x, const void* dy_pooled, const void* pool_code, float* dw, float* dbias, int B, int H,
+                                    int W, int Cin, int Cout, int Hp, int Wp, void* ws, size_t ws_bytes, void* stream);
 size_t ssd_conv2d_bwd_weight_workspace_bytes(int B, int Ho, int Wo, int Cin, int Cout, int ldy, int ksize);
 int ssd_conv2d_bwd_weight(const void* x, const void* dy, float* dw, float* dbias, int B, int H, int W, int Cin,
                           int Cout, int ldy, int ksize, int stride, int pad_t, int pad_l, int Ho, int Wo, void* ws,
diff --git a/ssd-object-detection_amd/_lib.py b/ssd-object-detection_amd/_lib.py
--- a/ssd-object-detection_amd/_lib.py
+++ b/ssd-object-detection_amd/_lib.py
@@ -109,6 +109,9 @@
     "ssd_conv2d_bwd_weight_unpooled": (ctypes.c_int, [VP] * 5 + [ctypes.c_int] * 7 + [VP, ctypes.c_size_t, VP]),
     "ssd_conv2d_bwd_data_wgrad_first_workspace_bytes": (ctypes.c_size_t, [ctypes.c_int] * 3),
     "ssd_conv2d_bwd_data_wgrad_first": (ctypes.c_int, [VP] * 6 + [ctypes.c_int] * 3 + [VP, ctypes.c_size_t, VP]),
+    "ssd_conv2d_bwd_data_wgrad_first_pooled": (ctypes.c_int, [VP] * 7 + [ctypes.c_int] * 5 + [VP, ctypes.c_size_t, VP]),
+    "ssd_conv2d_bwd_weight_pooled_dy_workspace_bytes": (ctypes.c_size_t, [ctypes.c_int] * 5),
+    "ssd_conv2d_bwd_weight_pooled_dy": (ctypes.c_int, [VP] * 5 + [ctypes.c_int] * 7 + [VP, ctypes.c_size_t, VP]),
     "ssd_conv2d_bwd_weight_workspace_bytes": (ctypes.c_size_t, [ctypes.c_int] * 7),
     "ssd_conv2d_bwd_weight": (ctypes.c_int, [VP, VP, VP, VP] + [ctypes.c_int] * 12 + [VP, ctypes.c_size_t, VP]),
     "ssd_weight_transpose": (ctypes.c_int, [VP, VP, ctypes.c_int, ctypes.c_int, ctypes.c_int, ctypes.c_int, VP]),
diff --git a/ssd-object-detection_amd/csrc/conv.hip b/ssd-object-detection_amd/csrc/conv.hip
--- a/ssd-object-detection_amd/csrc/conv.hip
+++ b/ssd-object-detection_amd/csrc/conv.hip
@@ -877,7 +877,11 @@
     const bf16_raw* img;
     float* slab_w;
     float* slab_b;
+    const unsigned* pcode;
+    int hp, wp;
 };
+constexpr int C64B_PDY_CODES = 8 * 1024;
+constexpr int C64B_PDY_PIX = 6 * 10;
 constexpr int C64B_IMG = 6 * 256;
 constexpr int C64B_W0_IMG = 2 * C64B_PATCH;
 constexpr int C64B_W0_SUMS = C64B_W0_IMG + 2 * C64B_IMG;
@@ -889,17 +893,19 @@
     return __builtin_amdgcn_ds_read_tr16_b64_v4i16((lds_s16x4*)p);
 }
 
-template <int EPI, bool W0 = false>
+template <int EPI, bool W0 = false, bool PDY = false>
 __global__ __launch_bounds__(256) __attribute__((amdgpu_waves_per_eu(2, 2)))
 void k_conv3x3_c64b(const bf16_raw* __restrict__ x, const bf16_raw* __restrict__ w, ConvGeom g, Epilogue ep, int tiles_x, int tiles_y,
                     C64W0 w0) {
     static_assert(!W0 || EPI == EPI_DGRAD, "the fused first-layer weight gradient belongs to the data gradient");
+    static_assert(!PDY || W0, "the pooled-operand loader exists for the W0 form");
     extern __shared__ __attribute__((aligned(16))) char smem[];
     const int tid = threadIdx.x, lane = tid & 63;
     const int wave = __builtin_amdgcn_readfirstlane(tid >> 6);
     const int wave_m = wave & 1, wave_n = wave >> 1;
     const int nblocks = g.B * tiles_x * tiles_y;
-    const __amdgpu_buffer_rsrc_t xres = __builtin_amdgcn_make_buffer_rsrc((void*)x, 0, (unsigned)g.B * g.H * g.W * 64u * 2u, 0x00020000);
+    const __amdgpu_buffer_rsrc_t xres = __builtin_amdgcn_make_buffer_rsrc(
+        (void*)x, 0, PDY ? (unsigned)g.B * w0.hp * w0.wp * 64u * 2u : (unsigned)g.B * g.H * g.W * 64u * 2u, 0x00020000);
     constexpr unsigned OOB = 0xfffffff0u;
     constexpr int NJ = (C64B_NDMA + 3) / 4;
     const __amdgpu_buffer_rsrc_t ires = __builtin_amdgcn_make_buffer_rsrc((void*)(W0 ? w0.img : x), 0, (unsigned)g.B * g.H * g.W * 16u, 0x00020000);
@@ -917,8 +923,26 @@
         const int tx = r % tiles_x; r /= tiles_x;
         const int ty = r % tiles_y;
         const int b = r / tiles_y;
-#pragma unroll
-        for (int j = 0; j < NJ; ++j) {
+        if constexpr (PDY) {
+            const __amdgpu_buffer_rsrc_t cres = __builtin_amdgcn_make_buffer_rsrc((void*)w0.pcode, 0, (unsigned)g.B * w0.hp * w0.wp * 32u, 0x00020000);
+#pragma unroll
+            for (int j = 0; j < 3; ++j) {
+                const int i = wave + 4 * j;
+                if (i < 10) {
+                    const int q = (i < 8 ? i : i - 8) * 64 + lane;
+                    const int pp = i < 8 ? q >> 3 : q >> 1;
+                    const int prow = pp / 10, pcol = pp - prow * 10;
+                    const int gy = ty * (C64B_ROWS / 2) - 1 + prow, gx = tx * 8 - 1 + pcol;
+                    const bool ok = pp < C64B_PDY_PIX && (unsigned)gy < (unsigned)w0.hp && (unsigned)gx < (unsigned)w0.wp;
+                    const unsigned pix = (unsigned)((b * w0.hp + gy) * w0.wp + gx);
+                    char* dst = smem + buf * C64B_PATCH + (i < 8 ? i * 1024 : C64B_PDY_CODES + (i - 8) * 1024);
+                    if (i < 8) __builtin_amdgcn_raw_ptr_buffer_load_lds(xres, (lds_void*)dst, 16, ok ? pix * 128u + (unsigned)(q & 7) * 16u : OOB, 0, 0, 0);
+                    else __builtin_amdgcn_raw_ptr_buffer_load_lds(cres, (lds_void*)dst, 16, ok ? pix * 32u + (unsigned)(q & 1) * 16u : OOB, 0, 0, 0);
+                }
+            }
+        }
+#pragma unroll
+        for (int j = 0; j < (PDY ? 0 : NJ); ++j) {
             if (wave + 4 * j < C64B_NDMA) {
                 const int iy = ty * C64B_ROWS - 1 + (pcode[j] >> 16), ix = tx * 16 - 1 + ((pcode[j] >> 8) & 255);
                 const bool ok = pcode[j] >= 0 && (unsigned)iy < (unsigned)g.H && (unsigned)ix < (unsigned)g.W;
@@ -1004,7 +1028,7 @@
         else if (prev_st == 1) asm volatile("s_waitcnt vmcnt(1) lgkmcnt(0)" ::: "memory");
         else asm volatile("s_waitcnt vmcnt(0) lgkmcnt(0)" ::: "memory");
         __syncthreads();
-        __builtin_amdgcn_s_setprio(0);
+        if constexpr (!PDY) __builtin_amdgcn_s_setprio(0);
         int r = t;
         const int tx = r % tiles_x; r /= tiles_x;
         const int ty = r % tiles_y;
@@ -1030,6 +1054,46 @@
         const int tnext = block_of(it + 1);
         if (tnext >= 0 && !(g.ablate & 1)) issue_patch(tnext, cur ^ 1);
         if constexpr (W0) { if (tnext >= 0) load_masks(tnext); }
+        if constexpr (PDY) {
+            char* pbuf = smem + cur * C64B_PATCH;
+            uint4 pv[2];
+            unsigned pc[2];
+#pragma unroll
+            for (int h = 0; h < 2; ++h) {
+                const int q = tid + 256 * h;
+                pv[h] = make_uint4(0u, 0u, 0u, 0u);
+                pc[h] = 0u;
+                if (q < C64B_PDY_PIX * 8) {
+                    pv[h] = lds_ld16_scoped(pbuf + q * 16, smem);
+                    pc[h] = *reinterpret_cast<const unsigned*>(pbuf + C64B_PDY_CODES + q * 4);
+                }
+            }
+            asm volatile("s_waitcnt lgkmcnt(0)" ::: "memory");
+            __builtin_amdgcn_s_barrier();
+#pragma unroll
+            for (int h = 0; h < 2; ++h) {
+                const int q = tid + 256 * h;
+                if (q >= C64B_PDY_PIX * 8) continue;
+                const int pp = q >> 3, c8 = q & 7, prow = pp / 10, pcol = pp - prow * 10;
+                const unsigned v[4] = {pv[h].x, pv[h].y, pv[h].z, pv[h].w};
+#pragma unroll
+                for (int pos = 0; pos < 4; ++pos) {
+                    const int py = 2 * prow + (pos >> 1) - 1, px = 2 * pcol + (pos & 1) - 1;
+                    if (py < 0 || py >= C64B_ROWS + 2 || px < 0 || px >= PATCH_W) continue;
+                    unsigned o[4];
+#pragma unroll
+                    for (int k = 0; k < 4; ++k) {
+                        const unsigned lo = ((pc[h] >> (8 * k)) & 15u) == (unsigned)pos ? 0x0000ffffu : 0u;
+                        const unsigned hi = ((pc[h] >> (8 * k + 4)) & 15u) == (unsigned)pos ? 0xffff0000u : 0u;
+                        o[k] = v[k] & (lo | hi);
+                    }
+                    lds_st16_scoped(pbuf + (py * PATCH_W + px) * C64_PITCH + c8 * 16, smem, make_uint4(o[0], o[1], o[2], o[3]));
+                }
+            }
+            asm volatile("s_waitcnt lgkmcnt(0)" ::: "memory");
+            __builtin_amdgcn_s_barrier();
+            __builtin_amdgcn_s_setprio(0);
+        }
         const int pb = cur * C64B_PATCH + xbase;
         f32x4_t acc[2][4];
 #pragma unroll
@@ -1780,12 +1844,14 @@
 
 __device__ __forceinline__ int wp_key(int px) { return (px >> 1) & 3; }
 
-template <int BH, int BW8>
+template <int BH, int BW8, bool PDY = false>
 __global__ __launch_bounds__(512) void k_conv3x3_wgrad_patch(const bf16_raw* __restrict__ x, const bf16_raw* __restrict__ dy,
                                                              float* __restrict__ slab_w, float* __restrict__ slab_b,
                                                              ConvGeom g, int tiles_x, int tiles_y, int tiles_per_split,
-                                                             int nsplit, int cout, int single_buf, int xg) {
+                                                             int nsplit, int cout, int single_buf, int xg,
+                                                             const unsigned* __restrict__ pcode, int hp, int wp) {
     using G = WpGeom<BH, BW8>;
+    static_assert(!PDY || (BH == 16 && BW8 == 2), "pooled dY: 16x16 blocks (8x8 pooling windows)");
     extern __shared__ __attribute__((aligned(16))) char smem[];
 
     const int tid = threadIdx.x, lane = tid & 63;
@@ -1806,6 +1872,8 @@
     const __amdgpu_buffer_rsrc_t xres = __builtin_amdgcn_make_buffer_rsrc((void*)x, 0, (unsigned)g.B * g.H * g.W * g.C * 2u, 0x00020000);
     const __amdgpu_buffer_rsrc_t dyres = __builtin_amdgcn_make_buffer_rsrc((void*)dy, 0, (unsigned)g.B * g.Ho * g.Wo * g.N * 2u, 0x00020000);
     constexpr unsigned WP_OOB = 0xfffffff0u;
+    uint4 pv[2] = {make_uint4(0u, 0u, 0u, 0u), make_uint4(0u, 0u, 0u, 0u)};
+    unsigned pc[2] = {0u, 0u};
     auto issue_dma = [&](int t, int buf) {
         int r = t;
         const int tx = r % tiles_x; r /= tiles_x;
@@ -1813,8 +1881,22 @@
         const int b = r / tiles_y;
         const int y0 = ty * BH, x0 = tx * G::BW;
         char* base = smem + buf * G::BUF;
-#pragma unroll
-        for (int j = 0; j < G::DY_INSTR / 4; ++j) {
+        if constexpr (PDY) {
+#pragma unroll
+            for (int j = 0; j < 2; ++j) {
+                const int q = (ct * 2 + j) * 64 + lane, c16 = q & 7;
+                const int gy = (y0 >> 1) + (q >> 6), gx = (x0 >> 1) + ((q >> 3) & 7), co = co0 + c16 * 8;
+                pv[j] = make_uint4(0u, 0u, 0u, 0u);
+                pc[j] = 0u;
+                if (gy < hp && gx < wp && co < g.N) {
+                    const long long pix = ((long long)b * hp + gy) * wp + gx;
+                    pv[j] = *reinterpret_cast<const uint4*>(dy + pix * g.N + co);
+                    pc[j] = pcode[pix * (g.N >> 3) + (co >> 3)];
+                }
+            }
+        }
+#pragma unroll
+        for (int j = 0; j < (PDY ? 0 : G::DY_INSTR / 4); ++j) {
             const int i = ct + 4 * j;
             const int kk = 8 * i + (lane >> 3), sl = lane & 7;
             const int c16 = (((sl >> 1) ^ wp_key(kk)) << 1) | (sl & 1);
@@ -1855,7 +1937,32 @@
 #pragma unroll
     for (int i = 0; i < 8; ++i) ones[i] = (__bf16)1.0f;
 
-    if (t_begin < t_end && role == 0) issue_dma(t_begin, 0);
+    auto store_pdy = [&](int buf) {
+        char* base = smem + buf * G::BUF;
+#pragma unroll
+        for (int j = 0; j < 2; ++j) {
+            const int q = (ct * 2 + j) * 64 + lane, c16 = q & 7, py = q >> 6, px = (q >> 3) & 7;
+            const unsigned v[4] = {pv[j].x, pv[j].y, pv[j].z, pv[j].w};
+#pragma unroll
+            for (int pos = 0; pos < 4; ++pos) {
+                const int ly = 2 * py + (pos >> 1), lx = 2 * px + (pos & 1);
+                const int kk = ((ly >> 1) * BW8 + (lx >> 3)) * 16 + (ly & 1) * 8 + (lx & 7);
+                const int sl = (((c16 >> 1) ^ wp_key(kk)) << 1) | (c16 & 1);
+                unsigned o[4];
+#pragma unroll
+                for (int k = 0; k < 4; ++k) {
+                    const unsigned lo = ((pc[j] >> (8 * k)) & 15u) == (unsigned)pos ? 0x0000ffffu : 0u;
+                    const unsigned hi = ((pc[j] >> (8 * k + 4)) & 15u) == (unsigned)pos ? 0xffff0000u : 0u;
+                    o[k] = v[k] & (lo | hi);
+                }
+                *reinterpret_cast<uint4*>(base + kk * 128 + sl * 16) = make_uint4(o[0], o[1], o[2], o[3]);
+            }
+        }
+    };
+    if (t_begin < t_end && role == 0) {
+        issue_dma(t_begin, 0);
+        if constexpr (PDY) store_pdy(0);
+    }
     const int gq = lane >> 4, li = lane & 15;
     int abase[4];
     {
@@ -1944,6 +2051,7 @@
             load_frag(f1, ab, gb, std::integral_constant<int, 7>{}); mma(f0); weave();
             mma(f1);
             __builtin_amdgcn_s_setprio(3);
+            if constexpr (PDY && ROLE == 0) { if (t + 1 < t_end) store_pdy(cur ^ 1); }
         }
     };
     if (role == 0) run(std::integral_constant<int, 0>{}, std::false_type{});
@@ -2794,8 +2902,9 @@
     return (size_t)512 * (64 * 72 + 64) * sizeof(float);
 }
 
-int ssd_conv2d_bwd_data_wgrad_first(const void* dy, const void* w_t, const void* relu_bits, const void* image, float* dw0,
-                                    float* dbias0, int B, int H, int W, void* ws, size_t ws_bytes, void* stream) {
+static int conv2d_bwd_data_wgrad_first_impl(const void* dy, const void* w_t, const void* relu_bits, const void* image, float* dw0,
+                                            float* dbias0, int B, int H, int W, void* ws, size_t ws_bytes, void* stream,
+                                            const void* pool_code, int Hp, int Wp) {
     if (!dy || !w_t || !relu_bits || !image || !dw0 || B <= 0 || H <= 0 || W <= 0) return SSD_ERR_VALUE;
     if (H < 16 || W < 16 || (long long)B * H * W * 64 >= (1ll << 31) - 16) return SSD_ERR_UNSUPPORTED;
     if (!ws || ws_bytes < ssd_conv2d_bwd_data_wgrad_first_workspace_bytes(B, H, W)) return SSD_ERR_WORKSPACE;
@@ -2809,13 +2918,33 @@
     float* slab_w = static_cast<float*>(ws);
     float* slab_b = slab_w + (size_t)512 * 64 * 72;
     hipStream_t s = (hipStream_t)stream;
-    auto kern = k_conv3x3_c64b<EPI_DGRAD, true>;
-    static OnceLds set; if (ensure_lds(set, reinterpret_cast<const void*>(kern), (int)(C64B_W0_LDS)) != 0) return SSD_ERR_LAUNCH;
-    hipLaunchKernelGGL(kern, dim3(grid), dim3(256), C64B_W0_LDS, s, static_cast<const bf16_raw*>(dy), static_cast<const bf16_raw*>(w_t),
-                       g, ep, tiles_x, tiles_y, C64W0{static_cast<const bf16_raw*>(image), slab_w, dbias0 ? slab_b : nullptr});
+    const C64W0 w0{static_cast<const bf16_raw*>(image), slab_w, dbias0 ? slab_b : nullptr, static_cast<const unsigned*>(pool_code), Hp, Wp};
+    if (pool_code) {
+        auto kern = k_conv3x3_c64b<EPI_DGRAD, true, true>;
+        static OnceLds set; if (ensure_lds(set, reinterpret_cast<const void*>(kern), (int)(C64B_W0_LDS)) != 0) return SSD_ERR_LAUNCH;
+        hipLaunchKernelGGL(kern, dim3(grid), dim3(256), C64B_W0_LDS, s, static_cast<const bf16_raw*>(dy), static_cast<const bf16_raw*>(w_t),
+                           g, ep, tiles_x, tiles_y, w0);
+    } else {
+        auto kern = k_conv3x3_c64b<EPI_DGRAD, true>;
+        static OnceLds set; if (ensure_lds(set, reinterpret_cast<const void*>(kern), (int)(C64B_W0_LDS)) != 0) return SSD_ERR_LAUNCH;
+        hipLaunchKernelGGL(kern, dim3(grid), dim3(256), C64B_W0_LDS, s, static_cast<const bf16_raw*>(dy), static_cast<const bf16_raw*>(w_t),
+                           g, ep, tiles_x, tiles_y, w0);
+    }
     if (hipGetLastError() != hipSuccess) return SSD_ERR_LAUNCH;
     launch_wgrad_reduce(s, slab_w, 64ll * 72, 64ll * 72, dw0, slab_b, 64ll, 64, dbias0, (int)grid);
     return ssd_launch_status();
+}
+
+int ssd_conv2d_bwd_data_wgrad_first(const void* dy, const void* w_t, const void* relu_bits, const void* image, float* dw0,
+                                    float* dbias0, int B, int H, int W, void* ws, size_t ws_bytes, void* stream) {
+    return conv2d_bwd_data_wgrad_first_impl(dy, w_t, relu_bits, image, dw0, dbias0, B, H, W, ws, ws_bytes, stream, nullptr, 0, 0);
+}
+
+int ssd_conv2d_bwd_data_wgrad_first_pooled(const void* dy_pooled, const void* pool_code, const void* w_t, const void* relu_bits,
+                                           const void* image, float* dw0, float* dbias0, int B, int H, int W, int Hp, int Wp, void* ws,
+                                           size_t ws_bytes, void* stream) {
+    if (!pool_code || !dy_pooled || Hp != (H + 1) / 2 || Wp != (W + 1) / 2) return SSD_ERR_VALUE;
+    return conv2d_bwd_data_wgrad_first_impl(dy_pooled, w_t, relu_bits, image, dw0, dbias0, B, H, W, ws, ws_bytes, stream, pool_code, Hp, Wp);
 }
 
 static bool wgrad_first_layer(int H, int W, int Ho, int Wo, int Cin, int Cout, int ldy, int ksize, int stride, int pad_t, int pad_l) {
@@ -2919,11 +3048,18 @@
 
 static int conv2d_bwd_weight_impl(const void* x, const void* dy, float* dw, float* dbias, int B, int H, int W, int Cin, int Cout,
                                   int ldy, int ksize, int stride, int pad_t, int pad_l, int Ho, int Wo, void* ws, size_t ws_bytes,
-                                  void* stream, int* plan) {
+                                  void* stream, int* plan, const void* pcode = nullptr, int hp = 0, int wp = 0) {
     if (!x || !dy || !dw || !geom_ok(B, H, W, Cin, Ho, Wo, Cout, ksize) || stride <= 0 || ldy < Cout || ldy % 8) return SSD_ERR_VALUE;
     if (!ws || ws_bytes < ssd_conv2d_bwd_weight_workspace_bytes(B, Ho, Wo, Cin, Cout, ldy, ksize)) return SSD_ERR_WORKSPACE;
     ConvGeom g = make_geom(B, H, W, Cin, Ho, Wo, ldy, ksize, ksize, stride, 1, pad_t, pad_l);
     const long long ktot = g.ldw;
+    if (pcode) {
+        int bh, bw;
+        if (wgrad_first_layer(H, W, Ho, Wo, Cin, Cout, ldy, ksize, stride, pad_t, pad_l) ||
+            !wgrad_use_patch(H, W, Ho, Wo, Cin, ksize, stride, pad_t, pad_l) || wgrad_patch_shape(Ho, Wo, &bh, &bw) != 0 ||
+            (long long)B * H * W * Cin * 2 >= (1ll << 32) - 16 || (long long)B * Ho * Wo * ldy * 2 >= (1ll << 32) - 16)
+            return SSD_ERR_UNSUPPORTED;
+    }
     if (wgrad_first_layer(H, W, Ho, Wo, Cin, Cout, ldy, ksize, stride, pad_t, pad_l)) {
         const int tx = (Wo + 15) / 16, ty = (Ho + 15) / 16, ntiles = B * tx * ty;
         const int ns = ntiles < 512 ? ntiles : 512;
@@ -2963,18 +3099,20 @@
         const int shape = wgrad_patch_shape(Ho, Wo, &bh, &bw);
         SSD_PLAN((shape == 1 ? SSD_PLAN_WG_PATCH_6x40 : (shape == 2 ? SSD_PLAN_WG_PATCH_10x24 : SSD_PLAN_WG_PATCH_16x16)) |
                  (ns >= 32 ? SSD_PLAN_F_REDUCE_WIDE : 0));
-#define SSD_LAUNCH_WP(BH_, BW8_)                                                                                    \
+#define SSD_LAUNCH_WP(BH_, BW8_, PDY_)                                                                              \
         do {                                                                                                        \
             using G_ = WpGeom<BH_, BW8_>;                                                                           \
-            auto kern_ = k_conv3x3_wgrad_patch<BH_, BW8_>;                                                          \
+            auto kern_ = k_conv3x3_wgrad_patch<BH_, BW8_, PDY_>;                                                    \
             static OnceLds set_; if (ensure_lds(set_, reinterpret_cast<const void*>(kern_), (int)(2 * G_::BUF)) != 0) return SSD_ERR_LAUNCH; \
             hipLaunchKernelGGL(kern_, dim3(grid), dim3(512), (size_t)(single ? 1 : 2) * G_::BUF, s,                  \
                                static_cast<const bf16_raw*>(x), static_cast<const bf16_raw*>(dy), slab_w,          \
-                               dbias ? slab_b : nullptr, g, tx, ty, tps, ns, Cout, single, xg);                     \
+                               dbias ? slab_b : nullptr, g, tx, ty, tps, ns, Cout, single, xg,                      \
+                               static_cast<const unsigned*>(pcode), hp, wp);                                        \
         } while (0)
-        if (shape == 1) SSD_LAUNCH_WP(6, 5);
-        else if (shape == 2) SSD_LAUNCH_WP(10, 3);
-        else SSD_LAUNCH_WP(16, 2);
+        if (pcode) SSD_LAUNCH_WP(16, 2, true);
+        else if (shape == 1) SSD_LAUNCH_WP(6, 5, false);
+        else if (shape == 2) SSD_LAUNCH_WP(10, 3, false);
+        else SSD_LAUNCH_WP(16, 2, false);
 #undef SSD_LAUNCH_WP
         if (hipGetLastError() != hipSuccess) return SSD_ERR_LAUNCH;
         launch_wgrad_reduce(s, slab_w, (long long)ldy * ktot, (long long)Cout * ktot, dw, slab_b, (long long)ldy, Cout, dbias, ns);
@@ -3091,6 +3229,17 @@
                                   stream, nullptr);
 }
 
+size_t ssd_conv2d_bwd_weight_pooled_dy_workspace_bytes(int B, int H, int W, int Cin, int Cout) {
+    return ssd_conv2d_bwd_weight_workspace_bytes(B, H, W, Cin, Cout, Cout, 3);
+}
+
+int ssd_conv2d_bwd_weight_pooled_dy(const void* x, const void* dy_pooled, const void* pool_code, float* dw, float* dbias, int B, int H,
+                                    int W, int Cin, int Cout, int Hp, int Wp, void* ws, size_t ws_bytes, void* stream) {
+    if (!pool_code || !dy_pooled || Cout <= 0 || Cout % 8 || Hp != (H + 1) / 2 || Wp != (W + 1) / 2) return SSD_ERR_VALUE;
+    return conv2d_bwd_weight_impl(x, dy_pooled, dw, dbias, B, H, W, Cin, Cout, Cout, 3, 1, 1, 1, H, W, ws, ws_bytes, stream, nullptr,
+                                  pool_code, Hp, Wp);
+}
+
 static void* const PLAN_PTR = reinterpret_cast<void*>(static_cast<uintptr_t>(64));
 
 int ssd_conv2d_fwd_plan(int B, int H, int W, int Cin, int Cout, int ksize, int stride, int pad_t, int pad_l, int Ho, int Wo,
diff --git a/ssd-object-detection_amd/engine.py b/ssd-object-detection_amd/engine.py
--- a/ssd-object-detection_amd/engine.py
+++ b/ssd-object-detection_amd/engine.py
@@ -154,6 +154,7 @@
         self.relu_bits = {} if os.environ.get("SSD_RELU_BITS", "1") == "1" else None
         self.bits_valid = set()
         self.fuse_first = os.environ.get("SSD_FUSE_FIRST", "1") == "1"
+        self.pooled_first = os.environ.get("SSD_POOLED_FIRST", "1") == "1"
         self.wgrad_probe = None
         self._vgg_mx, self._vgg_mx_range, self._vgg_mx_w = None, None, None
         self._vgg_fp8_fwd = False
@@ -882,6 +883,13 @@
                         self.batch_chain_front = False
                     else:
                         self.batch_chain_wgrads = False
+        def first_pair_fusable():
+            nd0, nd1 = self.nodes[0], self.nodes[1]
+            return (self.fuse_first and not written[1] and nd0["kind"] == "conv" and nd0["cin"] == 8 and nd0["cout"] == 64
+                    and nd1["kind"] == "conv" and nd1["cin"] == 64 and nd1["cout"] == 64 and nd1["k"] == 3 and nd1["stride"] == 1
+                    and nd1["pt"] == 1 and nd1["pl"] == 1 and nd0["k"] == 3 and nd0["stride"] == 1
+                    and self.relu_bits is not None and 1 in self.bits_valid)
+        pooled_dy = None
         for i in range(len(self.nodes) - 1, -1, -1):
             nd = self.nodes[i]
             g_out = gacts[i + 1]
@@ -897,14 +905,23 @@
                 on_side(lambda ws: None, [wt.index, bt.index])
                 opt_bucket(i)
                 continue
-            def wgrad(ws, i=i, a=acts[i], go=g_out, nd=nd, wt=wt, bt=bt):
+            def wgrad(ws, i=i, a=acts[i], go=g_out, nd=nd, wt=wt, bt=bt, pdy=pooled_dy if i == 1 else None):
                 probe = self.wgrad_probe
                 timed = probe is not None and i in probe["nodes"]
                 if timed:
                     e0, e1 = torch.cuda.Event(enable_timing=True), torch.cuda.Event(enable_timing=True)
                     e0.record()
-                ops.conv2d_bwd_weight(a, go, nd["cout"], nd["k"], nd["stride"], nd["pt"], nd["pl"], dw=self.view(wt, self.grad),
-                                      dbias=self.view(bt, self.grad), ws=ws)
+                done = False
+                if pdy is not None:
+                    try:
+                        ops.conv2d_bwd_weight_pooled_dy(a, pdy[0], pdy[1], dw=self.view(wt, self.grad), dbias=self.view(bt, self.grad), ws=ws)
+                        done = True
+                    except NotImplementedError:
+                        self.pooled_first = False
+                        ops.maxpool2x2_bwd_argmax(pdy[1], pdy[0], tuple(go.shape), out=go)
+                if not done:
+                    ops.conv2d_bwd_weight(a, go, nd["cout"], nd["k"], nd["stride"], nd["pt"], nd["pl"], dw=self.view(wt, self.grad),
+                                          dbias=self.view(bt, self.grad), ws=ws)
                 if timed:
                     e1.record()
                     probe["events"].append((i, e0, e1))
@@ -919,10 +936,19 @@
             if i == 0 or i in chained:
                 opt_bucket(i)
                 continue
-            if (i == 1 and self.fuse_first and not written[1] and self.nodes[0]["kind"] == "conv" and self.nodes[0]["cin"] == 8
-                    and self.nodes[0]["cout"] == 64 and nd["cin"] == 64 and nd["cout"] == 64 and nd["k"] == 3 and nd["stride"] == 1
-                    and nd["pt"] == 1 and nd["pl"] == 1 and self.nodes[0]["k"] == 3 and self.nodes[0]["stride"] == 1
-                    and self.relu_bits is not None and 1 in self.bits_valid):
+            if i == 1 and pooled_dy is not None:
+                wt0, bt0 = self.conv_params[0]
+                try:
+                    ops.conv2d_bwd_data_wgrad_first_pooled(pooled_dy[0], pooled_dy[1], self.w_t[1], c["rbits"][1], acts[0],
+                                                           dw=self.view(wt0, self.grad), dbias=self.view(bt0, self.grad), ws=self._ws)
+                    first_fused = True
+                    written[1] = True
+                    opt_bucket(i)
+                    continue
+                except NotImplementedError:
+                    self.pooled_first = False
+                    ops.maxpool2x2_bwd_argmax(pooled_dy[1], pooled_dy[0], tuple(g_out.shape), out=g_out)
+            if i == 1 and first_pair_fusable():
                 wt0, bt0 = self.conv_params[0]
                 try:
                     ops.conv2d_bwd_data_wgrad_first(g_out, self.w_t[1], c["rbits"][1], acts[0], dw=self.view(wt0, self.grad),
@@ -939,7 +965,14 @@
             if i in sparse_head_done:
                 main.wait_event(sparse_head_done.pop(i))
             fused = False
-            if (self.fuse_unpool is not None and self.fuse_unpool.get(i, True) and self.nodes[i - 1]["kind"] == "pool" and not written[i] and not written[i - 1]
+            if (i == 3 and self.pooled_first and self.nodes[2]["kind"] == "pool" and not written[3] and not written[2]
+                    and nd["k"] == 3 and nd["stride"] == 1 and nd["pt"] == 1 and nd["pl"] == 1 and first_pair_fusable()):
+                ops.conv2d_bwd_data(g_out, self.w_t[i], None, acts[i].shape, nd["stride"], nd["pt"], nd["pl"], accumulate=False,
+                                    out=gacts[i], ws=self._ws)
+                pooled_dy = (gacts[3], c["pool_code"][2])
+                unpooled.add(2)
+                fused = True
+            elif (self.fuse_unpool is not None and self.fuse_unpool.get(i, True) and self.nodes[i - 1]["kind"] == "pool" and not written[i] and not written[i - 1]
                     and nd["k"] == 3 and nd["stride"] == 1 and nd["pt"] == 1 and nd["pl"] == 1):
                 try:
                     ops.conv2d_bwd_data_unpool(g_out, self.w_t[i], None, c["pool_code"][i - 1], tuple(gacts[i - 1].shape),
diff --git a/ssd-object-detection_amd/ops.py b/ssd-object-detection_amd/ops.py
--- a/ssd-object-detection_amd/ops.py
+++ b/ssd-object-detection_amd/ops.py
@@ -535,6 +535,28 @@
     return dw, dbias
 
 
+def conv2d_bwd_data_wgrad_first_pooled(dy_pooled, pool_code, w_t, bits, image, dw=None, dbias=None, ws=None):
+    L = _lib.lib()
+    _bf(dy_pooled); _bf(w_t); _bf(image)
+    B, H, W, _ = image.shape
+    _, Hp, Wp, c = dy_pooled.shape
+    assert c == 64 and w_t.shape == (64, 3, 3, 64) and image.shape == (B, H, W, 8) and dy_pooled.shape[0] == B
+    assert pool_code.shape == (B, Hp, Wp, 8) and pool_code.dtype == torch.int32 and pool_code.is_contiguous()
+    assert bits.dtype == torch.uint8 and bits.shape == (B, H, W, 8)
+    if dw is None:
+        dw = torch.empty((64, 3, 3, 8), dtype=torch.float32, device=image.device)
+    if dbias is None:
+        dbias = torch.empty((64,), dtype=torch.float32, device=image.device)
+    assert dw.dtype == torch.float32 and dw.numel() == 64 * 72 and dw.is_contiguous() and dbias.dtype == torch.float32
+    wbuf = (ws or _conv_ws).get(L.ssd_conv2d_bwd_data_wgrad_first_workspace_bytes(B, H, W), image.device)
+    rc = L.ssd_conv2d_bwd_data_wgrad_first_pooled(_ptr(dy_pooled), _ptr(pool_code), _ptr(w_t), _ptr(bits), _ptr(image), _ptr(dw),
+                                                  _ptr(dbias), B, H, W, Hp, Wp, _ptr(wbuf), wbuf.numel(), _stream())
+    if rc == _lib.SSD_ERR_UNSUPPORTED:
+        raise NotImplementedError("maps smaller than 16x16 take the un-pooled form")
+    _lib.check(rc)
+    return dw, dbias
+
+
 def conv2d_bwd_data_unpool(dy, w_t, relu_src, pool_code, full_shape, out=None, ws=None, pooled_out=None):
     L = _lib.lib()
     _bf(dy); _bf(w_t)
@@ -568,6 +590,25 @@
     wbuf = (ws or _conv_ws).get(nbytes, x.device)
     _lib.check(L.ssd_conv2d_bwd_weight(_ptr(x), _ptr(dy), _ptr(dw), _ptr(dbias), B, H, W, Cin, Cout, ldy, k, stride,
                                        pad_t, pad_l, Ho, Wo, _ptr(wbuf), wbuf.numel(), _stream()))
+    return dw, dbias
+
+
+def conv2d_bwd_weight_pooled_dy(x, dy_pooled, pool_code, dw=None, dbias=None, ws=None):
+    L = _lib.lib()
+    _bf(x); _bf(dy_pooled)
+    B, H, W, Cin = x.shape
+    _, Hp, Wp, Cout = dy_pooled.shape
+    assert pool_code.shape == (B, Hp, Wp, Cout // 8) and pool_code.dtype == torch.int32 and pool_code.is_contiguous()
+    if dw is None:
+        dw = torch.empty((Cout, 3, 3, Cin), dtype=torch.float32, device=x.device)
+    if dbias is None:
+        dbias = torch.empty((Cout,), dtype=torch.float32, device=x.device)
+    wbuf = (ws or _conv_ws).get(L.ssd_conv2d_bwd_weight_pooled_dy_workspace_bytes(B, H, W, Cin, Cout), x.device)
+    rc = L.ssd_conv2d_bwd_weight_pooled_dy(_ptr(x), _ptr(dy_pooled), _ptr(pool_code), _ptr(dw), _ptr(dbias), B, H, W, Cin, Cout, Hp, Wp,
+                                           _ptr(wbuf), wbuf.numel(), _stream())
+    if rc == _lib.SSD_ERR_UNSUPPORTED:
+        raise NotImplementedError("only the 16x16-block patch kernel reads a pooled gradient")
+    _lib.check(rc)
     return dw, dbias
 
 
```
